# ebanalyse/ebnerd-benchmark

Measured on AMD Instinct MI355X. Metric: training impressions/sec, higher is better.
Workload: dtype f32

## Files before the change

### ebnerd-benchmark_amd/csrc/ebn_attpool.hip

```cpp
#include "ebn_common.h"
#include "ebn_reduce.h"

namespace {

constexpr int POOL_THREADS = 256;
constexpr int POOL_WAVES = POOL_THREADS / 64;
constexpr float KERAS_EPS = 1e-7f;

__global__ __launch_bounds__(POOL_THREADS) void attpool_fwd_kernel(float* __restrict__ U,
                                                                    const float* __restrict__ b,
                                                                    const float* __restrict__ q,
                                                                    const float* __restrict__ X,
                                                                    float* __restrict__ out,
                                                                    float* __restrict__ w, int L, int E, int A) {
  extern __shared__ float sm[];
  const int64_t n = blockIdx.x;
  const int tid = threadIdx.x, lane = tid & 63, wave = tid >> 6;
  for (int l = wave; l < L; l += POOL_WAVES) {
    float* urow = U + (n * L + l) * A;
    float part = 0.f;
    for (int k = lane; k < A; k += 64) {
      const float u = tanhf(urow[k] + b[k]);
      urow[k] = u;
      part = fmaf(u, q[k], part);
    }
    part = ebn_wave_sum(part);
    if (lane == 0) sm[l] = part;
  }
  __syncthreads();
  if (wave == 0) {
    float s = 0.f;
    for (int l = lane; l < L; l += 64) {
      const float a = expf(sm[l]);
      sm[l] = a;
      s += a;
    }
    s = ebn_wave_sum(s) + KERAS_EPS;
    for (int l = lane; l < L; l += 64) {
      const float wl = sm[l] / s;
      sm[l] = wl;
      w[n * L + l] = wl;
    }
  }
  __syncthreads();
  for (int c = tid; c < E; c += POOL_THREADS) {
    float acc = 0.f;
    for (int l = 0; l < L; ++l) acc = fmaf(sm[l], X[(n * L + l) * E + c], acc);
    out[n * E + c] = acc;
  }
}

__global__ __launch_bounds__(POOL_THREADS) void attpool_bwd_pool_kernel(const float* __restrict__ X,
                                                                         const float* __restrict__ w,
                                                                         const float* __restrict__ dout,
                                                                         float* __restrict__ dX,
                                                                         float* __restrict__ de, int L, int E) {
  extern __shared__ float sm[];
  const int64_t n = blockIdx.x;
  const int tid = threadIdx.x, lane = tid & 63, wave = tid >> 6;
  const float* g = dout + n * E;
  for (int l = wave; l < L; l += POOL_WAVES) {
    const float* xr = X + (n * L + l) * E;
    float part = 0.f;
    for (int c = lane; c < E; c += 64) part = fmaf(g[c], xr[c], part);
    part = ebn_wave_sum(part);
    if (lane == 0) sm[l] = part;
  }
  __syncthreads();
  if (wave == 0) {
    float s = 0.f;
    for (int l = lane; l < L; l += 64) s = fmaf(w[n * L + l], sm[l], s);
    s = ebn_wave_sum(s);
    for (int l = lane; l < L; l += 64) de[n * L + l] = w[n * L + l] * (sm[l] - s);
  }
  if (dX == nullptr) return;
  for (int l = 0; l < L; ++l) {
    const float wl = w[n * L + l];
    float* dr = dX + (n * L + l) * E;
    for (int c = tid; c < E; c += POOL_THREADS) dr[c] = wl * g[c];
  }
}

constexpr int POOL_RB = 8;

__device__ __forceinline__ float4 ld4_clamped(const float* __restrict__ base, int64_t off, bool ok) {
  return *reinterpret_cast<const float4*>(base + (ok ? off : 0));
}
__device__ __forceinline__ float4 ld4_or_zero(const float* __restrict__ base, int64_t off, bool ok) {
  const float4 v = ld4_clamped(base, off, ok);
  float4 r;
  r.x = ok ? v.x : 0.f;
  r.y = ok ? v.y : 0.f;
  r.z = ok ? v.z : 0.f;
  r.w = ok ? v.w : 0.f;
  return r;
}

__global__ __launch_bounds__(POOL_THREADS) void attpool_fwd_vec_kernel(float* __restrict__ U,
                                                                        const float* __restrict__ b,
                                                                        const float* __restrict__ q,
                                                                        const float* __restrict__ X,
                                                                        float* __restrict__ out,
                                                                        float* __restrict__ w, int L, int E, int A) {
  extern __shared__ float sm[];
  __shared__ float4 part_acc[POOL_THREADS];
  const int64_t n = blockIdx.x;
  const int tid = threadIdx.x, lane = tid & 63, wave = tid >> 6;
  const int A4 = A >> 2, E4 = E >> 2;
  {
    const bool kok = lane < A4;
    const float4 bb = ld4_or_zero(b, lane * 4, kok), qq = ld4_or_zero(q, lane * 4, kok);
    for (int l0 = wave; l0 < L; l0 += POOL_WAVES * POOL_RB) {
      float4 u[POOL_RB];
#pragma unroll
      for (int j = 0; j < POOL_RB; ++j) {
        const int l = l0 + POOL_WAVES * j;
        u[j] = ld4_clamped(U, (n * L + l) * A + lane * 4, kok && l < L);
      }
#pragma unroll
      for (int j = 0; j < POOL_RB; ++j) {
        const int l = l0 + POOL_WAVES * j;
        if (l >= L) break;
        float4 t;
        t.x = tanhf(u[j].x + bb.x);
        t.y = tanhf(u[j].y + bb.y);
        t.z = tanhf(u[j].z + bb.z);
        t.w = tanhf(u[j].w + bb.w);
        if (kok) *reinterpret_cast<float4*>(U + (n * L + l) * A + lane * 4) = t;
        float part = kok ? fmaf(t.w, qq.w, fmaf(t.z, qq.z, fmaf(t.y, qq.y, t.x * qq.x))) : 0.f;
        part = ebn_wave_sum(part);
        if (lane == 0) sm[l] = part;
      }
    }
  }
  __syncthreads();
  if (wave == 0) {
    float s = 0.f;
    for (int l = lane; l < L; l += 64) {
      const float a = expf(sm[l]);
      sm[l] = a;
      s += a;
    }
    s = ebn_wave_sum(s) + KERAS_EPS;
    for (int l = lane; l < L; l += 64) {
      const float wl = sm[l] / s;
      sm[l] = wl;
      w[n * L + l] = wl;
    }
  }
  __syncthreads();
  const int NP = (E4 <= POOL_THREADS) ? POOL_THREADS / E4 : 1;
  for (int c0 = 0; c0 < E4; c0 += POOL_THREADS) {
    const int c4 = c0 + tid % ((E4 <= POOL_THREADS) ? E4 : POOL_THREADS);
    const int part = (E4 <= POOL_THREADS) ? tid / E4 : 0;
    const bool ok = c4 < E4 && part < NP;
    float4 acc = make_float4(0.f, 0.f, 0.f, 0.f);
    for (int l0 = part; l0 < L; l0 += NP * POOL_RB) {
      float4 x[POOL_RB];
#pragma unroll
      for (int j = 0; j < POOL_RB; ++j) {
        const int l = l0 + NP * j;
        x[j] = ld4_clamped(X, (n * L + l) * E + c4 * 4, ok && l < L);
      }
#pragma unroll
      for (int j = 0; j < POOL_RB; ++j) {
        const int l = l0 + NP * j;
        const float wl = (l < L) ? sm[l] : 0.f;
        acc.x = fmaf(wl, x[j].x, acc.x);
        acc.y = fmaf(wl, x[j].y, acc.y);
        acc.z = fmaf(wl, x[j].z, acc.z);
        acc.w = fmaf(wl, x[j].w, acc.w);
      }
    }
    if (NP > 1) {
      part_acc[tid] = acc;
      __syncthreads();
      if (part == 0 && ok) {
        for (int pp = 1; pp < NP; ++pp) {
          const float4 o = part_acc[pp * E4 + c4];
          acc.x += o.x;
          acc.y += o.y;
          acc.z += o.z;
          acc.w += o.w;
        }
      }
      __syncthreads();
    }
    if (part == 0 && ok) *reinterpret_cast<float4*>(out + n * E + c4 * 4) = acc;
  }
}

__global__ __launch_bounds__(POOL_THREADS) void attpool_bwd_pool_vec_kernel(const float* __restrict__ X,
                                                                             const float* __restrict__ w,
                                                                             const float* __restrict__ dout,
                                                                             float* __restrict__ dX,
                                                                             float* __restrict__ de, int L, int E,
                                                                             int write_dx) {
  extern __shared__ float sm[];
  const int64_t n = blockIdx.x;
  const int tid = threadIdx.x, lane = tid & 63, wave = tid >> 6;
  const int E4 = E >> 2;
  const float* g = dout + n * E;
  constexpr int VL = 4;
  float4 gg[VL];
#pragma unroll
  for (int v = 0; v < VL; ++v) gg[v] = ld4_or_zero(g, (lane + 64 * v) * 4, lane + 64 * v < E4);
  for (int l0 = wave; l0 < L; l0 += POOL_WAVES * POOL_RB) {
    float part[POOL_RB];
#pragma unroll
    for (int j = 0; j < POOL_RB; ++j) part[j] = 0.f;
#pragma unroll
    for (int v = 0; v < VL; ++v) {
      if (64 * v >= E4) break;
      float4 x[POOL_RB];
#pragma unroll
      for (int j = 0; j < POOL_RB; ++j) {
        const int l = l0 + POOL_WAVES * j;
        x[j] = ld4_clamped(X, (n * L + l) * E + (lane + 64 * v) * 4, l < L && lane + 64 * v < E4);
      }
#pragma unroll
      for (int j = 0; j < POOL_RB; ++j)
        part[j] = fmaf(gg[v].w, x[j].w, fmaf(gg[v].z, x[j].z, fmaf(gg[v].y, x[j].y, fmaf(gg[v].x, x[j].x, part[j]))));
    }
#pragma unroll
    for (int j = 0; j < POOL_RB; ++j) {
      const int l = l0 + POOL_WAVES * j;
      const float t = ebn_wave_sum(part[j]);
      if (lane == 0 && l < L) sm[l] = t;
    }
  }
  __syncthreads();
  if (wave == 0) {
    float s = 0.f;
    for (int l = lane; l < L; l += 64) s = fmaf(w[n * L + l], sm[l], s);
    s = ebn_wave_sum(s);
    for (int l = lane; l < L; l += 64) de[n * L + l] = w[n * L + l] * (sm[l] - s);
  }
  if (!write_dx) return;
  for (int c4 = tid; c4 < E4; c4 += POOL_THREADS) {
    const float4 gv = *reinterpret_cast<const float4*>(g + c4 * 4);
    for (int l = 0; l < L; ++l) {
      const float wl = w[n * L + l];
      *reinterpret_cast<float4*>(dX + (n * L + l) * E + c4 * 4) = make_float4(wl * gv.x, wl * gv.y, wl * gv.z, wl * gv.w);
    }
  }
}

__global__ __launch_bounds__(POOL_THREADS) void attpool_bwd_dpre_kernel(float* __restrict__ U,
                                                                         const float* __restrict__ q,
                                                                         const float* __restrict__ de,
                                                                         float* __restrict__ partials,
                                                                         int64_t R, int A, int64_t rpb) {
  const int64_t r0 = static_cast<int64_t>(blockIdx.x) * rpb;
  const int64_t r1 = (r0 + rpb < R) ? r0 + rpb : R;
  for (int k = threadIdx.x; k < A; k += POOL_THREADS) {
    const float qk = q[k];
    float dq = 0.f, db = 0.f;
    for (int64_t rb = r0; rb < r1; rb += 8) {
      float u[8], der[8];
#pragma unroll
      for (int j = 0; j < 8; ++j) {
        const int64_t r = (rb + j < r1) ? rb + j : r1 - 1;
        u[j] = U[r * A + k];
        der[j] = de[r];
      }
#pragma unroll
      for (int j = 0; j < 8; ++j) {
        if (rb + j >= r1) break;
        dq = fmaf(der[j], u[j], dq);
        const float dp = der[j] * qk * (1.0f - u[j] * u[j]);
        U[(rb + j) * A + k] = dp;
        db += dp;
      }
    }
    partials[(static_cast<int64_t>(blockIdx.x) * 2 + 0) * A + k] = dq;
    partials[(static_cast<int64_t>(blockIdx.x) * 2 + 1) * A + k] = db;
  }
}

}

__global__ __launch_bounds__(POOL_THREADS) void attpool_bwd_dpre_vec_kernel(float* __restrict__ U, const float* __restrict__ q,
                                                                             const float* __restrict__ de, float* __restrict__ partials,
                                                                             int64_t R, int A, int64_t rpb) {
  extern __shared__ float sm[];
  const int A4 = A >> 2, RS = POOL_THREADS / A4;
  const int tid = threadIdx.x, c4 = tid % A4, rs = tid / A4;
  const bool active = rs < RS;
  const int64_t r0 = static_cast<int64_t>(blockIdx.x) * rpb;
  const int64_t r1 = (r0 + rpb < R) ? r0 + rpb : R;
  float4 dq = make_float4(0.f, 0.f, 0.f, 0.f), db = dq;
  if (active) {
    const float4 qk = *reinterpret_cast<const float4*>(q + c4 * 4);
    for (int64_t rb = r0 + rs; rb < r1; rb += static_cast<int64_t>(8) * RS) {
      float4 u[8];
      float der[8];
#pragma unroll
      for (int j = 0; j < 8; ++j) {
        int64_t r = rb + static_cast<int64_t>(j) * RS;
        r = r < r1 ? r : r1 - 1;
        u[j] = *reinterpret_cast<const float4*>(U + r * A + c4 * 4);
        der[j] = de[r];
      }
#pragma unroll
      for (int j = 0; j < 8; ++j) {
        const int64_t r = rb + static_cast<int64_t>(j) * RS;
        if (r >= r1) break;
        const float d = der[j];
        dq.x = fmaf(d, u[j].x, dq.x);
        dq.y = fmaf(d, u[j].y, dq.y);
        dq.z = fmaf(d, u[j].z, dq.z);
        dq.w = fmaf(d, u[j].w, dq.w);
        const float4 dp = make_float4(d * qk.x * (1.0f - u[j].x * u[j].x), d * qk.y * (1.0f - u[j].y * u[j].y),
                                      d * qk.z * (1.0f - u[j].z * u[j].z), d * qk.w * (1.0f - u[j].w * u[j].w));
        *reinterpret_cast<float4*>(U + r * A + c4 * 4) = dp;
        db.x += dp.x;
        db.y += dp.y;
        db.z += dp.z;
        db.w += dp.w;
      }
    }
    *reinterpret_cast<float4*>(&sm[rs * A + c4 * 4]) = dq;
    *reinterpret_cast<float4*>(&sm[(RS + rs) * A + c4 * 4]) = db;
  }
  __syncthreads();
  for (int k = tid; k < A; k += POOL_THREADS) {
    float tq = 0.f, tb = 0.f;
    for (int i = 0; i < RS; ++i) {
      tq += sm[i * A + k];
      tb += sm[(RS + i) * A + k];
    }
    partials[(static_cast<int64_t>(blockIdx.x) * 2 + 0) * A + k] = tq;
    partials[(static_cast<int64_t>(blockIdx.x) * 2 + 1) * A + k] = tb;
  }
}

extern "C" int64_t ebn_attpool_partials_len(int64_t R, int32_t A) { return ebn_dim_ok(R, A) ? ebn_colred_blocks(R) * 2 * A : 0; }

extern "C" int ebn_attpool_fwd_f32(float* U, const float* b, const float* q, const float* X, float* out,
                                   float* w, int64_t n_seq, int32_t L, int32_t E, int32_t A,
                                   ebn_stream_t stream) {
  EBN_REQUIRE(U && b && q && X && out && w, EBN_ERR_BAD_ARG);
  EBN_REQUIRE(n_seq >= 0 && L > 0 && E > 0 && A > 0, EBN_ERR_BAD_ARG);
  EBN_REQUIRE(L <= 8192, EBN_ERR_UNSUPPORTED);
  if (n_seq == 0) return EBN_OK;
  const bool vec = (A % 4 == 0) && A <= 256 && (E % 4 == 0) && E <= 1024 && ebn_aligned16(U) && ebn_aligned16(b) &&
                   ebn_aligned16(q) && ebn_aligned16(X) && ebn_aligned16(out);
  if (vec)
    EBN_LAUNCH(attpool_fwd_vec_kernel, dim3(static_cast<unsigned>(n_seq)), dim3(POOL_THREADS),
                       L * sizeof(float), ebn_stream(stream), U, b, q, X, out, w, L, E, A);
  else
    EBN_LAUNCH(attpool_fwd_kernel, dim3(static_cast<unsigned>(n_seq)), dim3(POOL_THREADS),
                       L * sizeof(float), ebn_stream(stream), U, b, q, X, out, w, L, E, A);
  EBN_CHECK_LAUNCH();
  return EBN_OK;
}

extern "C" int ebn_attpool_bwd_pool_f32(const float* X, const float* w, const float* dout, float* dX,
                                        float* de, int64_t n_seq, int32_t L, int32_t E,
                                        ebn_stream_t stream) {
  EBN_REQUIRE(X && w && dout && de, EBN_ERR_BAD_ARG);
  EBN_REQUIRE(n_seq >= 0 && L > 0 && E > 0, EBN_ERR_BAD_ARG);
  EBN_REQUIRE(L <= 8192, EBN_ERR_UNSUPPORTED);
  if (n_seq == 0) return EBN_OK;
  const bool vec = (E % 4 == 0) && E <= 1024 && ebn_aligned16(X) && ebn_aligned16(dout) && ebn_aligned16(dX);
  if (vec)
    EBN_LAUNCH(attpool_bwd_pool_vec_kernel, dim3(static_cast<unsigned>(n_seq)), dim3(POOL_THREADS),
                       L * sizeof(float), ebn_stream(stream), X, w, dout, dX, de, L, E, dX != nullptr ? 1 : 0);
  else
    EBN_LAUNCH(attpool_bwd_pool_kernel, dim3(static_cast<unsigned>(n_seq)), dim3(POOL_THREADS),
                       L * sizeof(float), ebn_stream(stream), X, w, dout, dX, de, L, E);
  EBN_CHECK_LAUNCH();
  return EBN_OK;
}

extern "C" int ebn_attpool_bwd_dpre_f32(float* U, const float* q, const float* de, float* dq, float* db,
                                        float* partials, int64_t R, int32_t A, int32_t accumulate,
                                        ebn_stream_t stream) {
  EBN_REQUIRE(U && q && de && partials && ((dq != nullptr) == (db != nullptr)), EBN_ERR_BAD_ARG);
  EBN_REQUIRE(R >= 0 && A > 0, EBN_ERR_BAD_ARG);
  if (R == 0) return EBN_OK;
  const int64_t nb = ebn_colred_blocks(R);
  const int64_t rpb = ebn_ceil_div(R, nb);
  if ((A % 4) == 0 && A >= 4 && A <= 1024 && ebn_aligned16(U) && ebn_aligned16(q)) {
    const size_t lds = static_cast<size_t>(2) * (POOL_THREADS / (A / 4)) * A * sizeof(float);
    EBN_LAUNCH(attpool_bwd_dpre_vec_kernel, dim3(static_cast<unsigned>(nb)), dim3(POOL_THREADS), lds, ebn_stream(stream), U, q, de, partials,
                       R, A, rpb);
  } else {
    EBN_LAUNCH(attpool_bwd_dpre_kernel, dim3(static_cast<unsigned>(nb)), dim3(POOL_THREADS), 0,
                       ebn_stream(stream), U, q, de, partials, R, A, rpb);
  }
  EBN_CHECK_LAUNCH();
  if (dq == nullptr) return EBN_OK;
  ebn_reduce_partials(partials, nb, 2, A, 1.0f, dq, db, accumulate, nullptr, nullptr, ebn_stream(stream));
  EBN_CHECK_LAUNCH();
  return EBN_OK;
}
```

### ebnerd-benchmark_amd/csrc/ebn_encoder.hip

```cpp
#include "ebn_common.h"

#define EBN_TRY(call)            \
  do {                           \
    int rc__ = (call);           \
    if (rc__ != EBN_OK) return rc__; \
  } while (0)

static int check_dims(const ebn_encoder_dims* d) {
  EBN_REQUIRE(d, EBN_ERR_BAD_ARG);
  EBN_REQUIRE(d->n_seq >= 0 && d->L > 0 && d->Din > 0 && d->h > 0 && d->d > 0 && d->A > 0, EBN_ERR_BAD_ARG);
  return EBN_OK;
}

extern "C" int ebn_encoder_fwd_f32(const ebn_encoder_dims* dims, const ebn_encoder_params* p,
                                   const ebn_encoder_acts* a, const ebn_encoder_scratch* s,
                                   const ebn_step_state* st, ebn_stream_t stream) {
  EBN_TRY(check_dims(dims));
  EBN_REQUIRE(p && a && p->Wqkv && p->W && p->b && p->q, EBN_ERR_BAD_ARG);
  EBN_REQUIRE(a->X && a->QKV && a->Y && a->U && a->w && a->out, EBN_ERR_BAD_ARG);
  const int64_t R = dims->n_seq * dims->L;
  const int E = dims->h * dims->d;
  if (R == 0) return EBN_OK;
  float* ws = s ? s->gemm_ws : nullptr;
  const int64_t ws_n = s ? s->gemm_ws_floats : 0;
  EBN_TRY(ebn_gemm_f32_site(0, 0, R, 3 * E, dims->Din, 1.0f, a->X, dims->Din, p->Wqkv, 3 * E, 0.0f, a->QKV, 3 * E, ws, ws_n,
                            1, stream));
  EBN_TRY(ebn_attn_fwd_f32(a->QKV, 3 * E, a->Y, E, dims->n_seq, dims->L, dims->h, dims->d, st, dims->drop_site,
                           dims->drop_p, stream));
  EBN_TRY(ebn_gemm_f32_ws(0, 0, R, dims->A, E, 1.0f, a->Y, E, p->W, dims->A, 0.0f, a->U, dims->A, ws, ws_n, stream));
  EBN_TRY(ebn_attpool_fwd_f32(a->U, p->b, p->q, a->Y, a->out, a->w, dims->n_seq, dims->L, E, dims->A, stream));
  return EBN_OK;
}

extern "C" int ebn_encoder_fwd_gather_f32(const ebn_encoder_dims* dims, const ebn_encoder_params* p, const ebn_encoder_acts* a,
                                          const ebn_encoder_scratch* s, const int32_t* ids, const float* table, int64_t table_rows,
                                          int32_t* oob_flag, ebn_stream_t stream) {
  EBN_TRY(check_dims(dims));
  EBN_REQUIRE(p && a && ids && table && p->Wqkv && p->W && p->b && p->q, EBN_ERR_BAD_ARG);
  EBN_REQUIRE(a->QKV && a->Y && a->U && a->w && a->out, EBN_ERR_BAD_ARG);
  EBN_REQUIRE(dims->drop_p <= 0.0f, EBN_ERR_UNSUPPORTED);
  const int64_t R = dims->n_seq * dims->L;
  const int E = dims->h * dims->d;
  if (R == 0) return EBN_OK;
  float* ws = s ? s->gemm_ws : nullptr;
  const int64_t ws_n = s ? s->gemm_ws_floats : 0;
  EBN_TRY(ebn_gemm_f32_rowmap(ids, table_rows, R, 3 * E, dims->Din, table, dims->Din, p->Wqkv, 3 * E, a->QKV, 3 * E, oob_flag, stream));
  EBN_TRY(ebn_attn_fwd_f32(a->QKV, 3 * E, a->Y, E, dims->n_seq, dims->L, dims->h, dims->d, nullptr, -1, 0.0f, stream));
  EBN_TRY(ebn_gemm_f32_ws(0, 0, R, dims->A, E, 1.0f, a->Y, E, p->W, dims->A, 0.0f, a->U, dims->A, ws, ws_n, stream));
  EBN_TRY(ebn_attpool_fwd_f32(a->U, p->b, p->q, a->Y, a->out, a->w, dims->n_seq, dims->L, E, dims->A, stream));
  return EBN_OK;
}

extern "C" int ebn_encoder_bwd_f32(const ebn_encoder_dims* dims, const ebn_encoder_params* p,
                                   const ebn_encoder_acts* a, const float* dout, const ebn_encoder_grads* g,
                                   const ebn_encoder_scratch* s, float* dX, int32_t accumulate,
                                   const ebn_step_state* st, ebn_stream_t stream) {
  EBN_TRY(check_dims(dims));
  EBN_REQUIRE(p && a && g && s && dout, EBN_ERR_BAD_ARG);
  EBN_REQUIRE(p->Wqkv && p->W && p->q, EBN_ERR_BAD_ARG);
  EBN_REQUIRE(a->X && a->QKV && a->Y && a->U && a->w, EBN_ERR_BAD_ARG);
  EBN_REQUIRE(g->dWqkv && g->dW && g->db && g->dq, EBN_ERR_BAD_ARG);
  EBN_REQUIRE(s->dY && s->dQKV && s->de && s->partials, EBN_ERR_BAD_ARG);
  const int64_t R = dims->n_seq * dims->L;
  const int E = dims->h * dims->d;
  const int A = dims->A;
  if (R == 0) return EBN_OK;
  const float beta = accumulate ? 1.0f : 0.0f;
  EBN_TRY(ebn_attpool_bwd_pool_f32(a->Y, a->w, dout, nullptr, s->de, dims->n_seq, dims->L, E, stream));
  EBN_TRY(ebn_attpool_bwd_dpre_f32(a->U, p->q, s->de, g->dq, g->db, s->partials, R, A, accumulate, stream));
  const bool fold = ebn_attn_bwd_pooled_supported(dims->L, dims->d) != 0 && (E % 4) == 0 && ebn_aligned16(dout) &&
                    ebn_aligned16(s->dY) && ebn_aligned16(a->QKV) && ebn_aligned16(s->dQKV);
  if (fold) {
    EBN_TRY(ebn_dense_bwd_pair_f32(R, E, A, a->Y, E, a->U, A, p->W, A, beta, g->dW, A, s->dY, E, s->gemm_ws, s->gemm_ws_floats,
                                   stream));
    EBN_TRY(ebn_attn_bwd_pooled_f32(a->QKV, 3 * E, s->dY, E, a->w, dout, E, s->dQKV, 3 * E, dims->n_seq, dims->L, dims->h,
                                    dims->d, st, dims->drop_site, dims->drop_p, stream));
  } else {
    EBN_TRY(ebn_gemm_f32_ws(1, 0, E, A, R, 1.0f, a->Y, E, a->U, A, beta, g->dW, A, s->gemm_ws, s->gemm_ws_floats, stream));
    EBN_TRY(ebn_gemm_f32_rank1(R, E, A, 1.0f, a->U, A, p->W, A, s->dY, E, a->w, dout, E, dims->L, s->gemm_ws,
                               s->gemm_ws_floats, stream));
    EBN_TRY(ebn_attn_bwd_f32(a->QKV, 3 * E, s->dY, E, s->dQKV, 3 * E, dims->n_seq, dims->L, dims->h, dims->d, st, dims->drop_site,
                             dims->drop_p, stream));
  }
  if (dX != nullptr)
    return ebn_dense_bwd_pair_f32(R, dims->Din, 3 * E, a->X, dims->Din, s->dQKV, 3 * E, p->Wqkv, 3 * E, beta, g->dWqkv, 3 * E, dX,
                                  dims->Din, s->gemm_ws, s->gemm_ws_floats, stream);
  EBN_TRY(ebn_gemm_f32_ws(1, 0, dims->Din, 3 * E, R, 1.0f, a->X, dims->Din, s->dQKV, 3 * E, beta, g->dWqkv, 3 * E,
                          s->gemm_ws, s->gemm_ws_floats, stream));
  return EBN_OK;
}

extern "C" int ebn_user_stage_train_f32(const ebn_encoder_dims* dims, const ebn_encoder_params* p, const ebn_encoder_acts* a,
                                        const float* cand, const float* labels, float* scores, float* probs, float* loss_rows,
                                        float* loss_out, float* dcand, float* duser, const ebn_encoder_grads* g,
                                        const ebn_encoder_scratch* s, float* head_partials, float* dX, int32_t C,
                                        int32_t loss_kind, float inv_batch, const ebn_step_state* st, ebn_stream_t stream) {
  EBN_TRY(check_dims(dims));
  EBN_REQUIRE(p && a && g && s && cand && labels && scores && probs && loss_rows && loss_out && dcand && duser && dX, EBN_ERR_BAD_ARG);
  EBN_REQUIRE(p->Wqkv && p->W && p->b && p->q && a->X && a->QKV && a->Y && a->U && a->w && a->out, EBN_ERR_BAD_ARG);
  EBN_REQUIRE(g->dWqkv && g->dW && g->db && g->dq && s->dY && s->dQKV && s->de && s->partials, EBN_ERR_BAD_ARG);
  EBN_REQUIRE(C > 0 && dims->drop_p <= 0.0f, EBN_ERR_BAD_ARG);
  const int64_t B = dims->n_seq, R = dims->n_seq * dims->L;
  const int E = dims->h * dims->d, A = dims->A, L = dims->L;
  if (R == 0) return EBN_OK;
  const bool fused = head_partials != nullptr && ebn_user_head_supported(L, C, E, A) != 0 &&
                     ebn_attn_bwd_pooled_supported(L, dims->d) != 0 && ebn_aligned16(a->U) && ebn_aligned16(a->Y) &&
                     ebn_aligned16(cand) && ebn_aligned16(dcand) && ebn_aligned16(duser) && ebn_aligned16(a->out) &&
                     ebn_aligned16(p->b) && ebn_aligned16(p->q) && ebn_aligned16(s->dY) && ebn_aligned16(a->QKV) &&
                     ebn_aligned16(s->dQKV);
  if (!fused) {
    EBN_TRY(ebn_encoder_fwd_f32(dims, p, a, s, st, stream));
    EBN_TRY(ebn_score_loss_train_f32(cand, a->out, labels, scores, probs, loss_rows, loss_out, dcand, duser, B, C, E, loss_kind,
                                     inv_batch, stream));
    return ebn_encoder_bwd_f32(dims, p, a, duser, g, s, dX, 0, st, stream);
  }
  float* ws = s->gemm_ws;
  const int64_t ws_n = s->gemm_ws_floats;
  EBN_TRY(ebn_gemm_f32_site(0, 0, R, 3 * E, dims->Din, 1.0f, a->X, dims->Din, p->Wqkv, 3 * E, 0.0f, a->QKV, 3 * E, ws, ws_n, 1, stream));
  EBN_TRY(ebn_attn_fwd_f32(a->QKV, 3 * E, a->Y, E, B, L, dims->h, dims->d, nullptr, -1, 0.0f, stream));
  EBN_TRY(ebn_gemm_f32_ws(0, 0, R, A, E, 1.0f, a->Y, E, p->W, A, 0.0f, a->U, A, ws, ws_n, stream));
  EBN_TRY(ebn_user_head_train_f32(a->U, p->b, p->q, a->Y, cand, labels, a->w, a->out, scores, probs, loss_rows, loss_out, dcand,
                                  duser, s->de, g->dq, g->db, head_partials, B, L, C, E, A, loss_kind, inv_batch, stream));
  EBN_TRY(ebn_dense_bwd_pair_f32(R, E, A, a->Y, E, a->U, A, p->W, A, 0.0f, g->dW, A, s->dY, E, ws, ws_n, stream));
  EBN_TRY(ebn_attn_bwd_pooled_f32(a->QKV, 3 * E, s->dY, E, a->w, duser, E, s->dQKV, 3 * E, B, L, dims->h, dims->d, nullptr, -1, 0.0f,
                                  stream));
  return ebn_dense_bwd_pair_f32(R, dims->Din, 3 * E, a->X, dims->Din, s->dQKV, 3 * E, p->Wqkv, 3 * E, 0.0f, g->dWqkv, 3 * E, dX,
                                dims->Din, ws, ws_n, stream);
}
```

### ebnerd-benchmark_amd/csrc/ebn_gemm.hip

```cpp
#include <stdlib.h>

#include "ebn_common.h"
#include "ebn_finish.h"
#include "ebn_tn_finale.h"

typedef float ebn_f32x4 __attribute__((ext_vector_type(4)));
typedef int ebn_i32x4 __attribute__((ext_vector_type(4)));
__device__ ebn_f32x4 ebn_raw_buffer_load_x4(ebn_i32x4 rsrc, int voffset, int soffset, int aux) __asm("llvm.amdgcn.raw.buffer.load.v4f32");
__device__ void ebn_raw_buffer_load_lds(ebn_i32x4 rsrc, __attribute__((address_space(3))) void* lds, int size, int voffset,
                                        int soffset, int offset, int aux) __asm("llvm.amdgcn.raw.buffer.load.lds");

int ebn_gemm_direct_tn_slices(int64_t M, int64_t N, int64_t K);
int ebn_gemm_direct_tn_launch(int64_t M, int64_t N, int64_t K, float alpha, const float* A, int64_t lda, const float* B, int64_t ldb,
                              float* part, hipStream_t s);
bool ebn_gemm_direct_wanted(int32_t transA, int32_t transB, int64_t M, int64_t N, int64_t K);
int ebn_gemm_direct_launch(int32_t transB, int64_t M, int64_t N, int64_t K, float alpha, const float* A, int64_t lda, const float* B,
                           int64_t ldb, float* C, int64_t ldc, hipStream_t s);

namespace {

typedef float f32x16 __attribute__((ext_vector_type(16)));


typedef float f32x4n __attribute__((ext_vector_type(4)));
__device__ __forceinline__ float4 gload4(const __attribute__((address_space(1))) float* p) {
  const f32x4n t = *reinterpret_cast<const __attribute__((address_space(1))) f32x4n*>(p);
  return make_float4(t.x, t.y, t.z, t.w);
}
typedef ebn_i32x4 i32x4n;
__device__ __forceinline__ i32x4n make_rsrc(const float* base) {
  const unsigned long long a = reinterpret_cast<unsigned long long>(base);
  i32x4n r;
  r.x = static_cast<int>(static_cast<uint32_t>(a));
  r.y = static_cast<int>(static_cast<uint32_t>(a >> 32) & 0xFFFFu);
  r.z = -1;
  r.w = 0x00020000;
  return r;
}
__device__ __forceinline__ float4 bload4(i32x4n r, uint32_t lane_bytes, uint32_t slab_bytes) {
  const f32x4n t = ebn_raw_buffer_load_x4(r, static_cast<int>(lane_bytes), static_cast<int>(slab_bytes), 0);
  return make_float4(t.x, t.y, t.z, t.w);
}

constexpr int GEMM_WPE = 3;
constexpr int BK = 16;
constexpr int PAD = 4;
constexpr int GEMM_THREADS = 256;

template <int BMN, bool KCONTIG, bool VEC, int PADX = PAD>
struct TileLoader {
  static constexpr int VECS = BMN * BK / 4;
  static constexpr int PER_THREAD = VECS / GEMM_THREADS;
  static_assert(VECS % GEMM_THREADS == 0, "tile/thread mismatch");

  __device__ static __forceinline__ float4 load(const float* __restrict__ P, int64_t ld, int64_t mn0,
                                                int64_t k0, int64_t MN, int64_t Kdim, int v) {
    int64_t gmn, gk;
    if (KCONTIG) {
      gmn = mn0 + v / (BK / 4);
      gk = k0 + (v % (BK / 4)) * 4;
    } else {
      gk = k0 + v / (BMN / 4);
      gmn = mn0 + (v % (BMN / 4)) * 4;
    }
    const int64_t off = KCONTIG ? (gmn * ld + gk) : (gk * ld + gmn);
    if (VEC) {
      const bool valid = (gmn < MN) && (gk < Kdim);
      const float4 r = *reinterpret_cast<const float4*>(P + (valid ? off : 0));
      float4 z;
      z.x = valid ? r.x : 0.f;
      z.y = valid ? r.y : 0.f;
      z.z = valid ? r.z : 0.f;
      z.w = valid ? r.w : 0.f;
      return z;
    }
    float4 r = make_float4(0.f, 0.f, 0.f, 0.f);
    if (KCONTIG) {
      if (gmn < MN) {
        const float* p = P + off;
        if (gk + 0 < Kdim) r.x = p[0];
        if (gk + 1 < Kdim) r.y = p[1];
        if (gk + 2 < Kdim) r.z = p[2];
        if (gk + 3 < Kdim) r.w = p[3];
      }
    } else {
      if (gk < Kdim) {
        const float* p = P + off;
        if (gmn + 0 < MN) r.x = p[0];
        if (gmn + 1 < MN) r.y = p[1];
        if (gmn + 2 < MN) r.z = p[2];
        if (gmn + 3 < MN) r.w = p[3];
      }
    }
    return r;
  }

  __device__ static __forceinline__ void store(float* __restrict__ S, int v, float4 r) {
    constexpr int LD = BMN + PADX;
    if (KCONTIG) {
      const int mn = v / (BK / 4);
      const int kq = v % (BK / 4);
      *reinterpret_cast<float4*>(&S[(mn * 4 + (kq ^ ((mn >> 2) & 3))) * 4]) = r;
    } else {
      const int k = v / (BMN / 4);
      const int mq = v % (BMN / 4);
      *reinterpret_cast<float4*>(&S[k * LD + mq * 4]) = r;
    }
  }
};

struct GemmEpi {
  const float* rs;
  const float* cv;
  int64_t ldcv;
  int32_t L;
  const float* bias;
  float* colsum = nullptr;
  const float* l2w = nullptr;
  float two_lambda = 0.f;
  const int32_t* rowmap = nullptr;
  int64_t rowmap_rows = 0;
  int32_t* oob = nullptr;
#ifdef EBN_GEMM_EXP_STAGGER
  uint32_t stagger_pct = 0;
#endif
};

template <int BM, int BN, int WAVES_M, bool TA, bool TB, bool VEC, int EPI = 0>
__global__ __launch_bounds__(GEMM_THREADS, GEMM_WPE) void gemm_f32_kernel(
    int64_t M, int64_t N, int64_t K, float alpha, const float* __restrict__ A, int64_t lda,
    const float* __restrict__ B, int64_t ldb, float beta, float* __restrict__ C, int64_t ldc,
    int64_t k_per_split, float* __restrict__ Cpart, GemmEpi epi) {
  constexpr int WAVES_N = 4 / WAVES_M;
  constexpr int WTM = BM / WAVES_M;
  constexpr int WTN = BN / WAVES_N;
  constexpr int TM = WTM / 32;
  constexpr int TN = WTN / 32;
  constexpr bool GLDS_A = VEC;
  constexpr bool GLDS_B = GLDS_A;
  constexpr int PADA = GLDS_A ? 0 : PAD, PADB = GLDS_B ? 0 : PAD;
  constexpr int LDA_S = BM + PADA;
  constexpr int LDB_S = BN + PADB;
  using LA = TileLoader<BM, !TA, VEC, PADA>;
  using LB = TileLoader<BN, TB, VEC, PADB>;

  constexpr bool A_KC = !TA, B_KC = TB;
  constexpr int A_FLOATS = A_KC ? BM * BK : BK * LDA_S, B_FLOATS = B_KC ? BN * BK : BK * LDB_S;
  __shared__ __attribute__((aligned(16))) float smem[2 * (A_FLOATS + B_FLOATS)];
#define EBN_AS(b) (smem + (b) * A_FLOATS)
#define EBN_BS(b) (smem + 2 * A_FLOATS + (b) * B_FLOATS)

  const int tid = threadIdx.x;
  const int lane = tid & 63;
  const int wave = __builtin_amdgcn_readfirstlane(tid >> 6);
  const int wm = wave / WAVES_N;
  const int wn = wave % WAVES_N;
  const int64_t GX = gridDim.x, GY = gridDim.y, GZ = gridDim.z;
  const int64_t per_z = GX * GY, nwg = per_z * GZ;
  const int64_t vb = static_cast<int64_t>(blockIdx.y) * gridDim.x + blockIdx.x + per_z * blockIdx.z;
  int64_t m0 = 0, n0 = 0, kbeg = 0, kend = 0, zsplit = 0;
  int nk = 0, nk_full = 0, nk_main = 0;

  f32x16 acc[TM][TN];

  float4 ra[LA::PER_THREAD], rb[LB::PER_THREAD];

  uint32_t oa[LA::PER_THREAD], ob[LB::PER_THREAD];
  i32x4n arsrc, brsrc;
  const uint32_t step_a = static_cast<uint32_t>((TA ? BK * lda : BK) * 4);
  const uint32_t step_b = static_cast<uint32_t>((TB ? BK : BK * ldb) * 4);
// ... 803 lines not shown
    if (b < nh - 1) {
      const int idx = b * 256 + tid;
      if (tid < 256 && idx < 2 * f.A) {
        const int sidx = idx / f.A, k = idx - sidx * f.A;
        float* gp = (sidx == 0 ? f.dq : f.db) + k;
        ebn_adam_flat_apply(f.adam, al, gp - f.adam.grad, *gp);
      }
    } else if (tid == 0 && f.n_l2 > 0) {
      float tot = 0.f;
      for (int l = 0; l < f.n_l2; ++l) {
        float tl = 0.f;
        for (int j = 0; j < f.l2_tiles[l]; ++j) tl += f.l2_part[l * f.l2_slots + j];
        tot += tl;
      }
      f.loss_out[0] += f.l2 * tot;
    }
  }
}

int launch_gemm_small(int transA, int transB, int64_t M, int64_t N, int64_t K, float alpha, const float* A, int64_t lda,
                      const float* B, int64_t ldb, float beta, float* C, int64_t ldc, int vecA, int vecB, hipStream_t s,
                      GemmEpi epi) {
  const dim3 grid(static_cast<unsigned>(ebn_ceil_div(N, SBN)), static_cast<unsigned>(ebn_ceil_div(M, SBM))), block(GEMM_THREADS);
  constexpr size_t lds = static_cast<size_t>(2) * 2 * SBM * SLD * sizeof(float);
#define EBN_SMALL_ONE(TA, TB, VA, VB)                                                                                     \
  do {                                                                                                                     \
    static const hipError_t attr__ = hipFuncSetAttribute(reinterpret_cast<const void*>(&gemm_small_kernel<TA, TB, VA, VB>), \
                                                         hipFuncAttributeMaxDynamicSharedMemorySize, static_cast<int>(lds)); \
    if (attr__ != hipSuccess) return static_cast<int>(attr__);                                                            \
    EBN_LAUNCH((gemm_small_kernel<TA, TB, VA, VB>), grid, block, lds, s, M, N, K, alpha, A, lda, B, ldb, beta, C, ldc, epi); \
  } while (0)
#define EBN_SMALL_VEC_T(TA, TB, T)                                                                                         \
  do {                                                                                                                     \
    constexpr size_t lds_t = static_cast<size_t>(2) * 2 * (T) * SLV * sizeof(float);                                       \
    static const hipError_t attr__ = hipFuncSetAttribute(reinterpret_cast<const void*>(&gemm_small_vec_kernel<TA, TB, T>), \
                                                         hipFuncAttributeMaxDynamicSharedMemorySize, static_cast<int>(lds_t)); \
    if (attr__ != hipSuccess) return static_cast<int>(attr__);                                                            \
    const dim3 grid_t(static_cast<unsigned>(ebn_ceil_div(N, T)), static_cast<unsigned>(ebn_ceil_div(M, T)));               \
    EBN_LAUNCH((gemm_small_vec_kernel<TA, TB, T>), grid_t, dim3((T) * (T) / 4), lds_t, s, M, N, K, alpha, A, lda, B, ldb, \
                       beta, C, ldc, epi);                                                                                 \
  } while (0)
#define EBN_SMALL_VEC(TA, TB) EBN_SMALL_VEC_T(TA, TB, 32)
  const bool fits32 = (K + SBK) * (transA ? lda : 1) * 4 + 64 * lda * 4 < (int64_t{1} << 31) &&
                      (K + SBK) * (transB ? 1 : ldb) * 4 + 64 * ldb * 4 < (int64_t{1} << 31);
#define EBN_SMALL(TA, TB)                              \
  do {                                                 \
    if (vecA && vecB && fits32) EBN_SMALL_VEC(TA, TB); \
    else EBN_SMALL_ONE(TA, TB, false, false);          \
  } while (0)
  if (!transA && !transB) EBN_SMALL(false, false);
  else if (!transA && transB) EBN_SMALL(false, true);
  else if (transA && !transB) EBN_SMALL(true, false);
  else EBN_SMALL(true, true);
#undef EBN_SMALL
#undef EBN_SMALL_VEC
#undef EBN_SMALL_VEC_T
#undef EBN_SMALL_ONE
  EBN_CHECK_LAUNCH();
  return EBN_OK;
}

}

struct GemmPlan {
  int bm, bn;
  int splits;
  int64_t kps;
  double cost;
};

static GemmPlan gemm_plan(int64_t M, int64_t N, int64_t K, int64_t ws_floats) {
  int64_t max_split = K / (4 * BK);
  if (max_split > 64) max_split = 64;
  const int64_t max_by_ws = (M * N > 0) ? ws_floats / (M * N) : 0;
  if (max_split > max_by_ws) max_split = max_by_ws;
  if (max_split < 1 || M * N >= (static_cast<int64_t>(1) << 31)) max_split = 1;
  static const struct {
    int bm, bn;
    double ts_full, ts_lone;
    int resident;
    int family;
  } kTiles[4] = {{128, 128, 1.15, 1.5, 3, 128}, {256, 64, 1.17, 1.5, 3, 256}, {64, 64, 0.32, 0.48, 4, 64}, {128, 64, 0.60, 0.8, 3, 96}};
  const double out_mb = static_cast<double>(M) * static_cast<double>(N) * 4e-6;
  GemmPlan best{128, 128, 1, ebn_ceil_div(K > 0 ? K : 1, BK) * BK, 1e300};
  {
    const int64_t wgs = ebn_ceil_div(M, SBM) * ebn_ceil_div(N, SBN);
    const int64_t tiles64 = ebn_ceil_div(M, 64) * ebn_ceil_div(N, 64);
    if (tiles64 <= 256 && K <= 4096) {
      const int64_t W = ebn_ceil_div(wgs, 256);
      double per_slab = static_cast<double>(W / 2) * 1.6 + static_cast<double>(W % 2) * 1.1;
      if (W >= 3) per_slab *= 1.3;
      const double cost = static_cast<double>(ebn_ceil_div(K > 0 ? K : 1, SBK)) * per_slab + 3.0;
      const bool measured = K <= 1536 && W <= 3;
      best = GemmPlan{32, 32, 1, ebn_ceil_div(K > 0 ? K : 1, SBK) * SBK, measured ? cost : 0.8 * cost};
      if (measured) return best;
    }
  }
  for (int t = 0; t < 4; ++t) {
    if (kTiles[t].bm == 256 && M < 256) continue;
    const int64_t tiles = ebn_ceil_div(M, kTiles[t].bm) * ebn_ceil_div(N, kTiles[t].bn);
    int64_t prev_s = 0;
    for (int64_t c = 1; c <= max_split; ++c) {
      const int64_t kps = ebn_ceil_div(ebn_ceil_div(K > 0 ? K : 1, c), BK) * BK;
      const int64_t sp = ebn_ceil_div(K > 0 ? K : 1, kps);
      if (sp == prev_s) continue;
      prev_s = sp;
      const int64_t W = ebn_ceil_div(tiles * sp, 256);
      const double full = static_cast<double>(W) * kTiles[t].ts_full;
      const double lone = static_cast<double>(ebn_ceil_div(W, kTiles[t].resident)) * kTiles[t].ts_lone;
      double cost = static_cast<double>(kps / BK) * (full > lone ? full : lone) + 3.0;
      if (sp > 1) cost += 4.5 + static_cast<double>(sp + 1) * out_mb / 2.5;
      if (kTiles[t].bm == 64 && sp > 1 && kps / BK >= 64 && W <= 6) cost *= 1.0 - 0.01 * static_cast<double>(W);
      if (cost < best.cost) best = GemmPlan{kTiles[t].bm, kTiles[t].bn, static_cast<int>(sp), kps, cost};
    }
  }
  return best;
}

extern "C" int64_t ebn_gemm_workspace_floats(int64_t M, int64_t N, int64_t K) {
  if (!ebn_dim_ok(M, N, K)) return 0;
  const GemmPlan p = gemm_plan(M, N, K, INT64_MAX / 4);
  int64_t slices = p.splits > 1 ? p.splits : 0;
  const int64_t tn = ebn_gemm_direct_tn_slices(M, N, K);
  if (tn > slices) slices = tn;
  return ebn_sat_mul(slices * M, N);
}

extern "C" int ebn_gemm_plan(int64_t M, int64_t N, int64_t K, int64_t workspace_floats, int32_t* bm, int32_t* bn,
                             int32_t* splits) {
  EBN_REQUIRE(M >= 0 && N >= 0 && K >= 0 && bm && bn && splits, EBN_ERR_BAD_ARG);
  const GemmPlan p = gemm_plan(M, N, K, workspace_floats);
  *bm = p.bm;
  *bn = p.bn;
  *splits = p.splits;
  return EBN_OK;
}

static int gemm_dispatch(int32_t transA, int32_t transB, int64_t M, int64_t N, int64_t K, float alpha, const float* A,
                         int64_t lda, const float* B, int64_t ldb, float beta, float* C, int64_t ldc, float* workspace,
                         int64_t workspace_floats, int32_t site, GemmEpi epi, hipStream_t s, int32_t* defer_parts = nullptr) {
  if (defer_parts != nullptr) {
    C = workspace;
    ldc = N;
    beta = 0.f;
    *defer_parts = 1;
  }
  const bool spanA = (transA ? (K + 16) * lda + 256 : 256 * lda + K + 16) * 4 < (int64_t{1} << 32);
  const bool spanB = (transB ? 256 * ldb + K + 16 : (K + 16) * ldb + 256) * 4 < (int64_t{1} << 32);
  const int vecA = ((lda % 4) == 0 && ebn_aligned16(A) && ((transA ? M : K) % 4) == 0 && spanA) ? 1 : 0;
  const int vecB = ((ldb % 4) == 0 && ebn_aligned16(B) && ((transB ? K : N) % 4) == 0 && spanB) ? 1 : 0;
  if ((epi.bias != nullptr || epi.rs != nullptr) && !(vecA && vecB)) return EBN_ERR_UNSUPPORTED;
  if (epi.bias == nullptr && epi.rs == nullptr && beta == 0.f && vecA && (vecB || !transB) &&
      ebn_gemm_direct_wanted(transA, transB, M, N, K)) {
    const int rc_dir = ebn_gemm_direct_launch(transB, M, N, K, alpha, A, lda, B, ldb, C, ldc, s);
    if (rc_dir != EBN_ERR_UNSUPPORTED) return rc_dir;
  }
  if (transA && !transB && epi.bias == nullptr && epi.rs == nullptr && workspace != nullptr &&
      M * N < (int64_t{1} << 31)) {
    const int z = ebn_gemm_direct_tn_slices(M, N, K);
    if (z >= 2 && workspace_floats >= static_cast<int64_t>(z) * M * N) {
      const int rc_tn = ebn_gemm_direct_tn_launch(M, N, K, alpha, A, lda, B, ldb, workspace, s);
      if (rc_tn == EBN_OK) {
        if (defer_parts != nullptr) {
          *defer_parts = z;
          return EBN_OK;
        }
        int64_t grid = ebn_ceil_div(M * N, 256);
        if (grid > 4096) grid = 4096;
        EBN_LAUNCH(splitk_reduce_kernel, dim3(static_cast<unsigned>(grid)), dim3(256), 0, s, workspace, z, M, N, beta, C, ldc, epi);
        EBN_CHECK_LAUNCH();
        return EBN_OK;
      }
      if (rc_tn != EBN_ERR_UNSUPPORTED) return rc_tn;
    }
  }
  const GemmPlan plan = gemm_plan(M, N, K, workspace ? workspace_floats : 0);
  const int splits = plan.splits;
  const int64_t kps = plan.kps;
  int rc;
  if (plan.bm == 32)
    return launch_gemm_small(transA, transB, M, N, K, alpha, A, lda, B, ldb, beta, C, ldc, vecA, vecB, s, epi);
  if (!(vecA && vecB))
    rc = launch_gemm<64, 64, 2>(transA, transB, M, N, K, alpha, A, lda, B, ldb, beta, C, ldc, vecA, vecB, splits, kps, workspace, s, site, epi);
  else if (plan.bm == 256)
    rc = launch_gemm<256, 64, 4>(transA, transB, M, N, K, alpha, A, lda, B, ldb, beta, C, ldc, vecA, vecB, splits, kps,
                                 workspace, s, site, epi);
  else if (plan.bm == 128 && plan.bn == 64)
    rc = launch_gemm<128, 64, 2>(transA, transB, M, N, K, alpha, A, lda, B, ldb, beta, C, ldc, vecA, vecB, splits, kps,
                                 workspace, s, site, epi);
  else if (plan.bm == 128)
    rc = launch_gemm<128, 128, 2>(transA, transB, M, N, K, alpha, A, lda, B, ldb, beta, C, ldc, vecA, vecB, splits, kps,
                                  workspace, s, site, epi);
  else
    rc = launch_gemm<64, 64, 2>(transA, transB, M, N, K, alpha, A, lda, B, ldb, beta, C, ldc, vecA, vecB, splits, kps,
                                workspace, s, site, epi);
  if (rc != EBN_OK) return rc;
  if (splits > 1 && defer_parts != nullptr) {
    *defer_parts = splits;
    return EBN_OK;
  }
  if (splits > 1) {
    int64_t grid = ebn_ceil_div(M * N, 256);
    if (grid > 4096) grid = 4096;
    EBN_LAUNCH(splitk_reduce_kernel, dim3(static_cast<unsigned>(grid)), dim3(256), 0, s, workspace,
                       splits, M, N, beta, C, ldc, epi);
    EBN_CHECK_LAUNCH();
  }
  return EBN_OK;
}

extern "C" int64_t ebn_gemm_partials_workspace_floats(int64_t M, int64_t N, int64_t K) {
  if (!ebn_dim_ok(M, N, K)) return 0;
  const GemmPlan p = gemm_plan(M, N, K, INT64_MAX / 4);
  int64_t slices = p.splits > 1 ? p.splits : 1;
  const int64_t tn = ebn_gemm_direct_tn_slices(M, N, K);
  if (tn > slices) slices = tn;
  return ebn_sat_mul(slices * M, N);
}

extern "C" int ebn_gemm_f32_partials(int32_t transA, int32_t transB, int64_t M, int64_t N, int64_t K, float alpha, const float* A,
                                     int64_t lda, const float* B, int64_t ldb, float* workspace, int64_t workspace_floats,
                                     int32_t* n_parts, ebn_stream_t stream) {
  EBN_REQUIRE(M > 0 && N > 0 && K >= 0 && n_parts, EBN_ERR_BAD_ARG);
  EBN_REQUIRE(A && B && workspace && workspace_floats >= M * N, EBN_ERR_BAD_ARG);
  EBN_REQUIRE(lda >= (transA ? M : K) && ldb >= (transB ? K : N), EBN_ERR_BAD_ARG);
  return gemm_dispatch(transA, transB, M, N, K, alpha, A, lda, B, ldb, 0.0f, workspace, N, workspace, workspace_floats, 0,
                       GemmEpi{nullptr, nullptr, 0, 1, nullptr}, ebn_stream(stream), n_parts);
}

extern "C" int ebn_gemm_f32_site(int32_t transA, int32_t transB, int64_t M, int64_t N, int64_t K, float alpha,
                                 const float* A, int64_t lda, const float* B, int64_t ldb, float beta, float* C,
                                 int64_t ldc, float* workspace, int64_t workspace_floats, int32_t site,
                                 ebn_stream_t stream) {
  EBN_REQUIRE(M >= 0 && N >= 0 && K >= 0, EBN_ERR_BAD_ARG);
  if (M == 0 || N == 0) return EBN_OK;
  EBN_REQUIRE(A && B && C, EBN_ERR_BAD_ARG);
  EBN_REQUIRE(lda >= (transA ? M : K) && ldb >= (transB ? K : N) && ldc >= N, EBN_ERR_BAD_ARG);
  return gemm_dispatch(transA, transB, M, N, K, alpha, A, lda, B, ldb, beta, C, ldc, workspace, workspace_floats, site,
                       GemmEpi{nullptr, nullptr, 0, 1, nullptr}, ebn_stream(stream));
}

namespace {
__global__ __launch_bounds__(256) void rank1_fill_kernel(float* __restrict__ C, int64_t ldc, int64_t M, int64_t N,
                                                         GemmEpi epi) {
  const int64_t total = M * N;
  for (int64_t i = static_cast<int64_t>(blockIdx.x) * 256 + threadIdx.x; i < total; i += static_cast<int64_t>(gridDim.x) * 256) {
    const int64_t row = i / N, col = i - row * N;
    C[row * ldc + col] = epi.rs[row] * epi.cv[(row / epi.L) * epi.ldcv + col];
  }
}
}

extern "C" int ebn_gemm_f32_rank1(int64_t M, int64_t N, int64_t K, float alpha, const float* A, int64_t lda,
                                  const float* B, int64_t ldb, float* C, int64_t ldc, const float* row_scale,
                                  const float* seq_rows, int64_t ld_seq, int32_t L, float* workspace,
                                  int64_t workspace_floats, ebn_stream_t stream) {
  EBN_REQUIRE(M >= 0 && N >= 0 && K >= 0 && L > 0, EBN_ERR_BAD_ARG);
  EBN_REQUIRE(M < (static_cast<int64_t>(1) << 31), EBN_ERR_UNSUPPORTED);
  if (M == 0 || N == 0) return EBN_OK;
  EBN_REQUIRE(A && B && C && row_scale && seq_rows, EBN_ERR_BAD_ARG);
  EBN_REQUIRE(lda >= K && ldb >= K && ldc >= N && ld_seq >= N, EBN_ERR_BAD_ARG);
  const GemmEpi epi{row_scale, seq_rows, ld_seq, L, nullptr};
  hipStream_t s = ebn_stream(stream);
  const bool vec = (lda % 4) == 0 && ebn_aligned16(A) && (ldb % 4) == 0 && ebn_aligned16(B) && (K % 4) == 0;
  if (vec)
    return gemm_dispatch(0, 1, M, N, K, alpha, A, lda, B, ldb, 0.0f, C, ldc, workspace, workspace_floats, 0, epi, s);
  int64_t grid = ebn_ceil_div(M * N, 256);
  if (grid > 4096) grid = 4096;
  EBN_LAUNCH(rank1_fill_kernel, dim3(static_cast<unsigned>(grid)), dim3(256), 0, s, C, ldc, M, N, epi);
  EBN_CHECK_LAUNCH();
  return gemm_dispatch(0, 1, M, N, K, alpha, A, lda, B, ldb, 1.0f, C, ldc, workspace, workspace_floats, 0,
                       GemmEpi{nullptr, nullptr, 0, 1, nullptr}, s);
}

extern "C" int ebn_dense_relu_fwd_f32(int64_t M, int64_t N, int64_t K, const float* A, int64_t lda, const float* B,
                                      int64_t ldb, const float* bias, float* C, int64_t ldc, float* workspace,
                                      int64_t workspace_floats, ebn_stream_t stream) {
  EBN_REQUIRE(M >= 0 && N >= 0 && K >= 0, EBN_ERR_BAD_ARG);
  if (M == 0 || N == 0) return EBN_OK;
  EBN_REQUIRE(A && B && C && bias, EBN_ERR_BAD_ARG);
  EBN_REQUIRE(lda >= K && ldb >= N && ldc >= N, EBN_ERR_BAD_ARG);
  hipStream_t s = ebn_stream(stream);
  const bool vec = (lda % 4) == 0 && ebn_aligned16(A) && (K % 4) == 0 && (ldb % 4) == 0 && ebn_aligned16(B) && (N % 4) == 0;
  if (vec)
    return gemm_dispatch(0, 0, M, N, K, 1.0f, A, lda, B, ldb, 0.0f, C, ldc, workspace, workspace_floats, 0,
                         GemmEpi{nullptr, nullptr, 0, 1, bias}, s);
  const int rc = gemm_dispatch(0, 0, M, N, K, 1.0f, A, lda, B, ldb, 0.0f, C, ldc, workspace, workspace_floats, 0,
                               GemmEpi{nullptr, nullptr, 0, 1, nullptr}, s);
  if (rc != EBN_OK) return rc;
  for (int64_t r = 0; ldc != N && r < M; ++r) {
    const int rr = ebn_bias_relu_f32(C + r * ldc, bias, C + r * ldc, 1, static_cast<int32_t>(N), stream);
    if (rr != EBN_OK) return rr;
  }
  return (ldc == N) ? ebn_bias_relu_f32(C, bias, C, M, static_cast<int32_t>(N), stream) : EBN_OK;
}

extern "C" int ebn_gemm_f32_ws(int32_t transA, int32_t transB, int64_t M, int64_t N, int64_t K, float alpha,
                               const float* A, int64_t lda, const float* B, int64_t ldb, float beta,
                               float* C, int64_t ldc, float* workspace, int64_t workspace_floats,
                               ebn_stream_t stream) {
  return ebn_gemm_f32_site(transA, transB, M, N, K, alpha, A, lda, B, ldb, beta, C, ldc, workspace, workspace_floats, 0,
                           stream);
}

extern "C" int ebn_dense_bwd_pair_f32(int64_t R, int64_t K_in, int64_t N_out, const float* X, int64_t ldx, const float* dY,
                                      int64_t lddy, const float* W, int64_t ldw, float beta_w, float* dW, int64_t lddw,
                                      float* dX, int64_t lddx, float* workspace, int64_t workspace_floats,
                                      ebn_stream_t stream) {
  EBN_REQUIRE(R >= 0 && K_in >= 0 && N_out >= 0, EBN_ERR_BAD_ARG);
  if (K_in == 0 || N_out == 0) return EBN_OK;
  EBN_REQUIRE(X && dY && W && dW && dX, EBN_ERR_BAD_ARG);
  EBN_REQUIRE(ldx >= K_in && lddy >= N_out && ldw >= N_out && lddw >= N_out && lddx >= K_in, EBN_ERR_BAD_ARG);
  hipStream_t s = ebn_stream(stream);
  const bool aligned = (ldx % 4) == 0 && (lddy % 4) == 0 && (ldw % 4) == 0 && ebn_aligned16(X) && ebn_aligned16(dY) &&
                       ebn_aligned16(W) && (K_in % 4) == 0 && (N_out % 4) == 0;
  const int64_t span = (R + SBK) * (ldx > lddy ? ldx : lddy) * 4 + 64 * ((ldx > lddy ? ldx : lddy) > ldw ? (ldx > lddy ? ldx : lddy) : ldw) * 4;
  const bool small = R > 0 && gemm_plan(K_in, N_out, R, workspace ? workspace_floats : 0).bm == 32 &&
                     gemm_plan(R, K_in, N_out, workspace ? workspace_floats : 0).bm == 32;
  if (aligned && small && span < (int64_t{1} << 31)) {
    SmallProblem p0{K_in, N_out, R, 1.0f, X, ldx, dY, lddy, beta_w, dW, lddw, static_cast<int32_t>(ebn_ceil_div(N_out, SBN)), 0};
    p0.tiles = p0.tiles_x * static_cast<int32_t>(ebn_ceil_div(K_in, SBM));
    SmallProblem p1{R, K_in, N_out, 1.0f, dY, lddy, W, ldw, 0.0f, dX, lddx, static_cast<int32_t>(ebn_ceil_div(K_in, SBN)), 0};
    p1.tiles = p1.tiles_x * static_cast<int32_t>(ebn_ceil_div(R, SBM));
    constexpr size_t lds = static_cast<size_t>(2) * 2 * SBM * SLV * sizeof(float);
    static const hipError_t attr = hipFuncSetAttribute(reinterpret_cast<const void*>(&gemm_small_pair_kernel),
                                                       hipFuncAttributeMaxDynamicSharedMemorySize, static_cast<int>(lds));
    if (attr != hipSuccess) return static_cast<int>(attr);
    EBN_LAUNCH(gemm_small_pair_kernel, dim3(static_cast<unsigned>(p0.tiles + p1.tiles)), dim3(GEMM_THREADS), lds, s, p0, p1);
    EBN_CHECK_LAUNCH();
    return EBN_OK;
  }
  const GemmEpi none{nullptr, nullptr, 0, 1, nullptr};
  if (R == 0) {
    return gemm_dispatch(1, 0, K_in, N_out, 0, 1.0f, X, ldx, dY, lddy, beta_w, dW, lddw, workspace, workspace_floats, 0, none, s);
  }
  const int rc = gemm_dispatch(1, 0, K_in, N_out, R, 1.0f, X, ldx, dY, lddy, beta_w, dW, lddw, workspace, workspace_floats, 0, none, s);
  if (rc != EBN_OK) return rc;
  return gemm_dispatch(0, 1, R, K_in, N_out, 1.0f, dY, lddy, W, ldw, 0.0f, dX, lddx, workspace, workspace_floats, 0, none, s);
}

extern "C" int ebn_gemm_f32_rowmap(const int32_t* ids, int64_t table_rows, int64_t M, int64_t N, int64_t K, const float* table,
                                   int64_t ldt, const float* B, int64_t ldb, float* C, int64_t ldc, int32_t* oob_flag, ebn_stream_t stream) {
  EBN_REQUIRE(ebn_dim_ok(M, N, K) && table_rows > 0, EBN_ERR_BAD_ARG);
  if (M == 0 || N == 0) return EBN_OK;
  EBN_REQUIRE(ids && table && B && C && ldt >= K && ldb >= N && ldc >= N && K > 0, EBN_ERR_BAD_ARG);
  const bool ok = M >= 256 && (ldt % 4) == 0 && (ldb % 4) == 0 && (K % 4) == 0 && (N % 4) == 0 && ebn_aligned16(table) && ebn_aligned16(B) &&
                  (table_rows * ldt + K + 16) * 4 < (int64_t{1} << 32) && ((K + 16) * ldb + 256) * 4 < (int64_t{1} << 32);
  if (!ok) return EBN_ERR_UNSUPPORTED;
  GemmEpi epi{nullptr, nullptr, 0, 1, nullptr};
  epi.rowmap = ids;
  epi.rowmap_rows = table_rows;
  epi.oob = oob_flag;
  return launch_gemm<256, 64, 4>(0, 0, M, N, K, 1.0f, table, ldt, B, ldb, 0.0f, C, ldc, 1, 1, 1, ebn_ceil_div(K, BK) * BK, nullptr,
                                 ebn_stream(stream), 0, epi);
}

extern "C" int ebn_gemm_tn_group_f32(const ebn_tn_problem* problems, int32_t n, ebn_stream_t stream) {
  EBN_REQUIRE(problems != nullptr && n >= 1 && n <= EBN_TN_GROUP_MAX, EBN_ERR_BAD_ARG);
  int64_t tiles64 = 0;
  for (int i = 0; i < n; ++i) {
    const ebn_tn_problem& q = problems[i];
    EBN_REQUIRE(ebn_dim_ok(q.M, q.N, q.K) && q.K >= 1, EBN_ERR_BAD_ARG);
    if (q.M == 0 || q.N == 0) continue;
    EBN_REQUIRE(q.A && q.B && q.C, EBN_ERR_BAD_ARG);
    EBN_REQUIRE(q.lda >= q.M && q.ldb >= q.N && q.ldc >= q.N, EBN_ERR_BAD_ARG);
    EBN_REQUIRE((q.lda % 4) == 0 && (q.ldb % 4) == 0 && (q.M % 4) == 0 && (q.N % 4) == 0 && ebn_aligned16(q.A) && ebn_aligned16(q.B),
                EBN_ERR_UNSUPPORTED);
    EBN_REQUIRE((q.K + SBK) * (q.lda > q.ldb ? q.lda : q.ldb) * 4 + 64 * 4 < (int64_t{1} << 31), EBN_ERR_UNSUPPORTED);
    tiles64 += ebn_ceil_div(q.M, 64) * ebn_ceil_div(q.N, 64);
  }
  const int T = tiles64 >= 192 ? 64 : 32;
  SmallGroup g{};
  int64_t total = 0;
  g.n = 0;
  for (int i = 0; i < n; ++i) {
    const ebn_tn_problem& q = problems[i];
    if (q.M == 0 || q.N == 0) continue;
    const int j = g.n++;
    g.p[j] = SmallProblem{q.M, q.N, q.K, 1.0f, q.A, q.lda, q.B, q.ldb, 0.0f, q.C, q.ldc, static_cast<int32_t>(ebn_ceil_div(q.N, T)), 0};
    g.p[j].tiles = g.p[j].tiles_x * static_cast<int32_t>(ebn_ceil_div(q.M, T));
    g.colsum[j] = q.colsum;
    g.l2w[j] = q.l2_W;
    g.two_lambda[j] = q.two_lambda;
    g.first[j] = static_cast<int32_t>(total);
    total += g.p[j].tiles;
    EBN_REQUIRE(total < (int64_t{1} << 30), EBN_ERR_UNSUPPORTED);
  }
  if (g.n == 0) return EBN_OK;
  g.first[g.n] = static_cast<int32_t>(total);
#define EBN_TN_GROUP(TT)                                                                                                          \
  do {                                                                                                                            \
    constexpr size_t lds = static_cast<size_t>(2) * 2 * (TT) * SLV * sizeof(float);                                               \
    static const hipError_t attr = hipFuncSetAttribute(reinterpret_cast<const void*>(&gemm_small_tn_group_kernel<TT>),            \
                                                       hipFuncAttributeMaxDynamicSharedMemorySize, static_cast<int>(lds));        \
    if (attr != hipSuccess) return static_cast<int>(attr);                                                                        \
    EBN_LAUNCH(gemm_small_tn_group_kernel<TT>, dim3(static_cast<unsigned>(total)), dim3((TT) * (TT) / 4), lds, ebn_stream(stream), g); \
  } while (0)
  if (T == 64) EBN_TN_GROUP(64);
  else EBN_TN_GROUP(32);
#undef EBN_TN_GROUP
  EBN_CHECK_LAUNCH();
  return EBN_OK;
}

int ebn_tn_group_finale_launch(const ebn_tn_problem* problems, int32_t n, const EbnTnFinale& fin, hipStream_t s) {
  EBN_REQUIRE(problems != nullptr && n >= 1 && n <= EBN_TN_GROUP_MAX, EBN_ERR_BAD_ARG);
  int64_t tiles64 = 0;
  for (int i = 0; i < n; ++i) {
    const ebn_tn_problem& q = problems[i];
    EBN_REQUIRE(ebn_dim_ok(q.M, q.N, q.K) && q.K >= 1 && q.M > 0 && q.N > 0, EBN_ERR_BAD_ARG);
    EBN_REQUIRE(q.A && q.B && q.C, EBN_ERR_BAD_ARG);
    EBN_REQUIRE(q.lda >= q.M && q.ldb >= q.N && q.ldc >= q.N, EBN_ERR_BAD_ARG);
    EBN_REQUIRE((q.lda % 4) == 0 && (q.ldb % 4) == 0 && (q.M % 4) == 0 && (q.N % 4) == 0 && ebn_aligned16(q.A) && ebn_aligned16(q.B),
                EBN_ERR_UNSUPPORTED);
    EBN_REQUIRE((q.K + SBK) * (q.lda > q.ldb ? q.lda : q.ldb) * 4 + 64 * 4 < (int64_t{1} << 31), EBN_ERR_UNSUPPORTED);
    tiles64 += ebn_ceil_div(q.M, 64) * ebn_ceil_div(q.N, 64);
  }
  const int T = tiles64 >= 192 ? 64 : 32;
  SmallGroupFin gf{};
  gf.f = fin;
  SmallGroup& g = gf.g;
  int64_t total = 0;
  g.n = n;
  for (int i = 0; i < n; ++i) {
    const ebn_tn_problem& q = problems[i];
    g.p[i] = SmallProblem{q.M, q.N, q.K, 1.0f, q.A, q.lda, q.B, q.ldb, 0.0f, q.C, q.ldc, static_cast<int32_t>(ebn_ceil_div(q.N, T)), 0};
    g.p[i].tiles = g.p[i].tiles_x * static_cast<int32_t>(ebn_ceil_div(q.M, T));
    g.colsum[i] = q.colsum;
    g.l2w[i] = q.l2_W;
    g.two_lambda[i] = q.two_lambda;
    g.first[i] = static_cast<int32_t>(total);
    total += g.p[i].tiles;
    EBN_REQUIRE(total < (int64_t{1} << 30), EBN_ERR_UNSUPPORTED);
  }
  g.first[n] = static_cast<int32_t>(total);
  const int64_t nh = (2 * static_cast<int64_t>(fin.A) + 255) / 256 + 1, nwg = total > nh ? total : nh;
#define EBN_TN_FINALE(TT)                                                                                                         \
  do {                                                                                                                            \
    constexpr size_t lds = static_cast<size_t>(2) * 2 * (TT) * SLV * sizeof(float);                                               \
    static const hipError_t attr = hipFuncSetAttribute(reinterpret_cast<const void*>(&gemm_small_tn_finale_kernel<TT>),           \
                                                       hipFuncAttributeMaxDynamicSharedMemorySize, static_cast<int>(lds));        \
    if (attr != hipSuccess) return static_cast<int>(attr);                                                                        \
    EBN_LAUNCH(gemm_small_tn_finale_kernel<TT>, dim3(static_cast<unsigned>(nwg)), dim3((TT) * (TT) / 4), lds, s, gf);             \
  } while (0)
  if (T == 64) EBN_TN_FINALE(64);
  else EBN_TN_FINALE(32);
#undef EBN_TN_FINALE
  EBN_CHECK_LAUNCH();
  return EBN_OK;
}

extern "C" int ebn_gemm_f32(int32_t transA, int32_t transB, int64_t M, int64_t N, int64_t K, float alpha,
                            const float* A, int64_t lda, const float* B, int64_t ldb, float beta, float* C,
                            int64_t ldc, ebn_stream_t stream) {
  return ebn_gemm_f32_ws(transA, transB, M, N, K, alpha, A, lda, B, ldb, beta, C, ldc, nullptr, 0, stream);
// ... 2 lines not shown
```

### ebnerd-benchmark_amd/csrc/ebn_gemm_direct.hip

```cpp
#include <stdlib.h>

#include "ebn_common.h"

typedef float ebn_dir_f32x4 __attribute__((ext_vector_type(4)));
typedef int ebn_dir_i32x4 __attribute__((ext_vector_type(4)));
__device__ ebn_dir_f32x4 ebn_dir_buffer_load_x4(ebn_dir_i32x4 rsrc, int voffset, int soffset, int aux) __asm("llvm.amdgcn.raw.buffer.load.v4f32");
__device__ float ebn_dir_buffer_load_x1(ebn_dir_i32x4 rsrc, int voffset, int soffset, int aux) __asm("llvm.amdgcn.raw.buffer.load.f32");

namespace {

constexpr bool INTERLEAVE = true;
typedef float f32x4 __attribute__((ext_vector_type(4)));

__device__ __forceinline__ ebn_dir_i32x4 dir_rsrc(const float* base) {
  const unsigned long long a = reinterpret_cast<unsigned long long>(base);
  ebn_dir_i32x4 r;
  r.x = static_cast<int>(static_cast<uint32_t>(a));
  r.y = static_cast<int>(static_cast<uint32_t>(a >> 32) & 0xFFFFu);
  r.z = -1;
  r.w = 0x00020000;
  return r;
}

template <int R, int NC>
struct DirFrags {
  f32x4 a[R];
  f32x4 b[NC];
};

template <int R, int NC, bool B_KC>
struct DirPlan {
  ebn_dir_i32x4 arsrc, brsrc;
  uint32_t oa[R];
  uint32_t ob[NC];
  uint32_t ldb4;
};

template <int R, int NC, bool B_KC>
__device__ __forceinline__ void dir_fetch(DirFrags<R, NC>& f, const DirPlan<R, NC, B_KC>& p, uint32_t sa, uint32_t sb) {
#pragma unroll
  for (int r = 0; r < R; ++r) f.a[r] = ebn_dir_buffer_load_x4(p.arsrc, static_cast<int>(p.oa[r]), static_cast<int>(sa), 0);
  if (B_KC) {
#pragma unroll
    for (int c = 0; c < NC; ++c) f.b[c] = ebn_dir_buffer_load_x4(p.brsrc, static_cast<int>(p.ob[c]), static_cast<int>(sb), 0);
  } else {
#pragma unroll
    for (int s = 0; s < 4; ++s)
#pragma unroll
      for (int c = 0; c < NC; ++c)
        f.b[c][s] = ebn_dir_buffer_load_x1(p.brsrc, static_cast<int>(p.ob[c]), static_cast<int>(sb + static_cast<uint32_t>(s) * p.ldb4), 0);
  }
}

template <int R, int NC, bool B_KC>
__device__ __forceinline__ void dir_fetch_tail(DirFrags<R, NC>& f, const DirPlan<R, NC, B_KC>& p, uint32_t sa, uint32_t sb, bool ok) {
  const f32x4 zero = {0.f, 0.f, 0.f, 0.f};
#pragma unroll
  for (int r = 0; r < R; ++r) {
    const f32x4 t = ebn_dir_buffer_load_x4(p.arsrc, static_cast<int>(ok ? p.oa[r] + sa : 0u), 0, 0);
    f.a[r] = ok ? t : zero;
  }
  if (B_KC) {
#pragma unroll
    for (int c = 0; c < NC; ++c) {
      const f32x4 t = ebn_dir_buffer_load_x4(p.brsrc, static_cast<int>(ok ? p.ob[c] + sb : 0u), 0, 0);
      f.b[c] = ok ? t : zero;
    }
  } else {
#pragma unroll
    for (int s = 0; s < 4; ++s)
#pragma unroll
      for (int c = 0; c < NC; ++c) {
        const float t = ebn_dir_buffer_load_x1(p.brsrc, static_cast<int>(ok ? p.ob[c] + sb + static_cast<uint32_t>(s) * p.ldb4 : 0u), 0, 0);
        f.b[c][s] = ok ? t : 0.f;
      }
  }
}

template <int R, int NC>
__device__ __forceinline__ void dir_mma(f32x4 (&acc)[R][NC], const DirFrags<R, NC>& f) {
#pragma unroll
  for (int s = 0; s < 4; ++s)
#pragma unroll
    for (int r = 0; r < R; ++r)
#pragma unroll
      for (int c = 0; c < NC; ++c) acc[r][c] = __builtin_amdgcn_mfma_f32_16x16x4f32(f.a[r][s], f.b[c][s], acc[r][c], 0, 0, 0);
}

template <int R, int NC, bool B_KC, int DEPTH>
__device__ __forceinline__ void dir_task(int64_t M, int64_t N, int64_t K, float alpha, const float* __restrict__ A, int64_t lda,
                                         const float* __restrict__ B, int64_t ldb, float* __restrict__ C, int64_t ldc, int64_t rb0,
                                         int cb0, int lane) {
  const int ln = lane & 15, kq = lane >> 4;
  const int64_t row0 = rb0 * 16;
  DirPlan<R, NC, B_KC> p;
  p.arsrc = dir_rsrc(A + row0 * lda);
  p.brsrc = dir_rsrc(B);
  p.ldb4 = static_cast<uint32_t>(ldb * 4);
#pragma unroll
  for (int r = 0; r < R; ++r) {
    int64_t row = row0 + 16 * r + ln;
    row = row < M ? row : M - 1;
    p.oa[r] = static_cast<uint32_t>(((row - row0) * lda + 4 * kq) * 4);
  }
#pragma unroll
  for (int c = 0; c < NC; ++c) {
    int64_t col = static_cast<int64_t>(cb0 + c) * 16 + ln;
    col = col < N ? col : N - 1;
    p.ob[c] = B_KC ? static_cast<uint32_t>((col * ldb + 4 * kq) * 4) : static_cast<uint32_t>((4 * kq * ldb + col) * 4);
  }
  const uint32_t step_a = 64u, step_b = B_KC ? 64u : static_cast<uint32_t>(16 * ldb * 4);

  f32x4 acc[R][NC];
#pragma unroll
  for (int r = 0; r < R; ++r)
#pragma unroll
    for (int c = 0; c < NC; ++c) acc[r][c] = f32x4{0.f, 0.f, 0.f, 0.f};

  const int nkf = static_cast<int>(K / 16);
  const int krem = static_cast<int>(K - 16 * static_cast<int64_t>(nkf));
  DirFrags<R, NC> f0, f1;
  uint32_t sa = 0, sb = 0;
  constexpr int N_LOADS = R + (B_KC ? NC : 4 * NC), N_MFMA = 4 * R * NC, PER_LOAD = (N_MFMA / N_LOADS) > 0 ? (N_MFMA / N_LOADS) : 1;
#define EBN_DIR_STEP(FL, FM)                                                   \
  do {                                                                         \
    dir_fetch(FL, p, sa, sb);                                                  \
    sa += step_a;                                                              \
    sb += step_b;                                                              \
    dir_mma(acc, FM);                                                          \
    if (INTERLEAVE) {                                                          \
      _Pragma("unroll") for (int i__ = 0; i__ < N_LOADS; ++i__) {              \
        __builtin_amdgcn_sched_group_barrier(0x008, PER_LOAD, 0);    \
        __builtin_amdgcn_sched_group_barrier(0x020, 1, 0);         \
      }                                                                        \
      __builtin_amdgcn_sched_group_barrier(0x008, N_MFMA - PER_LOAD * N_LOADS, 0); \
    }                                                                          \
    __builtin_amdgcn_sched_barrier(0);                                         \
  } while (0)
#define EBN_DIR_FETCH(F)               \
  do {                                 \
    dir_fetch(F, p, sa, sb);           \
    sa += step_a;                      \
    sb += step_b;                      \
    __builtin_amdgcn_sched_barrier(0); \
  } while (0)
#define EBN_DIR_MMA(F)                 \
  do {                                 \
    dir_mma(acc, F);                   \
    __builtin_amdgcn_sched_barrier(0); \
  } while (0)
  {
    if (nkf > 0) {
      EBN_DIR_FETCH(f0);
      int g = 0;
      for (; g + 2 < nkf; g += 2) {
        EBN_DIR_STEP(f1, f0);
        EBN_DIR_STEP(f0, f1);
      }
      if (g + 1 < nkf) {
        EBN_DIR_STEP(f1, f0);
        EBN_DIR_MMA(f1);
      } else {
        EBN_DIR_MMA(f0);
      }
    }
  }
#undef EBN_DIR_FETCH
#undef EBN_DIR_MMA
#undef EBN_DIR_STEP
  if (krem > 0) {
    dir_fetch_tail(f0, p, sa, sb, 4 * kq < krem);
    dir_mma(acc, f0);
  }

#pragma unroll
  for (int r = 0; r < R; ++r) {
#pragma unroll
    for (int c = 0; c < NC; ++c) {
      const int64_t col = static_cast<int64_t>(cb0 + c) * 16 + ln;
#pragma unroll
      for (int i = 0; i < 4; ++i) {
        const int64_t row = row0 + 16 * r + 4 * kq + i;
        if (row < M && col < N) C[row * ldc + col] = alpha * acc[r][c][i];
      }
    }
  }
}

template <int R, int CW, bool B_KC, int DEPTH>
__global__ __launch_bounds__(256, 2) void gemm_direct16_kernel(int64_t M, int64_t N, int64_t K, float alpha, const float* __restrict__ A,
                                                               int64_t lda, const float* __restrict__ B, int64_t ldb,
                                                               float* __restrict__ C, int64_t ldc, int32_t G, int32_t n_wide, int64_t n_tasks) {
  const int lane = threadIdx.x & 63;
  const int wave = __builtin_amdgcn_readfirstlane(threadIdx.x >> 6);
  const int64_t t = static_cast<int64_t>(blockIdx.x) * 4 + wave;
  if (t >= n_tasks) return;
  const int64_t rg = t / G;
  const int cg = static_cast<int>(t - rg * G);
  const int cb0 = cg < n_wide ? cg * CW : n_wide * CW + (cg - n_wide) * (CW - 1);
  if (cg < n_wide) dir_task<R, CW, B_KC, DEPTH>(M, N, K, alpha, A, lda, B, ldb, C, ldc, rg * R, cb0, lane);
  else dir_task<R, CW - 1, B_KC, DEPTH>(M, N, K, alpha, A, lda, B, ldb, C, ldc, rg * R, cb0, lane);
}

template <int R, int NC>
struct TnPlan {
  ebn_dir_i32x4 arsrc, brsrc;
  uint32_t oa[R], ob[NC];
  uint32_t lda4, ldb4;
};

template <int R, int NC>
__device__ __forceinline__ void tn_fetch(DirFrags<R, NC>& f, const TnPlan<R, NC>& p, uint32_t sa, uint32_t sb) {
#pragma unroll
  for (int s = 0; s < 4; ++s) {
#pragma unroll
    for (int r = 0; r < R; ++r)
      f.a[r][s] = ebn_dir_buffer_load_x1(p.arsrc, static_cast<int>(p.oa[r]), static_cast<int>(sa + static_cast<uint32_t>(s) * p.lda4), 0);
#pragma unroll
    for (int c = 0; c < NC; ++c)
      f.b[c][s] = ebn_dir_buffer_load_x1(p.brsrc, static_cast<int>(p.ob[c]), static_cast<int>(sb + static_cast<uint32_t>(s) * p.ldb4), 0);
  }
}

template <int R, int NC>
__device__ __forceinline__ void tn_fetch_tail(DirFrags<R, NC>& f, const TnPlan<R, NC>& p, uint32_t sa, uint32_t sb, int kq, int krem) {
#pragma unroll
  for (int s = 0; s < 4; ++s) {
    const bool ok = 4 * kq + s < krem;
#pragma unroll
    for (int r = 0; r < R; ++r) {
      const float t = ebn_dir_buffer_load_x1(p.arsrc, static_cast<int>(ok ? p.oa[r] + sa + static_cast<uint32_t>(s) * p.lda4 : 0u), 0, 0);
      f.a[r][s] = ok ? t : 0.f;
    }
#pragma unroll
    for (int c = 0; c < NC; ++c) {
      const float t = ebn_dir_buffer_load_x1(p.brsrc, static_cast<int>(ok ? p.ob[c] + sb + static_cast<uint32_t>(s) * p.ldb4 : 0u), 0, 0);
      f.b[c][s] = ok ? t : 0.f;
    }
  }
}

template <int R, int NC>
__device__ __forceinline__ void tn_task(float* red, int64_t M, int64_t N, float alpha, const float* __restrict__ A, int64_t lda,
                                        const float* __restrict__ B, int64_t ldb, float* __restrict__ out, int64_t k0, int64_t klen,
                                        int64_t rb0, int cb0, int lane, int wave) {
  const int ln = lane & 15, kq = lane >> 4;
  TnPlan<R, NC> p;
  p.arsrc = dir_rsrc(A + k0 * lda);
  p.brsrc = dir_rsrc(B + k0 * ldb);
  p.lda4 = static_cast<uint32_t>(lda * 4);
  p.ldb4 = static_cast<uint32_t>(ldb * 4);
#pragma unroll
  for (int r = 0; r < R; ++r) {
    int64_t m = (rb0 + r) * 16 + ln;
    m = m < M ? m : M - 1;
    p.oa[r] = static_cast<uint32_t>((4 * kq * lda + m) * 4);
  }
#pragma unroll
  for (int c = 0; c < NC; ++c) {
    int64_t n = static_cast<int64_t>(cb0 + c) * 16 + ln;
    n = n < N ? n : N - 1;
    p.ob[c] = static_cast<uint32_t>((4 * kq * ldb + n) * 4);
  }
  f32x4 acc[R][NC];
#pragma unroll
  for (int r = 0; r < R; ++r)
#pragma unroll
    for (int c = 0; c < NC; ++c) acc[r][c] = f32x4{0.f, 0.f, 0.f, 0.f};

  const int ng = static_cast<int>((klen + 15) / 16), krem = static_cast<int>(klen - 16 * (klen / 16));
  const int mine = ng > wave ? (ng - wave + 3) / 4 : 0;
  const bool tail_mine = krem > 0 && mine > 0 && ((ng - 1) & 3) == wave;
  const int nkf = mine - (tail_mine ? 1 : 0);
  const uint32_t step_a = 64u * p.lda4, step_b = 64u * p.ldb4;
  uint32_t sa = static_cast<uint32_t>(wave) * 16u * p.lda4, sb = static_cast<uint32_t>(wave) * 16u * p.ldb4;
  DirFrags<R, NC> f0, f1;
  constexpr int N_LOADS = 4 * (R + NC), N_MFMA = 4 * R * NC, PER_LOAD = (N_MFMA / N_LOADS) > 0 ? (N_MFMA / N_LOADS) : 1;
#define EBN_TN_FETCH(F)                \
  do {                                 \
    tn_fetch(F, p, sa, sb);            \
    sa += step_a;                      \
    sb += step_b;                      \
    __builtin_amdgcn_sched_barrier(0); \
  } while (0)
#define EBN_TN_STEP(FL, FM)                                                    \
  do {                                                                         \
    tn_fetch(FL, p, sa, sb);                                                   \
    sa += step_a;                                                              \
    sb += step_b;                                                              \
    dir_mma(acc, FM);                                                          \
    if (INTERLEAVE) {                                                          \
      _Pragma("unroll") for (int i__ = 0; i__ < N_LOADS; ++i__) {              \
        __builtin_amdgcn_sched_group_barrier(0x008, PER_LOAD, 0);              \
        __builtin_amdgcn_sched_group_barrier(0x020, 1, 0);                     \
      }                                                                        \
      __builtin_amdgcn_sched_group_barrier(0x008, N_MFMA - PER_LOAD * N_LOADS, 0); \
    }                                                                          \
    __builtin_amdgcn_sched_barrier(0);                                         \
  } while (0)
  if (nkf > 0) {
    EBN_TN_FETCH(f0);
    int g = 0;
    for (; g + 2 < nkf; g += 2) {
      EBN_TN_STEP(f1, f0);
      EBN_TN_STEP(f0, f1);
    }
    if (g + 1 < nkf) {
      EBN_TN_STEP(f1, f0);
      dir_mma(acc, f1);
    } else {
      dir_mma(acc, f0);
    }
  }
#undef EBN_TN_FETCH
#undef EBN_TN_STEP
  if (tail_mine) {
    tn_fetch_tail(f0, p, sa, sb, kq, krem);
    dir_mma(acc, f0);
  }

#pragma unroll 1
  for (int w = 1; w < 4; ++w) {
    if (wave == w) {
#pragma unroll
      for (int r = 0; r < R; ++r)
#pragma unroll
        for (int c = 0; c < NC; ++c) *reinterpret_cast<f32x4*>(red + ((r * NC + c) * 64 + lane) * 4) = acc[r][c];
    }
    __syncthreads();
    if (wave == 0) {
#pragma unroll
      for (int r = 0; r < R; ++r)
#pragma unroll
        for (int c = 0; c < NC; ++c) acc[r][c] += *reinterpret_cast<const f32x4*>(red + ((r * NC + c) * 64 + lane) * 4);
    }
    __syncthreads();
  }
  if (wave != 0) return;
#pragma unroll
  for (int r = 0; r < R; ++r) {
#pragma unroll
    for (int c = 0; c < NC; ++c) {
      const int64_t col = static_cast<int64_t>(cb0 + c) * 16 + ln;
#pragma unroll
      for (int i = 0; i < 4; ++i) {
        const int64_t row = (rb0 + r) * 16 + 4 * kq + i;
        if (row < M && col < N) out[row * N + col] = alpha * acc[r][c][i];
      }
    }
  }
}

template <int R, int CW>
__global__ __launch_bounds__(256, (R * CW >= 20) ? 1 : 2) void gemm_direct16_tn_kernel(int64_t M, int64_t N, int64_t K, float alpha, const float* __restrict__ A,
                                                                  int64_t lda, const float* __restrict__ B, int64_t ldb,
                                                                  float* __restrict__ part, int32_t G, int32_t n_wide, int32_t tiles,
                                                                  int64_t kps) {
  __shared__ __attribute__((aligned(16))) float red[R * CW * 256];
  const int lane = threadIdx.x & 63;
  const int wave = __builtin_amdgcn_readfirstlane(threadIdx.x >> 6);
  int64_t lin = blockIdx.x;
  {
    const int64_t nwg = gridDim.x, q = nwg / 8, r = nwg % 8, xcd = lin % 8, idx = lin / 8;
    lin = ((xcd < r) ? xcd * (q + 1) : r * (q + 1) + (xcd - r) * q) + idx;
  }
  const int64_t z = lin / tiles;
  const int tile = static_cast<int>(lin - z * tiles);
  const int rg = tile / G, cg = tile - rg * G;
  const int cb0 = cg < n_wide ? cg * CW : n_wide * CW + (cg - n_wide) * (CW - 1);
  const int64_t k0 = z * kps;
  const int64_t klen = (k0 + kps < K) ? kps : K - k0;
  float* out = part + z * M * N;
  if (cg < n_wide) tn_task<R, CW>(red, M, N, alpha, A, lda, B, ldb, out, k0, klen, static_cast<int64_t>(rg) * R, cb0, lane, wave);
  else tn_task<R, CW - 1>(red, M, N, alpha, A, lda, B, ldb, out, k0, klen, static_cast<int64_t>(rg) * R, cb0, lane, wave);
}

struct TnDirectPlan {
  int R, CW, G, n_wide, tiles, Z;
  int64_t kps;
};

TnDirectPlan tn_direct_plan(int64_t M, int64_t N, int64_t K) {
  const int64_t MB = ebn_ceil_div(M, 16), NB = ebn_ceil_div(N, 16);
  TnDirectPlan best{0, 0, 0, 0, 0, 0, 0};
  double best_cost = 1e300;
  static const int kR[3] = {5, 4, 3}, kC[2] = {5, 4};
  constexpr int wgs = 256;
  for (int ci = 0; ci < 2; ++ci) {
    const int64_t cw = kC[ci], G = ebn_ceil_div(NB, cw), n_wide = NB - G * (cw - 1);
    if (n_wide < 0 || n_wide > G) continue;
    for (int ri = 0; ri < 3; ++ri) {
      const int64_t tiles = ebn_ceil_div(MB, kR[ri]) * G;
      if (tiles > wgs) continue;
      int64_t Z = wgs / tiles;
      if (Z < 2) continue;
      if (Z > 64) Z = 64;
      const int64_t kps = ebn_ceil_div(ebn_ceil_div(K, Z), 64) * 64;
      Z = ebn_ceil_div(K, kps);
      if (Z < 2 || kps < 256) continue;
      const double cost = static_cast<double>(kR[ri] * (n_wide > 0 ? cw : cw - 1)) * static_cast<double>(kps / 64) * (tiles * Z > wgs ? 2.0 : 1.0);
      if (cost < best_cost) {
        best_cost = cost;
        best = TnDirectPlan{kR[ri], static_cast<int>(cw), static_cast<int>(G), static_cast<int>(n_wide), static_cast<int>(tiles), static_cast<int>(Z), kps};
      }
    }
  }
  return best;
}

struct DirectPlan {
  int R, CW, G, n_wide;
  int64_t tasks;
  double cost;
};

DirectPlan direct_plan(int64_t M, int64_t N, bool b_kc) {
  const int64_t MB = ebn_ceil_div(M, 16), NB = ebn_ceil_div(N, 16);
  DirectPlan best{0, 0, 0, 0, 0, 1e300};
  static const int kR[4] = {4, 3, 2, 1}, kC[3] = {7, 5, 4};
  for (int ci = 0; ci < 3; ++ci) {
    const int64_t cw = kC[ci], G = ebn_ceil_div(NB, cw), n_wide = NB - G * (cw - 1);
    if (n_wide < 0 || n_wide > G) continue;
    const int64_t width = n_wide > 0 ? cw : cw - 1;
    for (int ri = 0; ri < 4; ++ri) {
      if (b_kc && kR[ri] == 1) continue;
      const int64_t tasks = ebn_ceil_div(MB, kR[ri]) * G;
      const double rounds = static_cast<double>(ebn_ceil_div(tasks, 1024));
      const double cost = rounds * kR[ri] * static_cast<double>(width) * (1.0 + 0.02 * static_cast<double>(kR[ri] + width) / static_cast<double>(kR[ri] * width));
      if (cost < best.cost) best = DirectPlan{kR[ri], static_cast<int>(cw), static_cast<int>(G), static_cast<int>(n_wide), tasks, cost};
    }
  }
  return best;
}

template <int R, int CW>
int direct_launch_rc(bool b_kc, const DirectPlan& pl, int64_t M, int64_t N, int64_t K, float alpha, const float* A, int64_t lda, const float* B,
                     int64_t ldb, float* C, int64_t ldc, hipStream_t s) {
  const dim3 grid(static_cast<unsigned>(ebn_ceil_div(pl.tasks, 4))), block(256);
#define EBN_DIR_GO(KC, DP) \
  EBN_LAUNCH((gemm_direct16_kernel<R, CW, KC, DP>), grid, block, 0, s, M, N, K, alpha, A, lda, B, ldb, C, ldc, pl.G, pl.n_wide, pl.tasks)
  if constexpr (R == 1) {
    if (b_kc) return EBN_ERR_UNSUPPORTED;
    EBN_DIR_GO(false, 2);
  } else if (b_kc) EBN_DIR_GO(true, 2);
  else EBN_DIR_GO(false, 2);
#undef EBN_DIR_GO
  EBN_CHECK_LAUNCH();
  return EBN_OK;
}

}

bool ebn_gemm_direct_wanted(int32_t transA, int32_t transB, int64_t M, int64_t N, int64_t K) {
  if (transA) return false;
  if (M < 4096 || N < 48 || N > 512 || K < 32 || K > 2048 || (K % 4)) return false;
  constexpr int64_t max_b = int64_t{2} << 20;
  if (N * K * 4 > max_b) return false;
  const DirectPlan pl = direct_plan(M, N, transB != 0);
  if (pl.R == 0) return false;
  if (N * K * 4 > (int64_t{1} << 20) && M * K * 4 > (int64_t{128} << 20)) return false;
  return true;
}

int ebn_gemm_direct_launch(int32_t transB, int64_t M, int64_t N, int64_t K, float alpha, const float* A, int64_t lda, const float* B,
                           int64_t ldb, float* C, int64_t ldc, hipStream_t s) {
  if ((64 * lda + K) * 4 >= (int64_t{1} << 31) || ((transB ? N : K) * ldb + (transB ? K : N) + 16 * ldb) * 4 >= (int64_t{1} << 31)) return EBN_ERR_UNSUPPORTED;
  const DirectPlan pl = direct_plan(M, N, transB != 0);
  if (pl.R == 0 || ebn_ceil_div(pl.tasks, 4) >= (int64_t{1} << 31)) return EBN_ERR_UNSUPPORTED;
  const bool kc = transB != 0;
#define EBN_DIR_CASE(RR, CC) \
  if (pl.R == RR && pl.CW == CC) return direct_launch_rc<RR, CC>(kc, pl, M, N, K, alpha, A, lda, B, ldb, C, ldc, s)
  EBN_DIR_CASE(4, 7); EBN_DIR_CASE(3, 7); EBN_DIR_CASE(2, 7); EBN_DIR_CASE(1, 7);
  EBN_DIR_CASE(4, 5); EBN_DIR_CASE(3, 5); EBN_DIR_CASE(2, 5); EBN_DIR_CASE(1, 5);
  EBN_DIR_CASE(4, 4); EBN_DIR_CASE(3, 4); EBN_DIR_CASE(2, 4); EBN_DIR_CASE(1, 4);
#undef EBN_DIR_CASE
  return EBN_ERR_UNSUPPORTED;
}

int ebn_gemm_direct_tn_slices(int64_t M, int64_t N, int64_t K) {
  if (M < 48 || N < 48 || M > 512 || N > 1280 || K < 4096) return 0;
  return tn_direct_plan(M, N, K).Z;
}

int ebn_gemm_direct_tn_launch(int64_t M, int64_t N, int64_t K, float alpha, const float* A, int64_t lda, const float* B, int64_t ldb,
                              float* part, hipStream_t s) {
  const TnDirectPlan pl = tn_direct_plan(M, N, K);
  if (pl.Z < 2) return EBN_ERR_UNSUPPORTED;
  if ((pl.kps + 16) * (lda > ldb ? lda : ldb) * 4 >= (int64_t{1} << 31)) return EBN_ERR_UNSUPPORTED;
  const dim3 grid(static_cast<unsigned>(pl.tiles * pl.Z)), block(256);
#define EBN_TN_CASE(RR, CC)                                                                                                        \
  if (pl.R == RR && pl.CW == CC) {                                                                                                 \
    EBN_LAUNCH((gemm_direct16_tn_kernel<RR, CC>), grid, block, 0, s, M, N, K, alpha, A, lda, B, ldb, part, pl.G, pl.n_wide, pl.tiles, \
                       pl.kps);                                                                                                    \
    EBN_CHECK_LAUNCH();                                                                                                            \
    return EBN_OK;                                                                                                                 \
  }
  EBN_TN_CASE(5, 5) EBN_TN_CASE(4, 5) EBN_TN_CASE(3, 5) EBN_TN_CASE(5, 4) EBN_TN_CASE(4, 4) EBN_TN_CASE(3, 4)
#undef EBN_TN_CASE
  return EBN_ERR_UNSUPPORTED;
}
```

### ebnerd-benchmark_amd/ebrec/models/newsrec/_engine.py

```python
from __future__ import annotations

import ctypes
import math

import numpy as np
import torch

from ebrec import _hip

BETA1, BETA2, ADAM_EPS = 0.9, 0.999, 1e-7
_ALIGN = 64

from ._engine_segments import SegmentsMixin
from ._engine_staging import StagingMixin

LOSS_KIND = {"cross_entropy_loss": 0, "log_loss": 1}
BCE_ON = ("logits", "probs")


def loss_kind_of(loss: str, bce_on: str) -> int:
    if bce_on not in BCE_ON:
        raise ValueError(f"bce_on must be one of {BCE_ON}, got {bce_on}")
    return 0 if loss == "cross_entropy_loss" else (1 if bce_on == "logits" else 2)

# ... 2 lines not shown
    if not torch.cuda.is_available():
        raise RuntimeError("the MI355X NRMS path needs a visible GPU (no CPU fallback); "
                           "torch.cuda.is_available() is False")
    _hip.lib()
    return torch.device("cuda", torch.cuda.current_device())


def eval_loss_from_news(eng, news_all: torch.Tensor, his_idx, pred_idx, y):
    his_idx, pred_idx = np.asarray(his_idx), np.asarray(pred_idx)
    B, C = his_idx.shape[0], pred_idx.shape[1]
    H, E = his_idx.shape[1], eng.E
    idx = torch.from_numpy(np.ascontiguousarray(np.concatenate([his_idx.reshape(-1), pred_idx.reshape(-1)]), dtype=np.int32)).to(eng.device)
    NE = torch.empty(B * (H + C), E, device=eng.device)
    S = _hip.stream_handle
    _hip.call("ebn_gather_rows_f32", _hip.ptr(idx), _hip.ptr(news_all), _hip.ptr(NE), B * (H + C), E, news_all.shape[0], None, -1,
              ctypes.c_float(0.0), None, S())
    user = eng.encode_users_from_news(NE[: B * H].view(B, H, E))
    cand = NE[B * H:]
    scores, probs = torch.empty(B, C, device=eng.device), torch.empty(B, C, device=eng.device)
    _hip.call("ebn_score_fwd_f32", _hip.ptr(cand), _hip.ptr(user), _hip.ptr(scores), _hip.ptr(probs), B, C, E, 0, S())
    labels = (y if isinstance(y, torch.Tensor) else torch.from_numpy(np.ascontiguousarray(np.asarray(y, dtype=np.float32))))
    labels = labels.to(device=eng.device, dtype=torch.float32).reshape(B, C).contiguous()
    rows, junk_c, junk_u = torch.empty(B, device=eng.device), torch.empty(B * C, E, device=eng.device), torch.empty(B, E, device=eng.device)
    loss = torch.empty(1, device=eng.device)
    _hip.call("ebn_score_loss_bwd_f32", _hip.ptr(cand), _hip.ptr(user), _hip.ptr(scores), _hip.ptr(labels), _hip.ptr(rows),
              _hip.ptr(junk_c), _hip.ptr(junk_u), B, C, E, eng.loss_kind, ctypes.c_float(1.0 / B), S())
    _hip.call("ebn_sum_f32", _hip.ptr(rows), B, ctypes.c_float(1.0), _hip.ptr(loss), 0, S())
    return loss, probs


def glorot_uniform_np(shape, seed):
    rng = np.random.default_rng(seed)
    lim = math.sqrt(6.0 / (shape[0] + shape[-1]))
    return rng.uniform(-lim, lim, size=shape).astype(np.float32)


class FlatParams:

    def __init__(self, shapes: dict, device):
        self.shapes = dict(shapes)
        self.offsets = {}
        off = 0
        for name, shp in shapes.items():
            self.offsets[name] = off
            off += -(-int(np.prod(shp)) // _ALIGN) * _ALIGN
        self.numel = off
        self.data = torch.zeros(off, device=device)
        self.grad = torch.zeros(off, device=device)
        self.m = torch.zeros(off, device=device)
        self.v = torch.zeros(off, device=device)

    def view(self, name, buf=None):
        buf = self.data if buf is None else buf
        n = int(np.prod(self.shapes[name]))
        return buf[self.offsets[name]: self.offsets[name] + n].view(*self.shapes[name])

    def g(self, name):
        return self.view(name, self.grad)


class EncoderBuffers:

    def __init__(self, n_seq, L, Din, E, A, device, own_input, need_dx):
        R = n_seq * L
        self.n_seq, self.L, self.Din, self.E, self.A, self.R = n_seq, L, Din, E, A, R
        f = lambda *s: torch.empty(*s, device=device)
        self.X = f(R, Din) if own_input else None
        self.QKV, self.Y, self.U, self.w = f(R, 3 * E), f(R, E), f(R, A), f(R)
        self.out = f(n_seq, E)
        self.dY, self.dQKV, self.de = f(R, E), f(R, 3 * E), f(R)
        self.partials = f(int(_hip.lib().ebn_attpool_partials_len(R, A)))
        wsf = _hip.lib().ebn_gemm_workspace_floats
        ws = max(int(wsf(Din, 3 * E, R)), int(wsf(E, A, R)), int(wsf(R, 3 * E, Din)), int(wsf(R, A, E)), int(wsf(R, E, A)),
                 int(wsf(R, Din, 3 * E)), 1)
        self.ws = f(ws)
        self.fwd_scratch = _hip.EncoderScratch(None, None, None, None, self.ws.data_ptr(), self.ws.numel())
        self.dX = f(R, Din) if need_dx else None


class NRMSEngine(StagingMixin, SegmentsMixin):
    def __init__(self, table: np.ndarray, title_size: int, history_size: int, head_num: int, head_dim: int,
                 attention_hidden_dim: int, dropout: float, learning_rate: float, loss: str, seed=None,
                 train_embedding: bool = True, device=None, process_group=None, shard_table: bool = False,
                 shard_mode: str = "alltoall", deterministic: bool = True, units=None, l2: float = 0.0,
                 shard_partition: str | None = None, shard_capacity_factor: float = 1.25, table_grad_exchange: str = "auto",
                 bce_on: str = "logits", precision: str = "exact"):
        self.device = require_gpu() if device is None else torch.device(device)
        if precision not in ("exact", "split"):
            raise ValueError(f"precision must be 'exact' (fp32 MFMA, the default) or 'split' (bf16x6 split on the bf16 matrix pipe, "
                             f"fp32-accurate, fp32 accumulate), got {precision}")
        self.precision = precision
        if loss not in LOSS_KIND:
            raise ValueError(f"this loss not defined {loss}")
        loss_kind_of(loss, bce_on)
        self.bce_on = bce_on
        self.T, self.H = int(title_size), int(history_size)
        self.h, self.d, self.A = int(head_num), int(head_dim), int(attention_hidden_dim)
        self.E = self.h * self.d
        self.p = float(dropout)
        self.loss = loss
        self.seed = seed
        self.train_embedding = bool(train_embedding)
        if table_grad_exchange not in ("auto", "dense", "sparse"):
            raise ValueError(f"table_grad_exchange must be auto | dense | sparse, got {table_grad_exchange}")
        self.table_grad_exchange = table_grad_exchange
        self._sparse_pin = None
        self.pg = process_group
        table = np.ascontiguousarray(table, dtype=np.float32)
        self.V, self.D = table.shape
        self.exchange = None
        if shard_table:
            from ._dist import ShardedTableExchange

            self.exchange = ShardedTableExchange(self.V, self.D, group=process_group, mode=shard_mode, partition=shard_partition,
                                                 capacity_factor=shard_capacity_factor)
            table = self.exchange.shard_of(table)
        self.table = torch.from_numpy(np.ascontiguousarray(table)).to(self.device)
        D, E, A = self.D, self.E, self.A
        self.units = [int(u) for u in units] if units else []
        if self.units and self.precision == "split":
            raise ValueError("precision='split' covers the news encoder without the optional per-token Dense stack "
                             "(newsencoder_units_per_layer); use precision='exact' with it")
        if self.units and self.units[-1] != E:
            raise ValueError(f"newsencoder_units_per_layer must end with head_num*head_dim = {E} (the news vector is dotted with "
                             f"the {E}-wide user vector, nrms.py:201), got {self.units}")
        shapes = {"n_Wqkv": (D, 3 * E)}
        if self.units:
            from ._mlp import MLPStack

            shapes.update(MLPStack.shapes("n_", E, self.units))
        shapes.update({"n_W": (E, A), "n_b": (A,), "n_q": (A,), "u_Wqkv": (E, 3 * E), "u_W": (E, A), "u_b": (A,), "u_q": (A,)})
        self.params = FlatParams(shapes, self.device)
        self._graphs = {}
        self.mlp = MLPStack(self.params, "n_", E, self.units, self.device, l2, on_realloc=lambda: self._graphs.clear()) if self.units else None
        self._init_weights(seed)
        self.deterministic = bool(deterministic)
        if self.train_embedding:
            self.table_grad = torch.zeros_like(self.table)
            self.table_m = torch.zeros_like(self.table)
            self.table_v = torch.zeros_like(self.table)
            if self.deterministic:
                self.table_acc = torch.zeros(self.table.shape, dtype=torch.int64, device=self.device)
        st = _hip.StepState()
        st.step, st.seed, st.lr, st.adam_alpha = 0, (0 if seed is None else int(seed)) & 0xFFFFFFFF, learning_rate, 0.0
        self.state = torch.frombuffer(bytearray(bytes(st)), dtype=torch.uint8).to(self.device)
        self._lr = float(learning_rate)
        self._bufs = {}
        self.oob_flag = torch.zeros(1, dtype=torch.int32, device=self.device)
        self.keep_table_grad = False
        self.range_flag = torch.zeros(1, dtype=torch.int32, device=self.device)
        self.loss_dev = torch.zeros(1, device=self.device)
        self.use_graph = False
        self.fuse_user_head = True
        self.fuse_eval_gather = True
        self.defer_finish = True
        self.atomic_table_grad = False
        self.graph_collectives = False
        self.overlap_collectives = True
        self.skip_collectives = False
        self._pending = []
        self.defer_flag_checks = False
        self.trace = None
        self.world = 1
        if process_group is not None or (torch.distributed.is_available() and torch.distributed.is_initialized()):
            self.world = torch.distributed.get_world_size(process_group)
        self.guard = None
        if self.world > 1:
            from ._dist import LockStepGuard

            self.guard = LockStepGuard(process_group)
        self.force_collectives = False
        self.adam_in_finish = True
        self._adam_done_in_finish = False

    @property
    def multi(self) -> bool:
        return self.world > 1 or self.force_collectives

    @property
    def loss_kind(self) -> int:
        return loss_kind_of(self.loss, self.bce_on)

    def _init_weights(self, seed):
        D, E, A = self.D, self.E, self.A
        s = (lambda: seed) if seed is not None else (lambda: None)
        pv = self.params.view
        with torch.no_grad():
            for pre, din in (("n", D), ("u", E)):
                w = np.concatenate([glorot_uniform_np((din, E), s()) for _ in range(3)], axis=1)
                pv(f"{pre}_Wqkv").copy_(torch.from_numpy(w))
                pv(f"{pre}_W").copy_(torch.from_numpy(glorot_uniform_np((E, A), s())))
                pv(f"{pre}_b").zero_()
                pv(f"{pre}_q").copy_(torch.from_numpy(glorot_uniform_np((A, 1), s())[:, 0]))
        if self.mlp is not None:
            self.mlp.init_weights((lambda k: None) if seed is None else (lambda k: int(seed) * 1000 + k), glorot_uniform_np)

    def weight_names(self):
        base = ["news.emb", "news.attn.WQ", "news.attn.WK", "news.attn.WV"]
        if self.mlp is not None:
            base += self.mlp.weight_names("news")
        return base + ["news.att.W", "news.att.b", "news.att.q", "user.attn.WQ", "user.attn.WK", "user.attn.WV", "user.att.W",
                       "user.att.b", "user.att.q"]

    def get_weights(self):
        E = self.E
        out = [self._full_table().cpu().numpy()]
        for pre in ("n", "u"):
            w = self.params.view(f"{pre}_Wqkv").cpu().numpy()
            out += [w[:, :E].copy(), w[:, E:2 * E].copy(), w[:, 2 * E:].copy()]
            if pre == "n" and self.mlp is not None:
                out += self.mlp.get_weights()
            out += [self.params.view(f"{pre}_W").cpu().numpy(), self.params.view(f"{pre}_b").cpu().numpy(),
                    self.params.view(f"{pre}_q").cpu().numpy().reshape(-1, 1)]
        return out

    def set_weights(self, weights):
        n_mlp = 6 * len(self.units)
        if len(weights) != 13 + n_mlp:
            raise ValueError(f"expected {13 + n_mlp} weight arrays (emb, 2x[WQ,WK,WV,W,b,q]{' + 6 per Dense/BN layer' if n_mlp else ''}), "
                             f"got {len(weights)}")
        w = [np.asarray(a, dtype=np.float32) for a in weights]
        if n_mlp:
            self.mlp.set_weights([torch.from_numpy(np.ascontiguousarray(a)) for a in w[4:4 + n_mlp]])
            w = w[:4] + w[4 + n_mlp:]
        if w[0].shape != (self.V, self.D):
            raise ValueError(f"embedding shape {w[0].shape} != {(self.V, self.D)}")
        with torch.no_grad():
            t0 = w[0] if self.exchange is None else self.exchange.shard_of(w[0])
            self.table.copy_(torch.from_numpy(np.ascontiguousarray(t0)))
            i = 1
            for pre in ("n", "u"):
                self.params.view(f"{pre}_Wqkv").copy_(torch.from_numpy(np.concatenate(w[i:i + 3], axis=1)))
                self.params.view(f"{pre}_W").copy_(torch.from_numpy(w[i + 3]))
                self.params.view(f"{pre}_b").copy_(torch.from_numpy(w[i + 4].reshape(-1)))
                self.params.view(f"{pre}_q").copy_(torch.from_numpy(w[i + 5].reshape(-1)))
                i += 6

    def _full_table(self) -> torch.Tensor:
        if self.exchange is None or self.exchange.world == 1:
            return self.table
        per = self.exchange.per
        mine = torch.zeros(per, self.D, device=self.device)
        mine[: self.table.shape[0]] = self.table
        parts = [torch.empty_like(mine) for _ in range(self.exchange.world)]
        torch.distributed.all_gather(parts, mine, group=self.pg)
        return self.exchange.unshard(parts)

    def count_params(self):
        return self.V * self.D + sum(int(np.prod(s)) for s in self.params.shapes.values()) + 2 * sum(self.units)

    @property
    def _planned(self) -> bool:
        return self.exchange is not None and self.exchange.mode == "alltoall"

    @property
    def _adam_from_acc(self) -> bool:
        return (self.train_embedding and self.deterministic and self.exchange is None and not self.multi
                and not self.keep_table_grad)

    def _sparse_dp(self, n_tok: int) -> bool:
        if not (self.multi and self.train_embedding and self.exchange is None and self.deterministic and not self.keep_table_grad):
            return False
        if self.table_grad_exchange != "auto":
            return self.table_grad_exchange == "sparse"
        return self.pin_table_grad_exchange(n_tok)

    def pin_table_grad_exchange(self, n_tok_full: int) -> bool:
        if self._sparse_pin is None:
            self._sparse_pin = bool(self.world * int(n_tok_full) < self.V)
        return self._sparse_pin

    @property
    def needs_equal_batches(self) -> bool:
        if self.world <= 1:
            return False
        if self.exchange is not None:
            return True
        if not (self.train_embedding and self.deterministic and not self.keep_table_grad):
            return False
        if self.table_grad_exchange != "auto":
            return self.table_grad_exchange == "sparse"
        return True if self._sparse_pin is None else self._sparse_pin

    @property
    def graph_capable(self) -> bool:
        return self.exchange is None or self._planned

    def allreduce_bytes(self, n_tok: int = 0) -> int:
        n = self.params.numel * 4
        if self.train_embedding and self.exchange is None:
            n += n_tok * (4 + self.D * 4) if self._sparse_dp(n_tok) else self.table_grad.numel() * 4
        return n

    def enable_graphs(self, flag=True):
        self.use_graph = bool(flag)
        if not flag:
            self._graphs = {}
        return self

    @property
    def learning_rate(self):
        return self._lr

    @learning_rate.setter
    def learning_rate(self, lr):
        self._lr = float(lr)
        st = self.read_state()
        st.lr = self._lr
        self.state.copy_(torch.frombuffer(bytearray(bytes(st)), dtype=torch.uint8))

    def read_state(self):
        return _hip.StepState.from_buffer_copy(self.state.cpu().numpy().tobytes())

    def _news_bufs(self, N, train):
        key = ("news", train)
        b = self._bufs.get(key)
        if b is None or b.n_seq < N:
            b = EncoderBuffers(N, self.T, self.D, self.E, self.A, self.device, own_input=True,
                               need_dx=train and self.train_embedding)
            b.ids = torch.empty(N * self.T, dtype=torch.int32, device=self.device)
            if self._planned:
                from ._dist import PlannedBuffers

                ws = int(_hip.lib().ebn_shard_plan_workspace_ints(self.V, self.exchange.world))
                b.xb = PlannedBuffers(self.exchange, N * self.T, self.device, need_grad=train and self.train_embedding, ws_ints=ws)
            self._bufs[key] = b
            if train:
                self._graphs.clear()
        return b

    def _user_bufs(self, B, train, H=None):
        H = self.H if H is None else int(H)
        key = ("user", train) if H == self.H else ("user", train, H)
        b = self._bufs.get(key)
        if b is None or b.n_seq < B:
            b = EncoderBuffers(B, H, self.E, self.E, self.A, self.device, own_input=False, need_dx=False)
            self._bufs[key] = b
            if train and H == self.H:
                self._graphs.clear()
        return b

    def _enc_structs(self, pre, b: EncoderBuffers, n_seq, X, drop_site, drop_p):
        pv = self.params.view
        dims = _hip.EncoderDims(n_seq, b.L, b.Din, self.h, self.d, self.A, drop_site, drop_p)
        params = _hip.EncoderParams(pv(f"{pre}_Wqkv").data_ptr(), pv(f"{pre}_W").data_ptr(),
                                    pv(f"{pre}_b").data_ptr(), pv(f"{pre}_q").data_ptr())
        acts = _hip.EncoderActs(X.data_ptr(), b.QKV.data_ptr(), b.Y.data_ptr(), b.U.data_ptr(), b.w.data_ptr(),
                                b.out.data_ptr())
        return dims, params, acts

    def _encoder_fwd(self, pre, b, n_seq, X, train, n_first=None):
        site, p = (1, self.p) if (train and pre == "n" and self.p > 0) else (-1, 0.0)
        st = _hip.ptr(self.state) if train else None
        if pre == "n" and self.mlp is not None:
            return self._news_encoder_fwd_mlp(b, n_seq, X, train, n_seq if n_first is None else n_first)
        if pre == "n" and self.precision == "split":
            return self._news_encoder_fwd_split(b, n_seq, X, st, site, p)
        dims, params, acts = self._enc_structs(pre, b, n_seq, X, site, p)
        _hip.call("ebn_encoder_fwd_f32", ctypes.byref(dims), ctypes.byref(params), ctypes.byref(acts),
                  ctypes.byref(self._fwd_scratch(b)), st, _hip.stream_handle())

    @staticmethod
    def _fwd_scratch(b):
        return b.fwd_scratch

    def _news_encoder_fwd_mlp(self, b, n_seq, X, train, n_first):
        S, E, A, T = _hip.stream_handle, self.E, self.A, b.L
        R = n_seq * T
        pv = self.params.view
        _hip.call("ebn_gemm_f32_site", 0, 0, R, 3 * E, b.Din, ctypes.c_float(1.0), _hip.ptr(X), b.Din, _hip.ptr(pv("n_Wqkv")), 3 * E,
                  ctypes.c_float(0.0), _hip.ptr(b.QKV), 3 * E, _hip.ptr(b.ws), b.ws.numel(), 1, S())
        _hip.call("ebn_attn_fwd_f32", _hip.ptr(b.QKV), 3 * E, _hip.ptr(b.Y), E, n_seq, T, self.h, self.d, None, -1, ctypes.c_float(0.0), S())
        b.Z = self.mlp.forward(b.Y, n_first * T, (n_seq - n_first) * T, train, self.state, self.p)
        _hip.call("ebn_gemm_f32_ws", 0, 0, R, A, E, ctypes.c_float(1.0), _hip.ptr(b.Z), E, _hip.ptr(pv("n_W")), A, ctypes.c_float(0.0),
                  _hip.ptr(b.U), A, _hip.ptr(b.ws), b.ws.numel(), S())
        _hip.call("ebn_attpool_fwd_f32", _hip.ptr(b.U), _hip.ptr(pv("n_b")), _hip.ptr(pv("n_q")), _hip.ptr(b.Z), _hip.ptr(b.out),
                  _hip.ptr(b.w), n_seq, T, E, A, S())

    def _news_encoder_bwd_mlp(self, b, n_seq, X, dout, dX, n_first):
        S, E, A, T = _hip.stream_handle, self.E, self.A, b.L
        R = n_seq * T
        pv, g = self.params.view, self.params.g
        ws, wsn = _hip.ptr(b.ws), b.ws.numel()
        one, zero = ctypes.c_float(1.0), ctypes.c_float(0.0)
        _hip.call("ebn_attpool_bwd_pool_f32", _hip.ptr(b.Z), _hip.ptr(b.w), _hip.ptr(dout), _hip.ptr(b.dY), _hip.ptr(b.de), n_seq, T, E, S())
        _hip.call("ebn_attpool_bwd_dpre_f32", _hip.ptr(b.U), _hip.ptr(pv("n_q")), _hip.ptr(b.de), _hip.ptr(g("n_q")), _hip.ptr(g("n_b")),
                  _hip.ptr(b.partials), R, A, 0, S())
        _hip.call("ebn_gemm_f32_ws", 1, 0, E, A, R, one, _hip.ptr(b.Z), E, _hip.ptr(b.U), A, zero, _hip.ptr(g("n_W")), A, ws, wsn, S())
        _hip.call("ebn_gemm_f32_ws", 0, 1, R, E, A, one, _hip.ptr(b.U), A, _hip.ptr(pv("n_W")), A, one, _hip.ptr(b.dY), E, ws, wsn, S())
        dYattn = self.mlp.backward(b.dY, b.Y, n_first * T, (n_seq - n_first) * T, self.state, self.p, need_dx0=True,
                                   loss_dev=self.loss_dev)
        _hip.call("ebn_attn_bwd_f32", _hip.ptr(b.QKV), 3 * E, _hip.ptr(dYattn), E, _hip.ptr(b.dQKV), 3 * E, n_seq, T, self.h, self.d,
                  None, -1, ctypes.c_float(0.0), S())
        _hip.call("ebn_gemm_f32_ws", 1, 0, b.Din, 3 * E, R, one, _hip.ptr(X), b.Din, _hip.ptr(b.dQKV), 3 * E, zero, _hip.ptr(g("n_Wqkv")),
                  3 * E, ws, wsn, S())
        if dX is not None:
            _hip.call("ebn_gemm_f32_ws", 0, 1, R, b.Din, 3 * E, one, _hip.ptr(b.dQKV), 3 * E, _hip.ptr(pv("n_Wqkv")), 3 * E, zero,
                      _hip.ptr(dX), b.Din, ws, wsn, S())

    def _split_ws(self, b):
        if getattr(b, "split_ws", None) is None:
            f = _hip.lib().ebn_gemm_prec_workspace_bytes
            R, E3, D = b.R, 3 * b.E, b.Din
            nbytes = max(int(f(R, E3, D, 1)), int(f(D, E3, R, 1)), int(f(R, D, E3, 1)) if b.dX is not None else 0)
            b.split_ws = torch.empty(nbytes // 4 + 64, device=self.device)
            b.split_ws_bytes = nbytes
        return b.split_ws

    def _split_bufs(self, b):
        sb = getattr(b, "split_bufs", None)
        if sb is None:
            L = _hip.lib()
            R, E3, D = b.R, 3 * b.E, b.Din
            u8 = lambda n: torch.empty(int(n) + 64, dtype=torch.uint8, device=self.device)
            sb = b.split_bufs = {"XN": u8(L.ebn_planes_bytes(R, D)), "XT": u8(L.ebn_planes_bytes(D, R)), "Wp": u8(L.ebn_planes_bytes(E3, D)),
                                 "dQp": u8(L.ebn_planes_bytes(E3, R)),
                                 "part": torch.empty(max(int(L.ebn_gemm_planes_workspace_floats(D, E3, R)), int(L.ebn_gemm_planes_workspace_floats(R, E3, D)), 1),
                                                     device=self.device)}
        return sb

    def _gemm_prec(self, b, tA, tB, M, N, K, A, lda, Bm, ldb, C, ldc):
        ws = self._split_ws(b)
        _hip.call("ebn_gemm_f32_prec", tA, tB, M, N, K, ctypes.c_float(1.0), _hip.ptr(A), lda, _hip.ptr(Bm), ldb, ctypes.c_float(0.0),
                  _hip.ptr(C), ldc, _hip.ptr(ws), b.split_ws_bytes, 1, _hip.stream_handle())

    def _news_encoder_fwd_split_gemm(self, b, R):
        S, E = _hip.stream_handle, self.E
        sb = self._split_bufs(b)
        _hip.call("ebn_split_planes_f32", _hip.ptr(self.params.view("n_Wqkv")), 3 * E, 3 * E, b.Din, 1, _hip.ptr(sb["Wp"]), S())
        _hip.call("ebn_gemm_planes_f32", _hip.ptr(sb["XN"]), R, _hip.ptr(sb["Wp"]), 3 * E, b.Din, ctypes.c_float(1.0), ctypes.c_float(0.0),
                  _hip.ptr(b.QKV), 3 * E, _hip.ptr(sb["part"]), sb["part"].numel(), S())

    def _news_encoder_fwd_split(self, b, n_seq, X, st, site, p):
        S, E, A, T = _hip.stream_handle, self.E, self.A, b.L
        R = n_seq * T
        pv = self.params.view
        if getattr(b, "planes_rows", -1) == R:
            self._news_encoder_fwd_split_gemm(b, R)
        else:
            self._gemm_prec(b, 0, 0, R, 3 * E, b.Din, X, b.Din, pv("n_Wqkv"), 3 * E, b.QKV, 3 * E)
        _hip.call("ebn_attn_fwd_f32", _hip.ptr(b.QKV), 3 * E, _hip.ptr(b.Y), E, n_seq, T, self.h, self.d, st, site, ctypes.c_float(p), S())
        _hip.call("ebn_gemm_f32_ws", 0, 0, R, A, E, ctypes.c_float(1.0), _hip.ptr(b.Y), E, _hip.ptr(pv("n_W")), A, ctypes.c_float(0.0),
                  _hip.ptr(b.U), A, _hip.ptr(b.ws), b.ws.numel(), S())
        _hip.call("ebn_attpool_fwd_f32", _hip.ptr(b.U), _hip.ptr(pv("n_b")), _hip.ptr(pv("n_q")), _hip.ptr(b.Y), _hip.ptr(b.out),
                  _hip.ptr(b.w), n_seq, T, E, A, S())

    def _news_encoder_bwd_split(self, b, n_seq, X, dout, dX, site, p):
        self._news_bwd_p1(b, n_seq, dout)
        self._news_bwd_p2(b, n_seq, X, dout, site, p)
        if dX is not None:
            self._news_bwd_p3(b, n_seq, dX)

    def _news_bwd_p1(self, b, n_seq, dout):
        S, E, A, T = _hip.stream_handle, self.E, self.A, b.L
        R = n_seq * T
        pv, g = self.params.view, self.params.g
        ws, wsn = _hip.ptr(b.ws), b.ws.numel()
        one, zero = ctypes.c_float(1.0), ctypes.c_float(0.0)
        _hip.call("ebn_attpool_bwd_pool_f32", _hip.ptr(b.Y), _hip.ptr(b.w), _hip.ptr(dout), None, _hip.ptr(b.de), n_seq, T, E, S())
        _hip.call("ebn_attpool_bwd_dpre_f32", _hip.ptr(b.U), _hip.ptr(pv("n_q")), _hip.ptr(b.de), _hip.ptr(g("n_q")), _hip.ptr(g("n_b")),
                  _hip.ptr(b.partials), R, A, 0, S())
        if self._fold_pooling(T):
            _hip.call("ebn_dense_bwd_pair_f32", R, E, A, _hip.ptr(b.Y), E, _hip.ptr(b.U), A, _hip.ptr(pv("n_W")), A, zero, _hip.ptr(g("n_W")), A,
                      _hip.ptr(b.dY), E, ws, wsn, S())
        else:
            _hip.call("ebn_gemm_f32_ws", 1, 0, E, A, R, one, _hip.ptr(b.Y), E, _hip.ptr(b.U), A, zero, _hip.ptr(g("n_W")), A, ws, wsn, S())
            _hip.call("ebn_gemm_f32_rank1", R, E, A, one, _hip.ptr(b.U), A, _hip.ptr(pv("n_W")), A, _hip.ptr(b.dY), E, _hip.ptr(b.w), _hip.ptr(dout), E,
                      T, ws, wsn, S())

    def _fold_pooling(self, T) -> bool:
        return int(_hip.lib().ebn_attn_bwd_pooled_supported(T, self.d)) != 0 and self.E % 4 == 0

    def _news_bwd_p2(self, b, n_seq, X, dout, site, p):
        S, E, T = _hip.stream_handle, self.E, b.L
        R = n_seq * T
        g = self.params.g
        st = _hip.ptr(self.state)
        one, zero = ctypes.c_float(1.0), ctypes.c_float(0.0)
        if self._fold_pooling(T):
            _hip.call("ebn_attn_bwd_pooled_f32", _hip.ptr(b.QKV), 3 * E, _hip.ptr(b.dY), E, _hip.ptr(b.w), _hip.ptr(dout), E, _hip.ptr(b.dQKV), 3 * E,
                      n_seq, T, self.h, self.d, st, site, ctypes.c_float(p), S())
        else:
            _hip.call("ebn_attn_bwd_f32", _hip.ptr(b.QKV), 3 * E, _hip.ptr(b.dY), E, _hip.ptr(b.dQKV), 3 * E, n_seq, T, self.h, self.d, st, site,
                      ctypes.c_float(p), S())
        if self.precision != "split":
            _hip.call("ebn_gemm_f32_ws", 1, 0, b.Din, 3 * E, R, one, _hip.ptr(X), b.Din, _hip.ptr(b.dQKV), 3 * E, zero, _hip.ptr(g("n_Wqkv")), 3 * E,
                      _hip.ptr(b.ws), b.ws.numel(), S())
        elif getattr(b, "planes_rows", -1) == R:
            sb = self._split_bufs(b)
            _hip.call("ebn_split_planes_f32", _hip.ptr(b.dQKV), 3 * E, 3 * E, R, 1, _hip.ptr(sb["dQp"]), S())
            _hip.call("ebn_gemm_planes_f32", _hip.ptr(sb["XT"]), b.Din, _hip.ptr(sb["dQp"]), 3 * E, R, one, zero, _hip.ptr(g("n_Wqkv")), 3 * E,
                      _hip.ptr(sb["part"]), sb["part"].numel(), S())
        else:
            self._gemm_prec(b, 1, 0, b.Din, 3 * E, R, X, b.Din, b.dQKV, 3 * E, g("n_Wqkv"), 3 * E)

    def _news_bwd_p3(self, b, n_seq, dX):
        E, R = self.E, n_seq * b.L
        pv = self.params.view
        if self.precision != "split":
            _hip.call("ebn_gemm_f32_ws", 0, 1, R, b.Din, 3 * E, ctypes.c_float(1.0), _hip.ptr(b.dQKV), 3 * E, _hip.ptr(pv("n_Wqkv")), 3 * E,
                      ctypes.c_float(0.0), _hip.ptr(dX), b.Din, _hip.ptr(b.ws), b.ws.numel(), _hip.stream_handle())
        else:
            self._gemm_prec(b, 0, 1, R, b.Din, 3 * E, b.dQKV, 3 * E, pv("n_Wqkv"), 3 * E, dX, b.Din)

    def roofline_kernels(self, B, C):
        N = B * (self.H + C)
        nb, _ub = self._train_bufs(B, C)
        S, E, R = _hip.stream_handle, self.E, N * self.T
        pv = self.params.view
        site, p = (0, self.p) if self.p > 0 else (-1, 0.0)
        st = _hip.ptr(self.state)

        def qkv_gemm():
            if self.precision == "split":
                nb.planes_rows = R
                return self._news_encoder_fwd_split_gemm(nb, R)
            _hip.call("ebn_gemm_f32_site", 0, 0, R, 3 * E, nb.Din, ctypes.c_float(1.0), _hip.ptr(nb.X), nb.Din,
                      _hip.ptr(pv("n_Wqkv")), 3 * E, ctypes.c_float(0.0), _hip.ptr(nb.QKV), 3 * E, _hip.ptr(nb.ws), nb.ws.numel(), 1, S())

        def make_gather(ids):
            table_rows = self.table.shape[0]
            src = ids if table_rows == self.V else torch.remainder(ids, table_rows).to(torch.int32)

            def gather():
                self._gather_tokens(nb, src, self.table, table_rows, R, st, site, p, True)

            return gather

        return {"qkv_gemm": qkv_gemm, "gather": make_gather}

    def _encoder_bwd(self, pre, b, n_seq, X, dout, dX, n_first=None):
        if pre == "n" and self.mlp is not None:
            return self._news_encoder_bwd_mlp(b, n_seq, X, dout, dX, n_seq if n_first is None else n_first)
        site, p = (1, self.p) if (pre == "n" and self.p > 0) else (-1, 0.0)
        if pre == "n" and self.precision == "split":
            return self._news_encoder_bwd_split(b, n_seq, X, dout, dX, site, p)
        dims, params, acts = self._enc_structs(pre, b, n_seq, X, site, p)
        g = self.params.g
        grads = _hip.EncoderGrads(g(f"{pre}_Wqkv").data_ptr(), g(f"{pre}_W").data_ptr(), g(f"{pre}_b").data_ptr(),
                                  g(f"{pre}_q").data_ptr())
        scratch = _hip.EncoderScratch(b.dY.data_ptr(), b.dQKV.data_ptr(), b.de.data_ptr(), b.partials.data_ptr(),
                                      b.ws.data_ptr(), b.ws.numel())
        _hip.call("ebn_encoder_bwd_f32", ctypes.byref(dims), ctypes.byref(params), ctypes.byref(acts), _hip.ptr(dout),
                  ctypes.byref(grads), ctypes.byref(scratch), _hip.ptr(dX), 0, _hip.ptr(self.state),
                  _hip.stream_handle())

    def _news_forward(self, b, N, train, n_first=None, looked_up=False):
        site, p = (0, self.p) if (train and self.p > 0) else (-1, 0.0)
        st = _hip.ptr(self.state) if train else None
        n_tok = N * self.T
        if self._planned:
            if not looked_up:
                for _kind, fn in self._lookup_segments(b, N):
                    fn()
            xb = b.xb
            self._gather_tokens(b, xb.inv, xb.rows, self.exchange.world * self.exchange.capacity(n_tok), n_tok, st, site, p, train)
            return self._encoder_fwd("n", b, N, b.X, train, n_first)
        if self.exchange is not None:
            b.plan = self.exchange.plan(b.ids[: n_tok])
            b.rows_uniq = self.exchange.lookup(b.plan, self._local_gather)
            self._gather_tokens(b, b.plan.inv, b.rows_uniq, b.rows_uniq.shape[0], n_tok, st, site, p, train)
            return self._encoder_fwd("n", b, N, b.X, train, n_first)
        if not train and self.fuse_eval_gather and self.mlp is None and self.precision == "exact":
            dims, params, acts = self._enc_structs("n", b, N, b.X, -1, 0.0)
            rc = _hip.lib().ebn_encoder_fwd_gather_f32(ctypes.byref(dims), ctypes.byref(params), ctypes.byref(acts), ctypes.byref(self._fwd_scratch(b)),
                                                       _hip.ptr(b.ids), _hip.ptr(self.table), self.V, _hip.ptr(self.oob_flag), _hip.stream_handle())
            if rc == 0:
                return
            if rc != -2:
                raise _hip.HipError(f"ebn_encoder_fwd_gather_f32 failed with code {rc}")
        self._gather_tokens(b, b.ids, self.table, self.V, n_tok, st, site, p, train)
        self._encoder_fwd("n", b, N, b.X, train, n_first)

    def _gather_tokens(self, b, ids, table, table_rows, n_tok, st, site, p, train):
        if self.precision == "split" and train and self.mlp is None and n_tok <= b.R:
            sb = self._split_bufs(b)
            _hip.call("ebn_gather_split_planes_f32", _hip.ptr(ids), _hip.ptr(table), n_tok, self.D, table_rows, st, site, ctypes.c_float(p),
                      _hip.ptr(self.oob_flag), _hip.ptr(sb["XN"]), _hip.ptr(sb["XT"]), _hip.stream_handle())
            b.planes_rows = n_tok
            return
        b.planes_rows = -1
        _hip.call("ebn_gather_rows_f32", _hip.ptr(ids), _hip.ptr(table), _hip.ptr(b.X), n_tok, self.D, table_rows, st, site,
                  ctypes.c_float(p), _hip.ptr(self.oob_flag), _hip.stream_handle())

    def encode_news(self, ids, chunk=8192) -> torch.Tensor:
        ids = ids if isinstance(ids, torch.Tensor) else np.asarray(ids)
        N = ids.shape[0]
        if ids.ndim != 2 or ids.shape[1] != self.T:
            raise ValueError(f"expected ids of shape (N, {self.T}), got {tuple(ids.shape)}")
        out = torch.empty(N, self.E, device=self.device)
        for s in range(0, N, chunk):
            n = min(chunk, N - s)
            b = self._news_bufs(min(chunk, N), False)
            self._upload_ids(b.ids, ids[s:s + n])
# ... 121 lines not shown
                          _hip.stream_handle())
                y, advanced = None, True
            elif not isinstance(his, torch.Tensor) and not isinstance(pred, torch.Tensor) and not isinstance(y, torch.Tensor):
                for a in (his, pred):
                    if a.size and (a.min() < 0 or a.max() >= self.V):
                        raise IndexError(f"token id out of range [0, {self.V}) for the embedding table")
                self._stage_host([his, pred], nb.ids, y, nb.labels)
                y, advanced = None, True
            else:
                self._upload_ids(nb.ids, his, pred)
        if y is not None:
            labels = (y if isinstance(y, torch.Tensor) else torch.from_numpy(np.ascontiguousarray(np.asarray(y, dtype=np.float32))))
            nb.labels[: B * C].copy_(labels.reshape(-1).to(device=self.device, dtype=torch.float32), non_blocking=True)
        if self.use_graph and self.graph_capable:
            key = self._graph_key(B, C, advanced)
            run = self._graphs.get(key)
            if run is None:
                run = self._capture(B, C, advanced)
            if self.trace is not None:
                self.trace.run(run, self._graph_desc.get(key, []))
            else:
                for fn in run:
                    fn()
        elif self.trace is not None:
            segs = self._segments(B, C, advanced)
            self.trace.run([fn for _kind, fn in segs], [self.SEG_KINDS.get(kind, kind) + (f": {fn.what}" if hasattr(fn, "what") else "") for kind, fn in segs])
        else:
            for _kind, fn in self._segments(B, C, advanced):
                fn()
        if return_probs:
            return self.loss_dev, nb.probs[: B * C].view(B, C), nb.labels[: B * C].view(B, C)
        return self.loss_dev

    def _train_bufs(self, B, C):
        N, E = B * (self.H + C), self.E
        nb = self._news_bufs(N, True)
        ub = self._user_bufs(B, True)
        if not hasattr(nb, "dNE"):
            nb.dNE = torch.empty(nb.n_seq, E, device=self.device)
            nb.scores = torch.empty(nb.n_seq, device=self.device)
            nb.probs = torch.empty(nb.n_seq, device=self.device)
            nb.labels = torch.empty(nb.n_seq, device=self.device)
        if self._deferred(C):
            self._defer_bufs(nb)
        if not hasattr(ub, "duser"):
            ub.duser = torch.empty(ub.n_seq, E, device=self.device)
            ub.loss_rows = torch.empty(ub.n_seq, device=self.device)
            ub.head_partials = torch.empty(max(int(_hip.lib().ebn_user_head_partials_len(ub.n_seq, self.A)), 1), device=self.device)
        return nb, ub

    SEG_KINDS = {"k": "kernels", "c": "collective", "a": "collective started asynchronously", "w": "wait for the started collectives"}

    def _fwd_bwd_kernels(self, B, C, sparse_table_grads=False, part="all"):
        H, E = self.H, self.E
        N = B * (H + C)
        S = _hip.stream_handle
        nb, ub = self._train_bufs(B, C)
        st = _hip.ptr(self.state)
        site1, p1 = (1, self.p) if self.p > 0 else (-1, 0.0)
        deferred = self._deferred(C)
        if part in ("all", "a"):
            self._adam_done_in_finish = False
        if part == "b":
            if deferred:
                return self._news_bwd_deferred(nb, ub, B, N, "p2")
            return self._news_bwd_p2(nb, N, nb.X, nb.dNE, site1, p1)
        if part in ("all", "a"):
            if deferred:
                self._news_forward(nb, N, True, B * H, looked_up=True)
                self._user_stage_deferred(B, C, nb, ub)
            else:
                self._fwd_user_stage_kernels(B, C, nb, ub)
        if part == "a":
            if deferred:
                return self._news_bwd_deferred(nb, ub, B, N, "p1")
            return self._news_bwd_p1(nb, N, nb.dNE)
        if part == "all" and deferred:
            self._news_bwd_deferred(nb, ub, B, N, "p1")
            self._adam_done_in_finish = self._adam_fused(C)
            if self._adam_done_in_finish:
                self._news_bwd_deferred(nb, ub, B, N, "p2a")
                if nb.dX is not None:
                    self._news_bwd_p3(nb, N, nb.dX)
                self._news_bwd_deferred(nb, ub, B, N, "p2b")
            else:
                self._news_bwd_deferred(nb, ub, B, N, "p2")
                if nb.dX is not None:
                    self._news_bwd_p3(nb, N, nb.dX)
        elif part == "all":
            self._encoder_bwd("n", nb, N, nb.X, nb.dNE, nb.dX, B * H)
        elif nb.dX is not None:
            self._news_bwd_p3(nb, N, nb.dX)
        self._table_grad_kernels(nb, N, sparse_table_grads)

    def _deferred(self, C) -> bool:
        L = _hip.lib()
        return bool(self.defer_finish and self.mlp is None and self.precision == "exact" and self.fuse_user_head
                    and self._fold_pooling(self.T) and self._fold_pooling(self.H)
                    and int(L.ebn_user_head_supported(self.H, C, self.E, self.A)) != 0)

    def _adam_fused(self, C) -> bool:
        return bool(self.adam_in_finish and not self.multi and self._deferred(C))

    def _adam_flat_args(self):
        a = getattr(self, "_adam_flat", None)
        if a is None:
            P = self.params
            a = _hip.AdamFlat()
            a.theta, a.grad, a.m, a.v, a.numel = P.data.data_ptr(), P.grad.data_ptr(), P.m.data_ptr(), P.v.data_ptr(), P.numel
            a.beta1, a.beta2, a.eps, a.grad_scale = BETA1, BETA2, ADAM_EPS, 1.0
            rest = sorted((P.offsets[k], int(np.prod(P.shapes[k]))) for k in ("u_Wqkv", "u_W"))
            a.n_rest = len(rest)
            for i, (off, n) in enumerate(rest):
                a.rest_off[i], a.rest_len[i] = off, n
            self._adam_flat = a
        return a

    def _defer_bufs(self, nb):
        if getattr(nb, "ws_dw", None) is None:
            L = _hip.lib()
            nb.ws_dw = torch.empty(max(int(L.ebn_gemm_partials_workspace_floats(self.E, self.A, nb.R)), 1), device=self.device)
            nb.ws_dwqkv = torch.empty(max(int(L.ebn_gemm_partials_workspace_floats(self.D, 3 * self.E, nb.R)), 1), device=self.device)
            nb.finish_jobs = {}
        return nb

    def _user_stage_deferred(self, B, C, nb, ub):
        S, H, E, A = _hip.stream_handle, self.H, self.E, self.A
        R = B * H
        pv, g = self.params.view, self.params.g
        ws, wsn = _hip.ptr(ub.ws), ub.ws.numel()
        one, zero = ctypes.c_float(1.0), ctypes.c_float(0.0)
        X, cand, dcand = nb.out, nb.out[B * H:], nb.dNE[B * H:]
        _hip.call("ebn_gemm_f32_site", 0, 0, R, 3 * E, E, one, _hip.ptr(X), E, _hip.ptr(pv("u_Wqkv")), 3 * E, zero, _hip.ptr(ub.QKV), 3 * E, ws, wsn, 1, S())
        _hip.call("ebn_attn_fwd_f32", _hip.ptr(ub.QKV), 3 * E, _hip.ptr(ub.Y), E, B, H, self.h, self.d, None, -1, zero, S())
        _hip.call("ebn_gemm_f32_ws", 0, 0, R, A, E, one, _hip.ptr(ub.Y), E, _hip.ptr(pv("u_W")), A, zero, _hip.ptr(ub.U), A, ws, wsn, S())
        _hip.call("ebn_user_head_train_f32", _hip.ptr(ub.U), _hip.ptr(pv("u_b")), _hip.ptr(pv("u_q")), _hip.ptr(ub.Y), _hip.ptr(cand), _hip.ptr(nb.labels),
                  _hip.ptr(ub.w), _hip.ptr(ub.out), _hip.ptr(nb.scores), _hip.ptr(nb.probs), _hip.ptr(ub.loss_rows), _hip.ptr(self.loss_dev), _hip.ptr(dcand),
                  _hip.ptr(ub.duser), _hip.ptr(ub.de), None, None, _hip.ptr(ub.head_partials), B, H, C, E, A, self.loss_kind, ctypes.c_float(1.0 / B), S())
        _hip.call("ebn_dense_bwd_pair_f32", R, E, A, _hip.ptr(ub.Y), E, _hip.ptr(ub.U), A, _hip.ptr(pv("u_W")), A, zero, _hip.ptr(g("u_W")), A,
                  _hip.ptr(ub.dY), E, ws, wsn, S())
        _hip.call("ebn_attn_bwd_pooled_f32", _hip.ptr(ub.QKV), 3 * E, _hip.ptr(ub.dY), E, _hip.ptr(ub.w), _hip.ptr(ub.duser), E, _hip.ptr(ub.dQKV), 3 * E,
                  B, H, self.h, self.d, None, -1, zero, S())
        _hip.call("ebn_dense_bwd_pair_f32", R, E, 3 * E, _hip.ptr(X), E, _hip.ptr(ub.dQKV), 3 * E, _hip.ptr(pv("u_Wqkv")), 3 * E, zero, _hip.ptr(g("u_Wqkv")),
                  3 * E, _hip.ptr(nb.dNE), E, ws, wsn, S())

    def _news_bwd_deferred(self, nb, ub, B, N, part):
        S, E, A, T, D = _hip.stream_handle, self.E, self.A, self.T, self.D
        R = N * T
        pv, g = self.params.view, self.params.g
        one, zero = ctypes.c_float(1.0), ctypes.c_float(0.0)
        L = _hip.lib()
        self._defer_bufs(nb)
        if part == "p1":
            _hip.call("ebn_attpool_bwd_pool_f32", _hip.ptr(nb.Y), _hip.ptr(nb.w), _hip.ptr(nb.dNE), None, _hip.ptr(nb.de), N, T, E, S())
            _hip.call("ebn_attpool_bwd_dpre_f32", _hip.ptr(nb.U), _hip.ptr(pv("n_q")), _hip.ptr(nb.de), None, None, _hip.ptr(nb.partials), R, A, 0, S())
            n = ctypes.c_int32(0)
            _hip.call("ebn_gemm_f32_partials", 1, 0, E, A, R, one, _hip.ptr(nb.Y), E, _hip.ptr(nb.U), A, _hip.ptr(nb.ws_dw), nb.ws_dw.numel(), ctypes.byref(n), S())
            nb.finish_jobs["dW"] = int(n.value)
            _hip.call("ebn_gemm_f32_ws", 0, 1, R, E, A, one, _hip.ptr(nb.U), A, _hip.ptr(pv("n_W")), A, zero, _hip.ptr(nb.dY), E, _hip.ptr(nb.ws), nb.ws.numel(), S())
            return
        site, p = (1, self.p) if self.p > 0 else (-1, 0.0)
        if part in ("p2", "p2a"):
            _hip.call("ebn_attn_bwd_pooled_f32", _hip.ptr(nb.QKV), 3 * E, _hip.ptr(nb.dY), E, _hip.ptr(nb.w), _hip.ptr(nb.dNE), E, _hip.ptr(nb.dQKV), 3 * E,
                      N, T, self.h, self.d, _hip.ptr(self.state), site, ctypes.c_float(p), S())
            n = ctypes.c_int32(0)
            _hip.call("ebn_gemm_f32_partials", 1, 0, D, 3 * E, R, one, _hip.ptr(nb.X), D, _hip.ptr(nb.dQKV), 3 * E, _hip.ptr(nb.ws_dwqkv), nb.ws_dwqkv.numel(),
                      ctypes.byref(n), S())
            nb.finish_jobs["dWqkv"] = int(n.value)
            if part == "p2a":
                return
        jobs = (_hip.FinishJob * 4)()
        jobs[0] = _hip.FinishJob(_hip.FINISH_COLRED, int(L.ebn_attpool_partials_len(R, A)) // (2 * A), 1, A, nb.partials.data_ptr(), g("n_q").data_ptr(),
                                 g("n_b").data_ptr(), A, 0.0, 1.0, None, None)
        jobs[1] = _hip.FinishJob(_hip.FINISH_HEAD, 1, B, A, ub.head_partials.data_ptr(), g("u_q").data_ptr(), g("u_b").data_ptr(), A, 0.0, 1.0,
                                 ub.loss_rows.data_ptr(), self.loss_dev.data_ptr())
        jobs[2] = _hip.FinishJob(_hip.FINISH_SPLITK, nb.finish_jobs["dW"], E, A, nb.ws_dw.data_ptr(), g("n_W").data_ptr(), None, A, 0.0, 1.0, None, None)
        jobs[3] = _hip.FinishJob(_hip.FINISH_SPLITK, nb.finish_jobs["dWqkv"], D, 3 * E, nb.ws_dwqkv.data_ptr(), g("n_Wqkv").data_ptr(), None, 3 * E, 0.0, 1.0, None, None)
        if part == "p2b":
            _hip.call("ebn_grad_finish_adam_f32", jobs, 4, ctypes.byref(self._adam_flat_args()), _hip.ptr(self.state), S())
        else:
            _hip.call("ebn_grad_finish_f32", jobs, 4, S())

    def _fwd_user_stage_kernels(self, B, C, nb, ub):
        H, E = self.H, self.E
        N = B * (H + C)
        S = _hip.stream_handle
        st = _hip.ptr(self.state)
        self._news_forward(nb, N, True, B * H, looked_up=True)
        cand, dcand = nb.out[B * H:], nb.dNE[B * H:]
        dims, params, acts = self._enc_structs("u", ub, B, nb.out, -1, 0.0)
        g = self.params.g
        grads = _hip.EncoderGrads(g("u_Wqkv").data_ptr(), g("u_W").data_ptr(), g("u_b").data_ptr(), g("u_q").data_ptr())
        scratch = _hip.EncoderScratch(ub.dY.data_ptr(), ub.dQKV.data_ptr(), ub.de.data_ptr(), ub.partials.data_ptr(),
                                      ub.ws.data_ptr(), ub.ws.numel())
        _hip.call("ebn_user_stage_train_f32", ctypes.byref(dims), ctypes.byref(params), ctypes.byref(acts), _hip.ptr(cand),
                  _hip.ptr(nb.labels), _hip.ptr(nb.scores), _hip.ptr(nb.probs), _hip.ptr(ub.loss_rows), _hip.ptr(self.loss_dev),
                  _hip.ptr(dcand), _hip.ptr(ub.duser), ctypes.byref(grads), ctypes.byref(scratch),
                  _hip.ptr(ub.head_partials) if self.fuse_user_head else None, _hip.ptr(nb.dNE), C, self.loss_kind,
                  ctypes.c_float(1.0 / B), st, S())

    def _accumulate_fixed(self, ids, dX, n_tok, st, site, p):
        _hip.call("ebn_embedding_grad_scatter_fixed_atomic" if self.atomic_table_grad else "ebn_embedding_grad_scatter_fixed", _hip.ptr(ids),
                  _hip.ptr(dX), _hip.ptr(self.table_acc), n_tok, self.D, self.V, st, site, ctypes.c_float(p), _hip.ptr(self.range_flag),
                  _hip.stream_handle())

    def _table_grad_kernels(self, nb, N, sparse_table_grads):
        S = _hip.stream_handle
        st = _hip.ptr(self.state)
        if self.train_embedding and not self._planned and not sparse_table_grads:
            if self.exchange is not None or not self.deterministic:
                self.table_grad.zero_()
            site, p = (0, self.p) if self.p > 0 else (-1, 0.0)
            if self.exchange is not None:
                d_uniq = torch.zeros_like(nb.rows_uniq)
                _hip.call("ebn_embedding_grad_scatter_f32", _hip.ptr(nb.plan.inv), _hip.ptr(nb.dX), _hip.ptr(d_uniq),
                          N * self.T, self.D, d_uniq.shape[0], st, site, ctypes.c_float(p), S())
                self.exchange.scatter_grads(nb.plan, d_uniq, self._local_scatter_add)
            elif self.deterministic:
                self._accumulate_fixed(nb.ids, nb.dX, N * self.T, st, site, p)
                if not self._adam_from_acc:
                    _hip.call("ebn_fixed_to_f32", _hip.ptr(self.table_acc), _hip.ptr(self.table_grad), self.table.numel(),
                              _hip.ptr(self.range_flag), S())
            else:
                _hip.call("ebn_embedding_grad_scatter_f32", _hip.ptr(nb.ids), _hip.ptr(nb.dX), _hip.ptr(self.table_grad),
                          N * self.T, self.D, self.V, st, site, ctypes.c_float(p), S())

    def _optimizer_kernels(self, from_acc=None):
        from_acc = self._adam_from_acc if from_acc is None else from_acc
        S = _hip.stream_handle
        st = _hip.ptr(self.state)
        gs = ctypes.c_float(1.0 / self.world)
        P = self.params
        if not self._adam_done_in_finish:
            _hip.call("ebn_adam_keras_step_f32", _hip.ptr(P.data), _hip.ptr(P.grad), _hip.ptr(P.m), _hip.ptr(P.v), P.numel,
                      st, BETA1, BETA2, ADAM_EPS, gs, S())
        if self.train_embedding and from_acc:
            _hip.call("ebn_adam_keras_step_fixed_f32", _hip.ptr(self.table), _hip.ptr(self.table_acc), _hip.ptr(self.table_m),
                      _hip.ptr(self.table_v), self.table.numel(), st, BETA1, BETA2, ADAM_EPS, gs, _hip.ptr(self.range_flag), S())
        elif self.train_embedding:
            _hip.call("ebn_adam_keras_step_f32", _hip.ptr(self.table), _hip.ptr(self.table_grad), _hip.ptr(self.table_m),
                      _hip.ptr(self.table_v), self.table.numel(), st, BETA1, BETA2, ADAM_EPS, gs, S())
```

### ebnerd-benchmark_amd/ebrec/models/newsrec/_engine_segments.py

```python
from __future__ import annotations

import ctypes

import numpy as np
import torch

from ebrec import _hip

BETA1, BETA2, ADAM_EPS = 0.9, 0.999, 1e-7


def _named(kind, fn, what):
    fn.what = what
    return kind, fn


class SegmentsMixin:
    def _lookup_segments(self, b, N):
        ex, n_tok = self.exchange, N * self.T

        def plan(ids, n, cap, ws, slot_rows, inv, counts):
            _hip.call("ebn_shard_plan_i32", _hip.ptr(ids), n, self.V, ex.world, 1 if ex.cyclic else 0, cap, _hip.ptr(ws),
                      _hip.ptr(slot_rows), _hip.ptr(inv), _hip.ptr(counts), _hip.stream_handle())

        def serve(local_rows, out):
            _hip.call("ebn_gather_rows_f32", _hip.ptr(local_rows), _hip.ptr(self.table), _hip.ptr(out), local_rows.numel(), self.D,
                      self.table.shape[0], None, -1, ctypes.c_float(0.0), None, _hip.stream_handle())

        return ex.lookup_segments(b.ids, n_tok, b.xb, plan, serve)

    def _table_grad_segments(self, b, N):
        ex, n_tok = self.exchange, N * self.T
        site, p = (0, self.p) if self.p > 0 else (-1, 0.0)

        def reduce_local(inv, d_slot):
            d_slot.zero_()
            _hip.call("ebn_embedding_grad_scatter_f32", _hip.ptr(inv), _hip.ptr(b.dX), _hip.ptr(d_slot), n_tok, self.D,
                      d_slot.shape[0], _hip.ptr(self.state), site, ctypes.c_float(p), _hip.stream_handle())

        def accumulate(local_rows, grads):
            self.table_grad.zero_()
            _hip.call("ebn_embedding_grad_scatter_f32", _hip.ptr(local_rows), _hip.ptr(grads), _hip.ptr(self.table_grad),
                      local_rows.numel(), self.D, self.table.shape[0], None, -1, ctypes.c_float(0.0), _hip.stream_handle())

        return ex.grad_segments(n_tok, b.xb, reduce_local, accumulate)

    def _local_gather(self, local_rows: torch.Tensor) -> torch.Tensor:
        m = local_rows.numel()
        out = torch.empty(m, self.D, device=self.device)
        if m:
            _hip.call("ebn_gather_rows_f32", _hip.ptr(local_rows), _hip.ptr(self.table), _hip.ptr(out), m, self.D,
                      self.table.shape[0], None, -1, ctypes.c_float(0.0), _hip.ptr(self.oob_flag), _hip.stream_handle())
        return out

    def _local_scatter_add(self, local_rows: torch.Tensor, grads: torch.Tensor) -> None:
        m = local_rows.numel()
        if m:
            _hip.call("ebn_embedding_grad_scatter_f32", _hip.ptr(local_rows), _hip.ptr(grads), _hip.ptr(self.table_grad),
                      m, self.D, self.table.shape[0], None, -1, ctypes.c_float(0.0), _hip.stream_handle())

    def _state_tensors(self):
        ts = [self.params.data, self.params.grad, self.params.m, self.params.v, self.state, self.loss_dev]
        if self.train_embedding:
            ts += [self.table, self.table_grad, self.table_m, self.table_v] + ([self.table_acc] if self.deterministic else [])
        return ts

    def verify_graph_collectives(self, his, pred, y) -> bool:
        if not (self.use_graph and self.graph_capable and self.multi):
            self.graph_collectives = False
            return False
        if torch.distributed.get_backend(self.pg) != "nccl":
            self.graph_collectives = False
            return False
        torch.cuda.synchronize()
        snap = [t.clone() for t in self._state_tensors()]

        def restore():
            for t, s in zip(self._state_tensors(), snap):
                t.copy_(s)

        def one_step(flag):
            self.graph_collectives = flag
            self._graphs.clear()
            self.train_step(his, pred, y)
            restore()
            self.train_step(his, pred, y)
            torch.cuda.synchronize()
            out = [t.clone() for t in self._state_tensors()]
            restore()
            return out

        ok = True
        try:
            ref = one_step(False)
            got = one_step(True)
            ok = all(torch.equal(a, b) for a, b in zip(ref, got))
        except Exception:
            ok = False
            restore()
        verdict = torch.tensor([1 if ok else 0], dtype=torch.int32, device=self.device)
        torch.distributed.all_reduce(verdict, op=torch.distributed.ReduceOp.MIN, group=self.pg)
        self.graph_collectives = bool(int(verdict.item()))
        self._graphs.clear()
        return self.graph_collectives

    def _graph_key(self, B, C, advanced=False):
        return (B, C, advanced, bool(self.adam_in_finish), bool(self.defer_finish), bool(self.multi))

    def _capture(self, B, C, advanced=False):
        torch.cuda.synchronize()
        key = self._graph_key(B, C, advanced)
        segs, run, pool, i = self._segments(B, C, advanced), [], None, 0
        desc = self.__dict__.setdefault("_graph_desc", {}).setdefault(key, [])
        desc.clear()
        if self.graph_collectives and self.multi:
            g = torch.cuda.CUDAGraph()
            with _hip.capture(g):
                for _kind, fn in segs:
                    fn()
            self._graph_objs = getattr(self, "_graph_objs", []) + [g]
            self._graphs[key] = [g.replay]
            desc.append("ONE hipGraph: " + " | ".join(self.SEG_KINDS[k] for k, _fn in segs))
            return self._graphs[key]
        while i < len(segs):
            if segs[i][0] != "k":
                run.append(segs[i][1])
                desc.append(f"{self.SEG_KINDS[segs[i][0]]}: {getattr(segs[i][1], 'what', 'unnamed')} (segment {i} of the step's {len(segs)})")
                i += 1
                continue
            j = i
            while j < len(segs) and segs[j][0] == "k":
                j += 1
            g = torch.cuda.CUDAGraph()
            with _hip.capture(g, pool=pool):
                for _kind, fn in segs[i:j]:
                    fn()
            pool = pool or g.pool()
            run.append(g.replay)
            desc.append(f"hipGraph replay of kernel segments {i}..{j - 1} of the step's {len(segs)}")
            self._graph_objs = getattr(self, "_graph_objs", []) + [g]
            i = j
        self._graphs[key] = run
        return run

    def _segments(self, B, C, advanced=False):
        N = B * (self.H + C)
        nb, _ub = self._train_bufs(B, C)
        multi = self.multi
        segs = [] if advanced else [("k", lambda: _hip.call("ebn_step_advance", _hip.ptr(self.state), BETA1, BETA2, _hip.stream_handle()))]
        if self._planned:
            segs += self._lookup_segments(nb, N)
        sparse = self._sparse_dp(N * self.T)
        if multi and self.mlp is None and self.overlap_collectives and self.train_embedding:
            segs.append(("k", lambda: (self._fwd_bwd_kernels(B, C, sparse, part="a"), self._fwd_bwd_kernels(B, C, sparse, part="b"))))
            segs.append(_named("a", lambda: self._allreduce_async(self.params.grad), "all-reduce of the flat dense-gradient bucket"))
            segs.append(("k", lambda: self._fwd_bwd_kernels(B, C, sparse, part="c")))
            if self._planned:
                segs += self._table_grad_segments(nb, N)
            if self.exchange is None and not sparse:
                segs.append(_named("c", lambda: self._allreduce_table_grad(), "all-reduce of the dense (V, D) table gradient"))
            if sparse:
                segs += self._sparse_table_grad_segments(nb, N)
            segs.append(("w", self._wait_collectives))
        else:
            segs.append(("k", lambda: self._fwd_bwd_kernels(B, C, sparse)))
            if self._planned and self.train_embedding:
                segs += self._table_grad_segments(nb, N)
            if multi:
                segs.append(_named("c", lambda: self._allreduce_grads(dense_table=not sparse),
                                   "all-reduce of the flat dense-gradient bucket" + (" and of the dense table gradient" if (self.train_embedding and self.exchange is None and not sparse) else "")))
            if sparse:
                segs += self._sparse_table_grad_segments(nb, N)
        segs.append(("k", lambda: self._optimizer_kernels(from_acc=self._adam_from_acc or sparse)))
        return segs

    def _allreduce_async(self, t):
        if self.multi and not self.skip_collectives:
            self._pending.append(torch.distributed.all_reduce(t, group=self.pg, async_op=True))

    def _wait_collectives(self):
        for w in self._pending:
            w.wait()
        self._pending = []

    def _allreduce_table_grad(self):
        if self.multi and not self.skip_collectives:
            torch.distributed.all_reduce(self.table_grad, group=self.pg)

    def _sparse_table_grad_segments(self, nb, N):
        n_tok, W = N * self.T, self.world
        if getattr(nb, "ids_all", None) is None or nb.ids_all.numel() < W * n_tok:
            nb.ids_all = torch.empty(W * nb.n_seq * self.T, dtype=torch.int32, device=self.device)
            nb.dX_all = torch.empty(W * nb.n_seq * self.T, self.D, device=self.device)
        ids_all, dX_all = nb.ids_all[: W * n_tok], nb.dX_all[: W * n_tok]
        site, p = (0, self.p) if self.p > 0 else (-1, 0.0)

        def gather():
            if self.skip_collectives:
                return
            torch.distributed.all_gather_into_tensor(ids_all, nb.ids[:n_tok], group=self.pg)
            torch.distributed.all_gather_into_tensor(dX_all, nb.dX[:n_tok], group=self.pg)

        def accumulate():
            for r in range(W):
                self._accumulate_fixed(ids_all[r * n_tok:], dX_all[r * n_tok:], n_tok, _hip.ptr(self.state), site, p)

        return [_named("c", gather, "all-gather of the per-token (id, gradient row) pairs (sparse table-gradient exchange)"), ("k", accumulate)]

    def _allreduce_grads(self, dense_table=True):
        if self.multi and not self.skip_collectives:
            torch.distributed.all_reduce(self.params.grad, group=self.pg)
            if self.train_embedding and self.exchange is None and dense_table:
                torch.distributed.all_reduce(self.table_grad, group=self.pg)
```

### include/ebnerd_hip.h

```cpp
#ifndef EBNERD_HIP_H
#define EBNERD_HIP_H

#include <stdint.h>

#ifdef __cplusplus
extern "C" {
#endif

#define EBN_ABI_VERSION 1

#define EBN_OK 0
#define EBN_ERR_BAD_ARG (-1)
#define EBN_ERR_UNSUPPORTED (-2)
#define EBN_ERR_ALIGN (-3)

typedef void* ebn_stream_t;

#define EBN_SITE_NEWS_IN 0
#define EBN_SITE_NEWS_ATT 1
#define EBN_SITE_MLP0 8
#define EBN_N_SITES 12

typedef struct ebn_step_state {
  uint32_t step;
  uint32_t seed;
  float adam_alpha;
  float lr;
  uint32_t drop_key[EBN_N_SITES];
} ebn_step_state;

int ebn_abi_version(void);
const char* ebn_error_string(int code);
int64_t ebn_launch_count(void);

int ebn_step_advance(ebn_step_state* st, double beta1, double beta2, ebn_stream_t stream);

int ebn_gather_rows_f32(const int32_t* ids, const float* table, float* out, int64_t n_tok,
                        int32_t D, int64_t V, const ebn_step_state* st, int32_t site,
                        float drop_p, int32_t* oob_flag, ebn_stream_t stream);

int ebn_expand_titles_i32(const int32_t* art_idx, const int32_t* token_matrix, int32_t* ids_out,
                          int64_t n_titles, int32_t T, int64_t n_rows, int32_t* oob_flag,
                          ebn_stream_t stream);

int ebn_embedding_grad_scatter_f32(const int32_t* ids, const float* dX, float* dTable,
                                   int64_t n_tok, int32_t D, int64_t V,
                                   const ebn_step_state* st, int32_t site, float drop_p,
                                   ebn_stream_t stream);

int ebn_embedding_grad_scatter_fixed(const int32_t* ids, const float* dX, int64_t* acc, int64_t n_tok,
                                     int32_t D, int64_t V, const ebn_step_state* st, int32_t site,
                                     float drop_p, int32_t* range_flag, ebn_stream_t stream);
int ebn_embedding_grad_scatter_fixed_atomic(const int32_t* ids, const float* dX, int64_t* acc, int64_t n_tok,
                                            int32_t D, int64_t V, const ebn_step_state* st, int32_t site,
                                            float drop_p, int32_t* range_flag, ebn_stream_t stream);
int ebn_fixed_to_f32(int64_t* acc, float* out, int64_t n, int32_t* range_flag, ebn_stream_t stream);
int ebn_adam_keras_step_fixed_f32(float* theta, int64_t* acc, float* m, float* v, int64_t n, const ebn_step_state* st,
                                  double beta1, double beta2, double eps, float grad_scale, int32_t* range_flag,
                                  ebn_stream_t stream);

int64_t ebn_gemm_split_workspace_bytes(int64_t M, int64_t N, int64_t K);
int ebn_gemm_f32_split(int32_t transA, int32_t transB, int64_t M, int64_t N, int64_t K, float alpha, const float* A,
                       int64_t lda, const float* B, int64_t ldb, float beta, float* C, int64_t ldc, void* workspace,
                       int64_t workspace_bytes, ebn_stream_t stream);
int64_t ebn_planes_bytes(int64_t rows, int64_t K);
int ebn_split_planes_f32(const float* src, int64_t ld, int64_t rows, int64_t K, int32_t trans, void* planes,
                         ebn_stream_t stream);
int ebn_gather_split_planes_f32(const int32_t* ids, const float* table, int64_t n_rows, int32_t D, int64_t V,
                                const ebn_step_state* st, int32_t site, float drop_p, int32_t* oob_flag, void* planes_n,
                                void* planes_t, ebn_stream_t stream);
int64_t ebn_gemm_planes_workspace_floats(int64_t M, int64_t N, int64_t K);
int ebn_gemm_planes_f32(const void* a_planes, int64_t M, const void* b_planes, int64_t N, int64_t K, float alpha, float beta,
                        float* C, int64_t ldc, float* workspace, int64_t workspace_floats, ebn_stream_t stream);
int64_t ebn_gemm_prec_workspace_bytes(int64_t M, int64_t N, int64_t K, int32_t precision);
int ebn_gemm_f32_prec(int32_t transA, int32_t transB, int64_t M, int64_t N, int64_t K, float alpha, const float* A,
                      int64_t lda, const float* B, int64_t ldb, float beta, float* C, int64_t ldc, void* workspace,
                      int64_t workspace_bytes, int32_t precision, ebn_stream_t stream);

int64_t ebn_shard_plan_workspace_ints(int64_t V, int32_t world);
int ebn_shard_plan_i32(const int32_t* ids, int64_t n_tok, int64_t V, int32_t world, int32_t cyclic, int64_t cap,
                       int32_t* workspace, int32_t* slot_rows, int32_t* inv, int32_t* counts, ebn_stream_t stream);

int ebn_gemm_f32(int32_t transA, int32_t transB, int64_t M, int64_t N, int64_t K, float alpha,
                 const float* A, int64_t lda, const float* B, int64_t ldb, float beta, float* C,
                 int64_t ldc, ebn_stream_t stream);
int64_t ebn_gemm_workspace_floats(int64_t M, int64_t N, int64_t K);
int ebn_gemm_plan(int64_t M, int64_t N, int64_t K, int64_t workspace_floats, int32_t* bm, int32_t* bn, int32_t* splits);
int ebn_gemm_f32_ws(int32_t transA, int32_t transB, int64_t M, int64_t N, int64_t K, float alpha,
                    const float* A, int64_t lda, const float* B, int64_t ldb, float beta, float* C,
                    int64_t ldc, float* workspace, int64_t workspace_floats, ebn_stream_t stream);

int64_t ebn_gemm_partials_workspace_floats(int64_t M, int64_t N, int64_t K);
int ebn_gemm_f32_partials(int32_t transA, int32_t transB, int64_t M, int64_t N, int64_t K, float alpha, const float* A,
                          int64_t lda, const float* B, int64_t ldb, float* workspace, int64_t workspace_floats,
                          int32_t* n_parts, ebn_stream_t stream);

#define EBN_FINISH_SPLITK 0
#define EBN_FINISH_COLRED 1
#define EBN_FINISH_HEAD 2
#define EBN_FINISH_MAX_JOBS 6
typedef struct {
  int32_t kind;
  int32_t n_parts;
  int64_t rows, cols;
  const float* partials;
  float* out0;
  float* out1;
  int64_t ld;
  float beta, scale;
  const float* loss_rows;
  float* loss_out;
} ebn_finish_job;
int ebn_grad_finish_f32(const ebn_finish_job* jobs, int32_t n_jobs, ebn_stream_t stream);

#define EBN_ADAM_FLAT_MAX_REST 12
typedef struct ebn_adam_flat {
  float* theta;
  const float* grad;
  float* m;
  float* v;
  int64_t numel;
  double beta1, beta2, eps;
  float grad_scale;
  int32_t n_rest;
  int64_t rest_off[EBN_ADAM_FLAT_MAX_REST];
  int64_t rest_len[EBN_ADAM_FLAT_MAX_REST];
} ebn_adam_flat;
int ebn_grad_finish_adam_f32(const ebn_finish_job* jobs, int32_t n_jobs, const ebn_adam_flat* adam, const ebn_step_state* st,
                             ebn_stream_t stream);

int ebn_gemm_f32_site(int32_t transA, int32_t transB, int64_t M, int64_t N, int64_t K, float alpha,
                      const float* A, int64_t lda, const float* B, int64_t ldb, float beta, float* C,
                      int64_t ldc, float* workspace, int64_t workspace_floats, int32_t site,
                      ebn_stream_t stream);

int ebn_attn_fwd_f32(const float* qkv, int64_t ld_qkv, float* out, int64_t ld_out, int64_t n_seq,
                     int32_t L, int32_t h, int32_t d, const ebn_step_state* st, int32_t site,
                     float drop_p, ebn_stream_t stream);
int ebn_attn_bwd_f32(const float* qkv, int64_t ld_qkv, const float* dout, int64_t ld_dout,
                     float* dqkv, int64_t ld_dqkv, int64_t n_seq, int32_t L, int32_t h, int32_t d,
                     const ebn_step_state* st, int32_t site, float drop_p, ebn_stream_t stream);
int ebn_attn_bwd_pooled_f32(const float* qkv, int64_t ld_qkv, const float* dout, int64_t ld_dout, const float* pool_w,
                            const float* pool_dout, int64_t ld_pool, float* dqkv, int64_t ld_dqkv, int64_t n_seq,
                            int32_t L, int32_t h, int32_t d, const ebn_step_state* st, int32_t site, float drop_p,
                            ebn_stream_t stream);
int ebn_attn_bwd_pooled_supported(int32_t L, int32_t d);

int ebn_gemm_f32_rank1(int64_t M, int64_t N, int64_t K, float alpha, const float* A, int64_t lda, const float* B,
                       int64_t ldb, float* C, int64_t ldc, const float* row_scale, const float* seq_rows,
                       int64_t ld_seq, int32_t L, float* workspace, int64_t workspace_floats, ebn_stream_t stream);

int ebn_dense_bwd_pair_f32(int64_t R, int64_t K_in, int64_t N_out, const float* X, int64_t ldx, const float* dY,
                           int64_t lddy, const float* W, int64_t ldw, float beta_w, float* dW, int64_t lddw, float* dX,
                           int64_t lddx, float* workspace, int64_t workspace_floats, ebn_stream_t stream);

int ebn_dense_relu_fwd_f32(int64_t M, int64_t N, int64_t K, const float* A, int64_t lda, const float* B, int64_t ldb,
                           const float* bias, float* C, int64_t ldc, float* workspace, int64_t workspace_floats,
                           ebn_stream_t stream);

int ebn_attpool_fwd_f32(float* U, const float* b, const float* q, const float* X, float* out,
                        float* w, int64_t n_seq, int32_t L, int32_t E, int32_t A,
                        ebn_stream_t stream);
int ebn_attpool_bwd_pool_f32(const float* X, const float* w, const float* dout, float* dX,
                             float* de, int64_t n_seq, int32_t L, int32_t E,
                             ebn_stream_t stream);
int64_t ebn_attpool_partials_len(int64_t R, int32_t A);
int ebn_attpool_bwd_dpre_f32(float* U, const float* q, const float* de, float* dq, float* db,
                             float* partials, int64_t R, int32_t A, int32_t accumulate,
                             ebn_stream_t stream);
typedef struct ebn_encoder_dims {
  int64_t n_seq;
  int32_t L;
  int32_t Din;
  int32_t h, d;
  int32_t A;
  int32_t drop_site;
  float drop_p;
} ebn_encoder_dims;

typedef struct ebn_encoder_params {
  const float* Wqkv;
  const float* W;
  const float* b;
  const float* q;
} ebn_encoder_params;

typedef struct ebn_encoder_acts {
  const float* X;
  float* QKV;
  float* Y;
  float* U;
  float* w;
  float* out;
} ebn_encoder_acts;

typedef struct ebn_encoder_grads {
  float* dWqkv;
  float* dW;
  float* db;
  float* dq;
} ebn_encoder_grads;

typedef struct ebn_encoder_scratch {
  float* dY;
  float* dQKV;
  float* de;
  float* partials;
  float* gemm_ws;
  int64_t gemm_ws_floats;
} ebn_encoder_scratch;

int ebn_encoder_fwd_f32(const ebn_encoder_dims* dims, const ebn_encoder_params* params,
                        const ebn_encoder_acts* acts, const ebn_encoder_scratch* scratch,
                        const ebn_step_state* st, ebn_stream_t stream);
int ebn_encoder_fwd_gather_f32(const ebn_encoder_dims* dims, const ebn_encoder_params* params, const ebn_encoder_acts* acts,
                               const ebn_encoder_scratch* scratch, const int32_t* ids, const float* table, int64_t table_rows,
                               int32_t* oob_flag, ebn_stream_t stream);
int ebn_gemm_f32_rowmap(const int32_t* ids, int64_t table_rows, int64_t M, int64_t N, int64_t K, const float* table,
                        int64_t ldt, const float* B, int64_t ldb, float* C, int64_t ldc, int32_t* oob_flag, ebn_stream_t stream);

int ebn_encoder_bwd_f32(const ebn_encoder_dims* dims, const ebn_encoder_params* params,
                        const ebn_encoder_acts* acts, const float* dout,
                        const ebn_encoder_grads* grads, const ebn_encoder_scratch* scratch,
                        float* dX, int32_t accumulate, const ebn_step_state* st,
                        ebn_stream_t stream);

int ebn_user_stage_train_f32(const ebn_encoder_dims* dims, const ebn_encoder_params* p, const ebn_encoder_acts* a,
                             const float* cand, const float* labels, float* scores, float* probs, float* loss_rows,
                             float* loss_out, float* dcand, float* duser, const ebn_encoder_grads* g,
                             const ebn_encoder_scratch* s, float* head_partials, float* dX, int32_t C, int32_t loss_kind,
                             float inv_batch, const ebn_step_state* st, ebn_stream_t stream);

int ebn_score_fwd_f32(const float* cand, const float* user, float* scores, float* probs,
                      int64_t B, int32_t C, int32_t E, int32_t mode, ebn_stream_t stream);
int ebn_score_loss_bwd_f32(const float* cand, const float* user, const float* scores,
                           const float* labels, float* loss_rows, float* dcand, float* duser,
                           int64_t B, int32_t C, int32_t E, int32_t loss_kind, float inv_batch,
                           ebn_stream_t stream);
int ebn_score_loss_train_f32(const float* cand, const float* user, const float* labels, float* scores, float* probs,
                             float* loss_rows, float* loss_out, float* dcand, float* duser, int64_t B, int32_t C,
                             int32_t E, int32_t loss_kind, float inv_batch, ebn_stream_t stream);
int ebn_user_head_supported(int32_t L, int32_t C, int32_t E, int32_t A);
int64_t ebn_user_head_partials_len(int64_t B, int32_t A);
int ebn_user_head_train_f32(float* U, const float* b, const float* q, const float* X, const float* cand, const float* labels,
                            float* w, float* user, float* scores, float* probs, float* loss_rows, float* loss_out,
                            float* dcand, float* duser, float* de, float* dq, float* db, float* partials, int64_t B,
                            int32_t L, int32_t C, int32_t E, int32_t A, int32_t loss_kind, float inv_batch,
                            ebn_stream_t stream);
int ebn_auc_hist_f32(const float* probs, const float* labels, int64_t n, const double* thresholds, int32_t n_thresholds,
                     int64_t* pos_hist, int64_t* neg_hist, ebn_stream_t stream);
int ebn_pair_score_f32(const float* user, const float* news, const int32_t* u_idx,
                       const int32_t* n_idx, float* out, int64_t n_pairs, int32_t E, int32_t mode,
                       ebn_stream_t stream);

int ebn_adam_keras_step_f32(float* theta, const float* g, float* m, float* v, int64_t n,
                            const ebn_step_state* st, double beta1, double beta2, double eps,
                            float grad_scale, ebn_stream_t stream);

int ebn_bias_relu_f32(const float* X, const float* bias, float* Y, int64_t R, int32_t Ccols,
                      ebn_stream_t stream);
int64_t ebn_colsum_partials_len(int64_t R, int32_t Ccols);
int ebn_bias_relu_bwd_f32(const float* Y, const float* dY, float* dX, float* dbias,
                          float* partials, int64_t R, int32_t Ccols, int32_t accumulate,
                          ebn_stream_t stream);
int ebn_batchnorm_fwd_f32(const float* X, const float* gamma, const float* beta,
                          float* moving_mean, float* moving_var, float* Y, float* xhat,
                          float* mean_out, float* istd_out, float* partials, int64_t R,
                          int32_t Ccols, int32_t training, const ebn_step_state* st,
                          int32_t site, float drop_p, int64_t elem_offset,
                          ebn_stream_t stream);
int ebn_batchnorm_bwd_f32(const float* dY, const float* xhat, const float* gamma,
                          const float* istd, float* dX, float* dgamma, float* dbeta,
                          float* partials, int64_t R, int32_t Ccols, int32_t training,
                          int32_t accumulate, const ebn_step_state* st, int32_t site,
                          float drop_p, int64_t elem_offset, ebn_stream_t stream);
int ebn_batchnorm2_fwd_f32(const float* X, const float* gamma, const float* beta, float* moving_mean, float* moving_var,
                           float* Y, float* xhat, float* mean_out0, float* istd_out0, float* mean_out1, float* istd_out1,
                           int64_t R0, int64_t R1, int32_t Ccols, const ebn_step_state* st, int32_t site, float drop_p,
                           ebn_stream_t stream);
int ebn_batchnorm2_relu_bwd_f32(const float* dY, const float* xhat, const float* relu_out, const float* gamma,
                                const float* istd0, const float* istd1, float* dX, float* dgamma, float* dbeta,
                                float* dbias, int64_t R0, int64_t R1, int32_t Ccols, const ebn_step_state* st, int32_t site,
                                float drop_p, ebn_stream_t stream);

#define EBN_DVN_MAX_LAYERS 4
typedef struct ebn_dvn_args {
  int32_t n_layers, din, e_out;
  int32_t units[EBN_DVN_MAX_LAYERS];
  int32_t n0, n1;
  float drop_p, l2;
  const float* W[EBN_DVN_MAX_LAYERS + 1];
  const float* b[EBN_DVN_MAX_LAYERS + 1];
  const float* gamma[EBN_DVN_MAX_LAYERS];
  const float* beta[EBN_DVN_MAX_LAYERS];
  float* moving_mean[EBN_DVN_MAX_LAYERS];
  float* moving_var[EBN_DVN_MAX_LAYERS];
  const float* X0;
  float* R[EBN_DVN_MAX_LAYERS];
  float* Xn[EBN_DVN_MAX_LAYERS];
  float* NE;
  float* stat;
  const float* dNE;
  float* dY[EBN_DVN_MAX_LAYERS];
  float* dP[EBN_DVN_MAX_LAYERS + 1];
  float* ggamma[EBN_DVN_MAX_LAYERS];
  float* gbeta[EBN_DVN_MAX_LAYERS];
  float* loss;
  int32_t* range_flag;
} ebn_dvn_args;
int ebn_dvn_supported(const ebn_dvn_args* args);
int64_t ebn_dvn_stat_floats(const ebn_dvn_args* args);
int ebn_dvn_fwd_train_f32(const ebn_dvn_args* args, const ebn_step_state* st, ebn_stream_t stream);
int ebn_dvn_bwd_f32(const ebn_dvn_args* args, const ebn_step_state* st, ebn_stream_t stream);

int ebn_docvec_stage_gather_f32(const int32_t* idx0, int64_t n0, const int32_t* idx1, int64_t n1, const float* labels_src,
                                float* labels_dst, int64_t n_labels, const float* matrix, int64_t n_rows, int32_t din, float* X0,
                                int32_t* oob_flag, ebn_step_state* st, double beta1, double beta2, ebn_stream_t stream);

#define EBN_TN_GROUP_MAX 8
typedef struct ebn_tn_problem {
  int64_t M, N, K;
  const float* A;
  int64_t lda;
  const float* B;
  int64_t ldb;
  float* C;
  int64_t ldc;
  float* colsum;
  const float* l2_W;
  float two_lambda;
} ebn_tn_problem;
int ebn_gemm_tn_group_f32(const ebn_tn_problem* problems, int32_t n, ebn_stream_t stream);

#define EBN_DVN_FINALE_MAX_REST 12
typedef struct ebn_dvn_finale {
  float* theta;
  const float* grad;
  float* m;
  float* v;
  int64_t numel;
  double beta1, beta2, eps;
  float grad_scale;
  int32_t n_rest;
  int64_t rest_off[EBN_DVN_FINALE_MAX_REST];
  int64_t rest_len[EBN_DVN_FINALE_MAX_REST];
  const float* head_partials;
  int64_t B;
  int32_t A;
  float* dq;
  float* db;
  const float* loss_rows;
  float* loss_out;
} ebn_dvn_finale;
int ebn_dvn_finale_f32(const ebn_dvn_args* args, const ebn_tn_problem* problems, int32_t n, const ebn_dvn_finale* fin,
                       const ebn_step_state* st, ebn_stream_t stream);

#define EBN_SITE_NPA_CONV 2
#define EBN_SITE_NPA_NEWS_PAP 3
#define EBN_SITE_NPA_USER_PAP 4

int ebn_conv1d_fwd_f32(const float* X, const float* W, const float* bias, float* Vd, int64_t n_titles, int32_t T, int32_t E,
                       int32_t F, int32_t window, const ebn_step_state* st, int32_t conv_site, float conv_p, int32_t pap_site,
                       float pap_p, ebn_stream_t stream);
int ebn_conv1d_bwd_data_f32(const float* dVd, const float* Vd, const float* W, float* dX, int64_t n_titles, int32_t T, int32_t E,
                            int32_t F, int32_t window, const ebn_step_state* st, float conv_p, float pap_p, ebn_stream_t stream);
int ebn_conv1d_wgrad_splits(int64_t n_titles, int32_t T, int32_t E, int32_t F, int32_t window);
int64_t ebn_conv1d_wgrad_workspace_floats(int64_t n_titles, int32_t T, int32_t E, int32_t F, int32_t window, int32_t splits);
// ... 158 lines not shown
```

Baseline: 25550.

## Fuse bias+tanh into attention GEMM epilogue and fuse attpool backward kernels

The forward path now applies bias and tanh inside the direct GEMM epilogue, so the attention-pool kernel only reads the finished U instead of rewriting it. The backward path merges the pool-gradient kernel and the dpre column-reduction kernel into one launch that keeps de in LDS. This is meant to cut a read-modify-write pass over U, one kernel launch, and a global round trip of de. In exchange it adds larger LDS use, with a fallback when that exceeds its limit, and a different work split per block in backward.

```diff
diff --git a/ebnerd-benchmark_amd/csrc/ebn_attlayer2.h b/ebnerd-benchmark_amd/csrc/ebn_attlayer2.h
--- /dev/null
+++ b/ebnerd-benchmark_amd/csrc/ebn_attlayer2.h
@@ -0,0 +1,14 @@
+#pragma once
+#include <hip/hip_runtime.h>
+
+__device__ __forceinline__ float ebn_att_tanh_bias(float pre, float b) {
+#pragma clang fp contract(off)
+  const float s = pre + b;
+  return tanhf(s);
+}
+
+__device__ __forceinline__ float ebn_att_scale_tanh_bias(float alpha, float acc, float b) {
+#pragma clang fp contract(off)
+  const float pre = alpha * acc;
+  return ebn_att_tanh_bias(pre, b);
+}
diff --git a/ebnerd-benchmark_amd/csrc/ebn_attpool.hip b/ebnerd-benchmark_amd/csrc/ebn_attpool.hip
--- a/ebnerd-benchmark_amd/csrc/ebn_attpool.hip
+++ b/ebnerd-benchmark_amd/csrc/ebn_attpool.hip
@@ -1,5 +1,6 @@
 #include "ebn_common.h"
 #include "ebn_reduce.h"
+#include "ebn_attlayer2.h"
 
 namespace {
 
@@ -7,6 +8,7 @@
 constexpr int POOL_WAVES = POOL_THREADS / 64;
 constexpr float KERAS_EPS = 1e-7f;
 
+template <bool FINISHED>
 __global__ __launch_bounds__(POOL_THREADS) void attpool_fwd_kernel(float* __restrict__ U,
                                                                     const float* __restrict__ b,
                                                                     const float* __restrict__ q,
@@ -20,8 +22,8 @@
     float* urow = U + (n * L + l) * A;
     float part = 0.f;
     for (int k = lane; k < A; k += 64) {
-      const float u = tanhf(urow[k] + b[k]);
-      urow[k] = u;
+      const float u = FINISHED ? urow[k] : ebn_att_tanh_bias(urow[k], b[k]);
+      if (!FINISHED) urow[k] = u;
       part = fmaf(u, q[k], part);
     }
     part = ebn_wave_sum(part);
@@ -96,6 +98,7 @@
   return r;
 }
 
+template <bool FINISHED>
 __global__ __launch_bounds__(POOL_THREADS) void attpool_fwd_vec_kernel(float* __restrict__ U,
                                                                         const float* __restrict__ b,
                                                                         const float* __restrict__ q,
@@ -121,12 +124,14 @@
       for (int j = 0; j < POOL_RB; ++j) {
         const int l = l0 + POOL_WAVES * j;
         if (l >= L) break;
-        float4 t;
-        t.x = tanhf(u[j].x + bb.x);
-        t.y = tanhf(u[j].y + bb.y);
-        t.z = tanhf(u[j].z + bb.z);
-        t.w = tanhf(u[j].w + bb.w);
-        if (kok) *reinterpret_cast<float4*>(U + (n * L + l) * A + lane * 4) = t;
+        float4 t = u[j];
+        if (!FINISHED) {
+          t.x = ebn_att_tanh_bias(u[j].x, bb.x);
+          t.y = ebn_att_tanh_bias(u[j].y, bb.y);
+          t.z = ebn_att_tanh_bias(u[j].z, bb.z);
+          t.w = ebn_att_tanh_bias(u[j].w, bb.w);
+          if (kok) *reinterpret_cast<float4*>(U + (n * L + l) * A + lane * 4) = t;
+        }
         float part = kok ? fmaf(t.w, qq.w, fmaf(t.z, qq.z, fmaf(t.y, qq.y, t.x * qq.x))) : 0.f;
         part = ebn_wave_sum(part);
         if (lane == 0) sm[l] = part;
@@ -335,25 +340,147 @@
   }
 }
 
+__global__ __launch_bounds__(POOL_THREADS) void attpool_bwd_fused_vec_kernel(const float* __restrict__ X, const float* __restrict__ w,
+                                                                              const float* __restrict__ dout, float* __restrict__ U,
+                                                                              const float* __restrict__ q, float* __restrict__ de,
+                                                                              float* __restrict__ partials, int64_t R, int L, int E, int A,
+                                                                              int64_t rpb, int de_off, int st_off) {
+  extern __shared__ float sm[];
+  float* sm_de = sm + de_off;
+  float* sm_st = sm + st_off;
+  const int tid = threadIdx.x, lane = tid & 63, wave = tid >> 6;
+  const int E4 = E >> 2;
+  const int64_t r0 = static_cast<int64_t>(blockIdx.x) * rpb;
+  const int64_t r1 = (r0 + rpb < R) ? r0 + rpb : R;
+  const int64_t n0 = r0 / L, n1 = (r1 - 1) / L;
+  constexpr int VL = 4;
+  for (int64_t n = n0; n <= n1; ++n) {
+    float* dw = sm + (n - n0) * L;
+    const float* g = dout + n * E;
+    float4 gg[VL];
+#pragma unroll
+    for (int v = 0; v < VL; ++v) gg[v] = ld4_or_zero(g, (lane + 64 * v) * 4, lane + 64 * v < E4);
+    for (int l0 = wave; l0 < L; l0 += POOL_WAVES * POOL_RB) {
+      float part[POOL_RB];
+#pragma unroll
+      for (int j = 0; j < POOL_RB; ++j) part[j] = 0.f;
+#pragma unroll
+      for (int v = 0; v < VL; ++v) {
+        if (64 * v >= E4) break;
+        float4 x[POOL_RB];
+#pragma unroll
+        for (int j = 0; j < POOL_RB; ++j) {
+          const int l = l0 + POOL_WAVES * j;
+          x[j] = ld4_clamped(X, (n * L + l) * E + (lane + 64 * v) * 4, l < L && lane + 64 * v < E4);
+        }
+#pragma unroll
+        for (int j = 0; j < POOL_RB; ++j)
+          part[j] = fmaf(gg[v].w, x[j].w, fmaf(gg[v].z, x[j].z, fmaf(gg[v].y, x[j].y, fmaf(gg[v].x, x[j].x, part[j]))));
+      }
+#pragma unroll
+      for (int j = 0; j < POOL_RB; ++j) {
+        const int l = l0 + POOL_WAVES * j;
+        const float t = ebn_wave_sum(part[j]);
+        if (lane == 0 && l < L) dw[l] = t;
+      }
+    }
+  }
+  __syncthreads();
+  for (int64_t n = n0 + wave; n <= n1; n += POOL_WAVES) {
+    const float* dw = sm + (n - n0) * L;
+    float s = 0.f;
+    for (int l = lane; l < L; l += 64) s = fmaf(w[n * L + l], dw[l], s);
+    s = ebn_wave_sum(s);
+    for (int l = lane; l < L; l += 64) {
+      const int64_t r = n * L + l;
+      if (r >= r0 && r < r1) {
+        const float d = w[r] * (dw[l] - s);
+        de[r] = d;
+        sm_de[r - r0] = d;
+      }
+    }
+  }
+  __syncthreads();
+  const int A4 = A >> 2, RS = POOL_THREADS / A4;
+  const int c4 = tid % A4, rs = tid / A4;
+  const bool active = rs < RS;
+  float4 dq = make_float4(0.f, 0.f, 0.f, 0.f), db = dq;
+  if (active) {
+    const float4 qk = *reinterpret_cast<const float4*>(q + c4 * 4);
+    for (int64_t rb = r0 + rs; rb < r1; rb += static_cast<int64_t>(8) * RS) {
+      float4 u[8];
+      float der[8];
+#pragma unroll
+      for (int j = 0; j < 8; ++j) {
+        int64_t r = rb + static_cast<int64_t>(j) * RS;
+        r = r < r1 ? r : r1 - 1;
+        u[j] = *reinterpret_cast<const float4*>(U + r * A + c4 * 4);
+        der[j] = sm_de[r - r0];
+      }
+#pragma unroll
+      for (int j = 0; j < 8; ++j) {
+        const int64_t r = rb + static_cast<int64_t>(j) * RS;
+        if (r >= r1) break;
+        const float d = der[j];
+        dq.x = fmaf(d, u[j].x, dq.x);
+        dq.y = fmaf(d, u[j].y, dq.y);
+        dq.z = fmaf(d, u[j].z, dq.z);
+        dq.w = fmaf(d, u[j].w, dq.w);
+        const float4 dp = make_float4(d * qk.x * (1.0f - u[j].x * u[j].x), d * qk.y * (1.0f - u[j].y * u[j].y),
+                                      d * qk.z * (1.0f - u[j].z * u[j].z), d * qk.w * (1.0f - u[j].w * u[j].w));
+        *reinterpret_cast<float4*>(U + r * A + c4 * 4) = dp;
+        db.x += dp.x;
+        db.y += dp.y;
+        db.z += dp.z;
+        db.w += dp.w;
+      }
+    }
+    *reinterpret_cast<float4*>(&sm_st[rs * A + c4 * 4]) = dq;
+    *reinterpret_cast<float4*>(&sm_st[(RS + rs) * A + c4 * 4]) = db;
+  }
+  __syncthreads();
+  for (int k = tid; k < A; k += POOL_THREADS) {
+    float tq = 0.f, tb = 0.f;
+    for (int i = 0; i < RS; ++i) {
+      tq += sm_st[i * A + k];
+      tb += sm_st[(RS + i) * A + k];
+    }
+    partials[(static_cast<int64_t>(blockIdx.x) * 2 + 0) * A + k] = tq;
+    partials[(static_cast<int64_t>(blockIdx.x) * 2 + 1) * A + k] = tb;
+  }
+}
+
 extern "C" int64_t ebn_attpool_partials_len(int64_t R, int32_t A) { return ebn_dim_ok(R, A) ? ebn_colred_blocks(R) * 2 * A : 0; }
+
+template <bool FINISHED>
+static int attpool_fwd(float* U, const float* b, const float* q, const float* X, float* out, float* w, int64_t n_seq, int32_t L,
+                       int32_t E, int32_t A, ebn_stream_t stream) {
+  EBN_REQUIRE(U && (FINISHED || b) && q && X && out && w, EBN_ERR_BAD_ARG);
+  EBN_REQUIRE(n_seq >= 0 && L > 0 && E > 0 && A > 0, EBN_ERR_BAD_ARG);
+  EBN_REQUIRE(L <= 8192, EBN_ERR_UNSUPPORTED);
+  if (n_seq == 0) return EBN_OK;
+  if (FINISHED) b = q;
+  const bool vec = (A % 4 == 0) && A <= 256 && (E % 4 == 0) && E <= 1024 && ebn_aligned16(U) && ebn_aligned16(b) &&
+                   ebn_aligned16(q) && ebn_aligned16(X) && ebn_aligned16(out);
+  if (vec)
+    EBN_LAUNCH(attpool_fwd_vec_kernel<FINISHED>, dim3(static_cast<unsigned>(n_seq)), dim3(POOL_THREADS),
+                       L * sizeof(float), ebn_stream(stream), U, b, q, X, out, w, L, E, A);
+  else
+    EBN_LAUNCH(attpool_fwd_kernel<FINISHED>, dim3(static_cast<unsigned>(n_seq)), dim3(POOL_THREADS),
+                       L * sizeof(float), ebn_stream(stream), U, b, q, X, out, w, L, E, A);
+  EBN_CHECK_LAUNCH();
+  return EBN_OK;
+}
 
 extern "C" int ebn_attpool_fwd_f32(float* U, const float* b, const float* q, const float* X, float* out,
                                    float* w, int64_t n_seq, int32_t L, int32_t E, int32_t A,
                                    ebn_stream_t stream) {
-  EBN_REQUIRE(U && b && q && X && out && w, EBN_ERR_BAD_ARG);
-  EBN_REQUIRE(n_seq >= 0 && L > 0 && E > 0 && A > 0, EBN_ERR_BAD_ARG);
-  EBN_REQUIRE(L <= 8192, EBN_ERR_UNSUPPORTED);
-  if (n_seq == 0) return EBN_OK;
-  const bool vec = (A % 4 == 0) && A <= 256 && (E % 4 == 0) && E <= 1024 && ebn_aligned16(U) && ebn_aligned16(b) &&
-                   ebn_aligned16(q) && ebn_aligned16(X) && ebn_aligned16(out);
-  if (vec)
-    EBN_LAUNCH(attpool_fwd_vec_kernel, dim3(static_cast<unsigned>(n_seq)), dim3(POOL_THREADS),
-                       L * sizeof(float), ebn_stream(stream), U, b, q, X, out, w, L, E, A);
-  else
-    EBN_LAUNCH(attpool_fwd_kernel, dim3(static_cast<unsigned>(n_seq)), dim3(POOL_THREADS),
-                       L * sizeof(float), ebn_stream(stream), U, b, q, X, out, w, L, E, A);
-  EBN_CHECK_LAUNCH();
-  return EBN_OK;
+  return attpool_fwd<false>(U, b, q, X, out, w, n_seq, L, E, A, stream);
+}
+
+extern "C" int ebn_attpool_fwd_u_f32(const float* U, const float* q, const float* X, float* out, float* w, int64_t n_seq,
+                                     int32_t L, int32_t E, int32_t A, ebn_stream_t stream) {
+  return attpool_fwd<true>(const_cast<float*>(U), nullptr, q, X, out, w, n_seq, L, E, A, stream);
 }
 
 extern "C" int ebn_attpool_bwd_pool_f32(const float* X, const float* w, const float* dout, float* dX,
@@ -396,3 +523,25 @@
   EBN_CHECK_LAUNCH();
   return EBN_OK;
 }
+
+
+extern "C" int ebn_attpool_bwd_fused_f32(const float* X, const float* w, const float* dout, float* U, const float* q, float* de,
+                                         float* partials, int64_t n_seq, int32_t L, int32_t E, int32_t A, ebn_stream_t stream) {
+  EBN_REQUIRE(X && w && dout && U && q && de && partials, EBN_ERR_BAD_ARG);
+  EBN_REQUIRE(n_seq >= 0 && L > 0 && E > 0 && A > 0, EBN_ERR_BAD_ARG);
+  if (n_seq == 0) return EBN_OK;
+  if (!((E % 4) == 0 && E <= 1024 && ebn_aligned16(X) && ebn_aligned16(dout) && (A % 4) == 0 && A >= 4 && A <= 1024 && ebn_aligned16(U) &&
+        ebn_aligned16(q)))
+    return EBN_ERR_UNSUPPORTED;
+  const int64_t R = n_seq * L;
+  const int64_t nb = ebn_colred_blocks(R);
+  const int64_t rpb = ebn_ceil_div(R, nb);
+  const int64_t nt = (rpb + L - 2) / L + 1;
+  const int64_t de_off = nt * L, st_off = (de_off + rpb + 3) / 4 * 4;
+  const int64_t lds = (st_off + static_cast<int64_t>(2) * (POOL_THREADS / (A / 4)) * A) * static_cast<int64_t>(sizeof(float));
+  if (lds > 48 * 1024) return EBN_ERR_UNSUPPORTED;
+  EBN_LAUNCH(attpool_bwd_fused_vec_kernel, dim3(static_cast<unsigned>(nb)), dim3(POOL_THREADS), static_cast<size_t>(lds), ebn_stream(stream), X, w,
+                     dout, U, q, de, partials, R, L, E, A, rpb, static_cast<int>(de_off), static_cast<int>(st_off));
+  EBN_CHECK_LAUNCH();
+  return EBN_OK;
+}
diff --git a/ebnerd-benchmark_amd/csrc/ebn_encoder.hip b/ebnerd-benchmark_amd/csrc/ebn_encoder.hip
--- a/ebnerd-benchmark_amd/csrc/ebn_encoder.hip
+++ b/ebnerd-benchmark_amd/csrc/ebn_encoder.hip
@@ -12,9 +12,19 @@
   return EBN_OK;
 }
 
-extern "C" int ebn_encoder_fwd_f32(const ebn_encoder_dims* dims, const ebn_encoder_params* p,
-                                   const ebn_encoder_acts* a, const ebn_encoder_scratch* s,
-                                   const ebn_step_state* st, ebn_stream_t stream) {
+static int att_layer2_fwd(const ebn_encoder_dims* dims, const ebn_encoder_params* p, const ebn_encoder_acts* a, int64_t R, int E,
+                          float* ws, int64_t ws_n, bool epilogue, ebn_stream_t stream) {
+  if (epilogue) {
+    const int rc = ebn_gemm_bias_tanh_f32(R, dims->A, E, 1.0f, a->Y, E, p->W, dims->A, p->b, a->U, dims->A, stream);
+    if (rc == EBN_OK) return ebn_attpool_fwd_u_f32(a->U, p->q, a->Y, a->out, a->w, dims->n_seq, dims->L, E, dims->A, stream);
+    if (rc != EBN_ERR_UNSUPPORTED) return rc;
+  }
+  EBN_TRY(ebn_gemm_f32_ws(0, 0, R, dims->A, E, 1.0f, a->Y, E, p->W, dims->A, 0.0f, a->U, dims->A, ws, ws_n, stream));
+  return ebn_attpool_fwd_f32(a->U, p->b, p->q, a->Y, a->out, a->w, dims->n_seq, dims->L, E, dims->A, stream);
+}
+
+static int encoder_fwd(const ebn_encoder_dims* dims, const ebn_encoder_params* p, const ebn_encoder_acts* a,
+                       const ebn_encoder_scratch* s, const ebn_step_state* st, bool epilogue, ebn_stream_t stream) {
   EBN_TRY(check_dims(dims));
   EBN_REQUIRE(p && a && p->Wqkv && p->W && p->b && p->q, EBN_ERR_BAD_ARG);
   EBN_REQUIRE(a->X && a->QKV && a->Y && a->U && a->w && a->out, EBN_ERR_BAD_ARG);
@@ -27,9 +37,19 @@
                             1, stream));
   EBN_TRY(ebn_attn_fwd_f32(a->QKV, 3 * E, a->Y, E, dims->n_seq, dims->L, dims->h, dims->d, st, dims->drop_site,
                            dims->drop_p, stream));
-  EBN_TRY(ebn_gemm_f32_ws(0, 0, R, dims->A, E, 1.0f, a->Y, E, p->W, dims->A, 0.0f, a->U, dims->A, ws, ws_n, stream));
-  EBN_TRY(ebn_attpool_fwd_f32(a->U, p->b, p->q, a->Y, a->out, a->w, dims->n_seq, dims->L, E, dims->A, stream));
-  return EBN_OK;
+  return att_layer2_fwd(dims, p, a, R, E, ws, ws_n, epilogue, stream);
+}
+
+extern "C" int ebn_encoder_fwd_f32(const ebn_encoder_dims* dims, const ebn_encoder_params* p,
+                                   const ebn_encoder_acts* a, const ebn_encoder_scratch* s,
+                                   const ebn_step_state* st, ebn_stream_t stream) {
+  return encoder_fwd(dims, p, a, s, st, false, stream);
+}
+
+extern "C" int ebn_encoder_fwd_epilogue_f32(const ebn_encoder_dims* dims, const ebn_encoder_params* p,
+                                            const ebn_encoder_acts* a, const ebn_encoder_scratch* s,
+                                            const ebn_step_state* st, ebn_stream_t stream) {
+  return encoder_fwd(dims, p, a, s, st, true, stream);
 }
 
 extern "C" int ebn_encoder_fwd_gather_f32(const ebn_encoder_dims* dims, const ebn_encoder_params* p, const ebn_encoder_acts* a,
diff --git a/ebnerd-benchmark_amd/csrc/ebn_gemm.hip b/ebnerd-benchmark_amd/csrc/ebn_gemm.hip
--- a/ebnerd-benchmark_amd/csrc/ebn_gemm.hip
+++ b/ebnerd-benchmark_amd/csrc/ebn_gemm.hip
@@ -15,7 +15,7 @@
                               float* part, hipStream_t s);
 bool ebn_gemm_direct_wanted(int32_t transA, int32_t transB, int64_t M, int64_t N, int64_t K);
 int ebn_gemm_direct_launch(int32_t transB, int64_t M, int64_t N, int64_t K, float alpha, const float* A, int64_t lda, const float* B,
-                           int64_t ldb, float* C, int64_t ldc, hipStream_t s);
+                           int64_t ldb, float* C, int64_t ldc, const float* bias, hipStream_t s);
 
 namespace {
 
@@ -1125,7 +1125,7 @@
   if ((epi.bias != nullptr || epi.rs != nullptr) && !(vecA && vecB)) return EBN_ERR_UNSUPPORTED;
   if (epi.bias == nullptr && epi.rs == nullptr && beta == 0.f && vecA && (vecB || !transB) &&
       ebn_gemm_direct_wanted(transA, transB, M, N, K)) {
-    const int rc_dir = ebn_gemm_direct_launch(transB, M, N, K, alpha, A, lda, B, ldb, C, ldc, s);
+    const int rc_dir = ebn_gemm_direct_launch(transB, M, N, K, alpha, A, lda, B, ldb, C, ldc, nullptr, s);
     if (rc_dir != EBN_ERR_UNSUPPORTED) return rc_dir;
   }
   if (transA && !transB && epi.bias == nullptr && epi.rs == nullptr && workspace != nullptr &&
@@ -1274,6 +1274,18 @@
                                ebn_stream_t stream) {
   return ebn_gemm_f32_site(transA, transB, M, N, K, alpha, A, lda, B, ldb, beta, C, ldc, workspace, workspace_floats, 0,
                            stream);
+}
+
+extern "C" int ebn_gemm_bias_tanh_f32(int64_t M, int64_t N, int64_t K, float alpha, const float* A, int64_t lda, const float* B,
+                                      int64_t ldb, const float* bias, float* C, int64_t ldc, ebn_stream_t stream) {
+  EBN_REQUIRE(M >= 0 && N >= 0 && K >= 0, EBN_ERR_BAD_ARG);
+  if (M == 0 || N == 0) return EBN_OK;
+  EBN_REQUIRE(A && B && bias && C, EBN_ERR_BAD_ARG);
+  EBN_REQUIRE(lda >= K && ldb >= N && ldc >= N, EBN_ERR_BAD_ARG);
+  const bool spanA = (256 * lda + K + 16) * 4 < (int64_t{1} << 32);
+  const bool vecA = (lda % 4) == 0 && ebn_aligned16(A) && (K % 4) == 0 && spanA;
+  if (!vecA || !ebn_gemm_direct_wanted(0, 0, M, N, K)) return EBN_ERR_UNSUPPORTED;
+  return ebn_gemm_direct_launch(0, M, N, K, alpha, A, lda, B, ldb, C, ldc, bias, ebn_stream(stream));
 }
 
 extern "C" int ebn_dense_bwd_pair_f32(int64_t R, int64_t K_in, int64_t N_out, const float* X, int64_t ldx, const float* dY,
diff --git a/ebnerd-benchmark_amd/csrc/ebn_gemm_direct.hip b/ebnerd-benchmark_amd/csrc/ebn_gemm_direct.hip
--- a/ebnerd-benchmark_amd/csrc/ebn_gemm_direct.hip
+++ b/ebnerd-benchmark_amd/csrc/ebn_gemm_direct.hip
@@ -1,6 +1,7 @@
 #include <stdlib.h>
 
 #include "ebn_common.h"
+#include "ebn_attlayer2.h"
 
 typedef float ebn_dir_f32x4 __attribute__((ext_vector_type(4)));
 typedef int ebn_dir_i32x4 __attribute__((ext_vector_type(4)));
@@ -87,10 +88,10 @@
       for (int c = 0; c < NC; ++c) acc[r][c] = __builtin_amdgcn_mfma_f32_16x16x4f32(f.a[r][s], f.b[c][s], acc[r][c], 0, 0, 0);
 }
 
-template <int R, int NC, bool B_KC, int DEPTH>
+template <int R, int NC, bool B_KC, int DEPTH, bool EPI>
 __device__ __forceinline__ void dir_task(int64_t M, int64_t N, int64_t K, float alpha, const float* __restrict__ A, int64_t lda,
-                                         const float* __restrict__ B, int64_t ldb, float* __restrict__ C, int64_t ldc, int64_t rb0,
-                                         int cb0, int lane) {
+                                         const float* __restrict__ B, int64_t ldb, float* __restrict__ C, int64_t ldc,
+                                         const float* __restrict__ bias, int64_t rb0, int cb0, int lane) {
   const int ln = lane & 15, kq = lane >> 4;
   const int64_t row0 = rb0 * 16;
   DirPlan<R, NC, B_KC> p;
@@ -173,24 +174,48 @@
     dir_mma(acc, f0);
   }
 
-#pragma unroll
-  for (int r = 0; r < R; ++r) {
+  if constexpr (!EPI) {
+    int lane_e = lane;
+    if constexpr (R * NC < 24) asm volatile("" : "+v"(lane_e));
+    const int ln_e = lane_e & 15, kq_e = lane_e >> 4;
+#pragma unroll
+    for (int r = 0; r < R; ++r) {
+#pragma unroll
+      for (int c = 0; c < NC; ++c) {
+        const int64_t col = static_cast<int64_t>(cb0 + c) * 16 + ln_e;
+#pragma unroll
+        for (int i = 0; i < 4; ++i) {
+          const int64_t row = row0 + 16 * r + 4 * kq_e + i;
+          if (row < M && col < N) C[row * ldc + col] = alpha * acc[r][c][i];
+        }
+      }
+    }
+  } else {
+    int lane_e = lane;
+    asm volatile("" : "+v"(lane_e));
+    const int ln_e = lane_e & 15, kq_e = lane_e >> 4;
 #pragma unroll
     for (int c = 0; c < NC; ++c) {
-      const int64_t col = static_cast<int64_t>(cb0 + c) * 16 + ln;
-#pragma unroll
-      for (int i = 0; i < 4; ++i) {
-        const int64_t row = row0 + 16 * r + 4 * kq + i;
-        if (row < M && col < N) C[row * ldc + col] = alpha * acc[r][c][i];
-      }
-    }
-  }
-}
-
-template <int R, int CW, bool B_KC, int DEPTH>
+      const int64_t col = static_cast<int64_t>(cb0 + c) * 16 + ln_e;
+      const float bv = bias[col < N ? col : N - 1];
+#pragma unroll
+      for (int r = 0; r < R; ++r) {
+#pragma unroll
+        for (int i = 0; i < 4; ++i) {
+          const int64_t row = row0 + 16 * r + 4 * kq_e + i;
+          if (row < M && col < N) C[row * ldc + col] = ebn_att_scale_tanh_bias(alpha, acc[r][c][i], bv);
+        }
+      }
+      __builtin_amdgcn_sched_barrier(0);
+    }
+  }
+}
+
+template <int R, int CW, bool B_KC, int DEPTH, bool EPI>
 __global__ __launch_bounds__(256, 2) void gemm_direct16_kernel(int64_t M, int64_t N, int64_t K, float alpha, const float* __restrict__ A,
                                                                int64_t lda, const float* __restrict__ B, int64_t ldb,
-                                                               float* __restrict__ C, int64_t ldc, int32_t G, int32_t n_wide, int64_t n_tasks) {
+                                                               float* __restrict__ C, int64_t ldc, const float* __restrict__ bias, int32_t G,
+                                                               int32_t n_wide, int64_t n_tasks) {
   const int lane = threadIdx.x & 63;
   const int wave = __builtin_amdgcn_readfirstlane(threadIdx.x >> 6);
   const int64_t t = static_cast<int64_t>(blockIdx.x) * 4 + wave;
@@ -198,8 +223,8 @@
   const int64_t rg = t / G;
   const int cg = static_cast<int>(t - rg * G);
   const int cb0 = cg < n_wide ? cg * CW : n_wide * CW + (cg - n_wide) * (CW - 1);
-  if (cg < n_wide) dir_task<R, CW, B_KC, DEPTH>(M, N, K, alpha, A, lda, B, ldb, C, ldc, rg * R, cb0, lane);
-  else dir_task<R, CW - 1, B_KC, DEPTH>(M, N, K, alpha, A, lda, B, ldb, C, ldc, rg * R, cb0, lane);
+  if (cg < n_wide) dir_task<R, CW, B_KC, DEPTH, EPI>(M, N, K, alpha, A, lda, B, ldb, C, ldc, bias, rg * R, cb0, lane);
+  else dir_task<R, CW - 1, B_KC, DEPTH, EPI>(M, N, K, alpha, A, lda, B, ldb, C, ldc, bias, rg * R, cb0, lane);
 }
 
 template <int R, int NC>
@@ -435,11 +460,14 @@
 
 template <int R, int CW>
 int direct_launch_rc(bool b_kc, const DirectPlan& pl, int64_t M, int64_t N, int64_t K, float alpha, const float* A, int64_t lda, const float* B,
-                     int64_t ldb, float* C, int64_t ldc, hipStream_t s) {
+                     int64_t ldb, float* C, int64_t ldc, const float* bias, hipStream_t s) {
   const dim3 grid(static_cast<unsigned>(ebn_ceil_div(pl.tasks, 4))), block(256);
 #define EBN_DIR_GO(KC, DP) \
-  EBN_LAUNCH((gemm_direct16_kernel<R, CW, KC, DP>), grid, block, 0, s, M, N, K, alpha, A, lda, B, ldb, C, ldc, pl.G, pl.n_wide, pl.tasks)
-  if constexpr (R == 1) {
+  EBN_LAUNCH((gemm_direct16_kernel<R, CW, KC, DP, false>), grid, block, 0, s, M, N, K, alpha, A, lda, B, ldb, C, ldc, bias, pl.G, pl.n_wide, pl.tasks)
+  if (bias != nullptr) {
+    if (b_kc) return EBN_ERR_UNSUPPORTED;
+    EBN_LAUNCH((gemm_direct16_kernel<R, CW, false, 2, true>), grid, block, 0, s, M, N, K, alpha, A, lda, B, ldb, C, ldc, bias, pl.G, pl.n_wide, pl.tasks);
+  } else if constexpr (R == 1) {
     if (b_kc) return EBN_ERR_UNSUPPORTED;
     EBN_DIR_GO(false, 2);
   } else if (b_kc) EBN_DIR_GO(true, 2);
@@ -463,13 +491,13 @@
 }
 
 int ebn_gemm_direct_launch(int32_t transB, int64_t M, int64_t N, int64_t K, float alpha, const float* A, int64_t lda, const float* B,
-                           int64_t ldb, float* C, int64_t ldc, hipStream_t s) {
+                           int64_t ldb, float* C, int64_t ldc, const float* bias, hipStream_t s) {
   if ((64 * lda + K) * 4 >= (int64_t{1} << 31) || ((transB ? N : K) * ldb + (transB ? K : N) + 16 * ldb) * 4 >= (int64_t{1} << 31)) return EBN_ERR_UNSUPPORTED;
   const DirectPlan pl = direct_plan(M, N, transB != 0);
   if (pl.R == 0 || ebn_ceil_div(pl.tasks, 4) >= (int64_t{1} << 31)) return EBN_ERR_UNSUPPORTED;
   const bool kc = transB != 0;
 #define EBN_DIR_CASE(RR, CC) \
-  if (pl.R == RR && pl.CW == CC) return direct_launch_rc<RR, CC>(kc, pl, M, N, K, alpha, A, lda, B, ldb, C, ldc, s)
+  if (pl.R == RR && pl.CW == CC) return direct_launch_rc<RR, CC>(kc, pl, M, N, K, alpha, A, lda, B, ldb, C, ldc, bias, s)
   EBN_DIR_CASE(4, 7); EBN_DIR_CASE(3, 7); EBN_DIR_CASE(2, 7); EBN_DIR_CASE(1, 7);
   EBN_DIR_CASE(4, 5); EBN_DIR_CASE(3, 5); EBN_DIR_CASE(2, 5); EBN_DIR_CASE(1, 5);
   EBN_DIR_CASE(4, 4); EBN_DIR_CASE(3, 4); EBN_DIR_CASE(2, 4); EBN_DIR_CASE(1, 4);
diff --git a/ebnerd-benchmark_amd/ebrec/models/newsrec/_engine.py b/ebnerd-benchmark_amd/ebrec/models/newsrec/_engine.py
--- a/ebnerd-benchmark_amd/ebrec/models/newsrec/_engine.py
+++ b/ebnerd-benchmark_amd/ebrec/models/newsrec/_engine.py
@@ -178,6 +178,8 @@
         self.loss_dev = torch.zeros(1, device=self.device)
         self.use_graph = False
         self.fuse_user_head = True
+        self.att_epilogue = True
+        self.att_bwd_fused = True
         self.fuse_eval_gather = True
         self.defer_finish = True
         self.atomic_table_grad = False
@@ -383,7 +385,7 @@
         if pre == "n" and self.precision == "split":
             return self._news_encoder_fwd_split(b, n_seq, X, st, site, p)
         dims, params, acts = self._enc_structs(pre, b, n_seq, X, site, p)
-        _hip.call("ebn_encoder_fwd_f32", ctypes.byref(dims), ctypes.byref(params), ctypes.byref(acts),
+        _hip.call("ebn_encoder_fwd_epilogue_f32" if (train and pre == "n" and self.att_epilogue) else "ebn_encoder_fwd_f32", ctypes.byref(dims), ctypes.byref(params), ctypes.byref(acts),
                   ctypes.byref(self._fwd_scratch(b)), st, _hip.stream_handle())
 
     @staticmethod
@@ -466,6 +468,14 @@
         else:
             self._gemm_prec(b, 0, 0, R, 3 * E, b.Din, X, b.Din, pv("n_Wqkv"), 3 * E, b.QKV, 3 * E)
         _hip.call("ebn_attn_fwd_f32", _hip.ptr(b.QKV), 3 * E, _hip.ptr(b.Y), E, n_seq, T, self.h, self.d, st, site, ctypes.c_float(p), S())
+        if st is not None and self.att_epilogue:
+            rc = _hip.lib().ebn_gemm_bias_tanh_f32(R, A, E, ctypes.c_float(1.0), _hip.ptr(b.Y), E, _hip.ptr(pv("n_W")), A, _hip.ptr(pv("n_b")),
+                                                   _hip.ptr(b.U), A, S())
+            if rc == 0:
+                return _hip.call("ebn_attpool_fwd_u_f32", _hip.ptr(b.U), _hip.ptr(pv("n_q")), _hip.ptr(b.Y), _hip.ptr(b.out), _hip.ptr(b.w),
+                                 n_seq, T, E, A, S())
+            if rc != -2:
+                raise _hip.HipError(f"ebn_gemm_bias_tanh_f32 failed with code {rc}")
         _hip.call("ebn_gemm_f32_ws", 0, 0, R, A, E, ctypes.c_float(1.0), _hip.ptr(b.Y), E, _hip.ptr(pv("n_W")), A, ctypes.c_float(0.0),
                   _hip.ptr(b.U), A, _hip.ptr(b.ws), b.ws.numel(), S())
         _hip.call("ebn_attpool_fwd_f32", _hip.ptr(b.U), _hip.ptr(pv("n_b")), _hip.ptr(pv("n_q")), _hip.ptr(b.Y), _hip.ptr(b.out),
@@ -893,8 +903,15 @@
         L = _hip.lib()
         self._defer_bufs(nb)
         if part == "p1":
-            _hip.call("ebn_attpool_bwd_pool_f32", _hip.ptr(nb.Y), _hip.ptr(nb.w), _hip.ptr(nb.dNE), None, _hip.ptr(nb.de), N, T, E, S())
-            _hip.call("ebn_attpool_bwd_dpre_f32", _hip.ptr(nb.U), _hip.ptr(pv("n_q")), _hip.ptr(nb.de), None, None, _hip.ptr(nb.partials), R, A, 0, S())
+            rc = -2
+            if self.att_bwd_fused:
+                rc = L.ebn_attpool_bwd_fused_f32(_hip.ptr(nb.Y), _hip.ptr(nb.w), _hip.ptr(nb.dNE), _hip.ptr(nb.U), _hip.ptr(pv("n_q")), _hip.ptr(nb.de),
+                                                 _hip.ptr(nb.partials), N, T, E, A, S())
+                if rc not in (0, -2):
+                    raise _hip.HipError(f"ebn_attpool_bwd_fused_f32 failed with code {rc}")
+            if rc == -2:
+                _hip.call("ebn_attpool_bwd_pool_f32", _hip.ptr(nb.Y), _hip.ptr(nb.w), _hip.ptr(nb.dNE), None, _hip.ptr(nb.de), N, T, E, S())
+                _hip.call("ebn_attpool_bwd_dpre_f32", _hip.ptr(nb.U), _hip.ptr(pv("n_q")), _hip.ptr(nb.de), None, None, _hip.ptr(nb.partials), R, A, 0, S())
             n = ctypes.c_int32(0)
             _hip.call("ebn_gemm_f32_partials", 1, 0, E, A, R, one, _hip.ptr(nb.Y), E, _hip.ptr(nb.U), A, _hip.ptr(nb.ws_dw), nb.ws_dw.numel(), ctypes.byref(n), S())
             nb.finish_jobs["dW"] = int(n.value)
diff --git a/ebnerd-benchmark_amd/ebrec/models/newsrec/_engine_segments.py b/ebnerd-benchmark_amd/ebrec/models/newsrec/_engine_segments.py
--- a/ebnerd-benchmark_amd/ebrec/models/newsrec/_engine_segments.py
+++ b/ebnerd-benchmark_amd/ebrec/models/newsrec/_engine_segments.py
@@ -105,7 +105,7 @@
         return self.graph_collectives
 
     def _graph_key(self, B, C, advanced=False):
-        return (B, C, advanced, bool(self.adam_in_finish), bool(self.defer_finish), bool(self.multi))
+        return (B, C, advanced, bool(self.adam_in_finish), bool(self.defer_finish), bool(self.multi), bool(self.att_epilogue), bool(self.att_bwd_fused))
 
     def _capture(self, B, C, advanced=False):
         torch.cuda.synchronize()
diff --git a/include/ebnerd_hip.h b/include/ebnerd_hip.h
--- a/include/ebnerd_hip.h
+++ b/include/ebnerd_hip.h
@@ -154,6 +154,9 @@
                            int64_t lddy, const float* W, int64_t ldw, float beta_w, float* dW, int64_t lddw, float* dX,
                            int64_t lddx, float* workspace, int64_t workspace_floats, ebn_stream_t stream);
 
+int ebn_gemm_bias_tanh_f32(int64_t M, int64_t N, int64_t K, float alpha, const float* A, int64_t lda, const float* B, int64_t ldb,
+                           const float* bias, float* C, int64_t ldc, ebn_stream_t stream);
+
 int ebn_dense_relu_fwd_f32(int64_t M, int64_t N, int64_t K, const float* A, int64_t lda, const float* B, int64_t ldb,
                            const float* bias, float* C, int64_t ldc, float* workspace, int64_t workspace_floats,
                            ebn_stream_t stream);
@@ -161,6 +164,8 @@
 int ebn_attpool_fwd_f32(float* U, const float* b, const float* q, const float* X, float* out,
                         float* w, int64_t n_seq, int32_t L, int32_t E, int32_t A,
                         ebn_stream_t stream);
+int ebn_attpool_fwd_u_f32(const float* U, const float* q, const float* X, float* out, float* w, int64_t n_seq, int32_t L,
+                          int32_t E, int32_t A, ebn_stream_t stream);
 int ebn_attpool_bwd_pool_f32(const float* X, const float* w, const float* dout, float* dX,
                              float* de, int64_t n_seq, int32_t L, int32_t E,
                              ebn_stream_t stream);
@@ -168,6 +173,8 @@
 int ebn_attpool_bwd_dpre_f32(float* U, const float* q, const float* de, float* dq, float* db,
                              float* partials, int64_t R, int32_t A, int32_t accumulate,
                              ebn_stream_t stream);
+int ebn_attpool_bwd_fused_f32(const float* X, const float* w, const float* dout, float* U, const float* q, float* de,
+                              float* partials, int64_t n_seq, int32_t L, int32_t E, int32_t A, ebn_stream_t stream);
 typedef struct ebn_encoder_dims {
   int64_t n_seq;
   int32_t L;
@@ -213,6 +220,9 @@
 int ebn_encoder_fwd_f32(const ebn_encoder_dims* dims, const ebn_encoder_params* params,
                         const ebn_encoder_acts* acts, const ebn_encoder_scratch* scratch,
                         const ebn_step_state* st, ebn_stream_t stream);
+int ebn_encoder_fwd_epilogue_f32(const ebn_encoder_dims* dims, const ebn_encoder_params* params,
+                                 const ebn_encoder_acts* acts, const ebn_encoder_scratch* scratch,
+                                 const ebn_step_state* st, ebn_stream_t stream);
 int ebn_encoder_fwd_gather_f32(const ebn_encoder_dims* dims, const ebn_encoder_params* params, const ebn_encoder_acts* acts,
                                const ebn_encoder_scratch* scratch, const int32_t* ids, const float* table, int64_t table_rows,
                                int32_t* oob_flag, ebn_stream_t stream);
```

Result: no change. 25340 (-0.8%).
